# ZikangYuan/sr_livo

Hardware: AMD Instinct MI355X
Metric: sweeps/s (full ESIKF solve of a 64k-pt Livox sweep vs 1M-pt voxel map) (higher is better)
Workload: dtype f64; 1 GPU; HEADLINE: stream of 4 distinct 65536-keypoint livox sweeps (own poses and priors), 978481-pt voxel map (1000000 target), max_num_residuals=2147483647, r=1, K=20; one full ESIKF solve per sweep, every sweep crosses PCIe once (uploaded on the copy stream during the solve before it: resident in HBM when its solve starts); sweeps drawn with seeds 20251309 + 100 j, keeping those that take sweep 0's 2 E; parallelism=single GPU

## Files before the change

include/srlivo_hip_debug.h:

```cpp
#ifndef SRLIVO_HIP_DEBUG_H
#define SRLIVO_HIP_DEBUG_H

#include "srlivo_hip.h"

#ifdef __cplusplus
extern "C" {
#endif

int srl_debug_set_select_mode(srl_ctx *ctx, int select_mode);

int srl_debug_radix_sort_pairs(srl_ctx *ctx, const uint32_t *keys, int n, int bits, uint32_t *keys_sorted, uint32_t *positions_sorted);

int srl_debug_color_map_rebuilds(srl_ctx *ctx, int32_t *voxel_table, int32_t *grid_table);

int srl_debug_set_frame_order_mode(srl_ctx *ctx, int mode);
int srl_debug_frame_order_used(srl_ctx *ctx, int *used);

int srl_debug_set_gather_counts(srl_ctx *ctx, int nranks, int rank, const int64_t *counts);

int srl_debug_set_ablate(srl_ctx *ctx, int bits);
int srl_debug_set_fused_reduce(srl_ctx *ctx, int enable);
int srl_debug_set_bound_culling(srl_ctx *ctx, int enable);
int srl_debug_set_pose_box(srl_ctx *ctx, int kind);
int srl_debug_set_arm_linger(srl_ctx *ctx, double host_linger_us, double kernel_linger_us);
int srl_debug_pass_stamps(srl_ctx *ctx, int enable, long long *gpu_out, long long *host_out);
int srl_debug_frame_timing(srl_ctx *ctx, int enable, double out16[16]);
int srl_debug_set_frame_epoch(srl_ctx *ctx, int frames_to_wrap);
int srl_debug_set_launch_shape(srl_ctx *ctx, int keypoints_per_wave, int waves_per_workgroup);
int srl_debug_set_search_select_mode(srl_ctx *ctx, int select_mode);
int srl_debug_heap_topk(const double *distances, int n, int K, int32_t *out_index);
int srl_debug_device_sqrt(srl_ctx *ctx, const double *in, int n, double *out);
int srl_debug_block_times(srl_ctx *ctx, double *out, int max_blocks, int *nblocks);
enum { SRL_FLOW_PREV = 0, SRL_FLOW_CUR = 1 };
int srl_flow_levels(srl_ctx *ctx, int *L);
int srl_flow_download_level(srl_ctx *ctx, int which, int level, uint8_t *image_padded, int16_t *deriv_padded, int *rows, int *cols);

#ifdef __cplusplus
}
#endif
#endif
```

sr_livo_amd/capi.py:

```python
import ctypes as C
import os
import re

import numpy as np

_HERE = os.path.dirname(os.path.abspath(__file__))
LIB_PATH = os.environ.get("SRL_LIB_PATH") or os.path.join(_HERE, "libsrlivo_hip.so")
INCLUDE_DIR = os.path.join(os.path.dirname(_HERE), "include")

SRL_OK = 0
SRL_ERR_NO_DEVICE = -1
SRL_ERR_BAD_ARG = -3
SRL_ERR_UNSUPPORTED = -4
SRL_ERR_COMM = -7
SRL_ERR_NAN_PLANARITY = -8
SRL_ERR_NOT_ENOUGH_RESIDUALS = -9
SRL_COMM_ID_BYTES = 128


SRL_PEER_HANDLE_BYTES = 64


class SrlError(RuntimeError):
    def __init__(self, status, what, detail=""):
# ... 181 lines not shown
        "srl_map_insert": ([p, p, C.c_int, C.c_double, C.c_int, C.c_double, C.c_int, C.POINTER(C.c_int)], C.c_int),
        "srl_map_insert_report": ([p, p, C.c_int, C.c_double, C.c_int, C.c_double, C.c_int, C.c_double, p, p, C.POINTER(C.c_int),
                                   C.POINTER(C.c_int)], C.c_int),
        "srl_map_size": ([p, C.POINTER(C.c_int64), C.POINTER(C.c_int32)], C.c_int),
        "srl_map_download": ([p, p, p, p, C.c_int], C.c_int),
        "srl_map_remove_far": ([p, dp, C.c_double, C.POINTER(C.c_int32), C.POINTER(C.c_int64)], C.c_int),
        "srl_map_probe_checksum": ([p, p, C.c_int, C.c_int, C.c_double, C.POINTER(C.c_uint64)], C.c_int),
        "srl_color_opts_default": ([C.POINTER(ColorOpts)], None),
        "srl_color_map_create": ([p, C.POINTER(ColorOpts)], C.c_int),
        "srl_color_map_destroy": ([p], C.c_int),
        "srl_color_map_insert": ([p, p, C.c_int, C.c_double, C.c_double, p, p, C.c_int, p, C.c_int, C.POINTER(ColorTotals)], C.c_int),
        "srl_color_map_size": ([p, C.POINTER(C.c_int64), C.POINTER(C.c_int32), C.POINTER(C.c_int64), C.POINTER(C.c_int64)], C.c_int),
        "srl_color_map_download": ([p, p, p, p, C.c_int, p, p, C.c_int64], C.c_int),
        "srl_color_registered_download": ([p, C.c_int64, C.c_int, p], C.c_int),
        "srl_debug_color_map_rebuilds": ([p, C.POINTER(C.c_int32), C.POINTER(C.c_int32)], C.c_int),
        "srl_color_image_upload": ([p, p, C.c_int, C.c_int, C.c_int64], C.c_int),
        "srl_color_select_opts_default": ([C.POINTER(ColorSelectOpts)], None),
        "srl_color_map_select": ([p, C.POINTER(ColorCamera), C.c_int, C.c_int, p, C.c_int, C.POINTER(ColorSelectOpts), p, C.c_int64,
                                  C.POINTER(ColorSelectTotals)], C.c_int),
        "srl_color_map_render": ([p, C.POINTER(ColorCamera), p, C.c_int, C.c_double, C.POINTER(ColorRenderTotals)], C.c_int),
        "srl_color_map_vio_rows": ([p, C.POINTER(ColorVioArgs), p, C.c_int, C.POINTER(ColorVioSums), p, p], C.c_int),
        "srl_flow_opts_default": ([C.POINTER(FlowOpts)], None),
        "srl_flow_create": ([p, C.POINTER(FlowOpts)], C.c_int),
        "srl_flow_destroy": ([p], C.c_int),
        "srl_flow_track_image": ([p, p, C.c_int, C.c_int, C.c_int64, p, C.c_int, p, p, C.POINTER(C.c_int)], C.c_int),
        "srl_flow_levels": ([p, C.POINTER(C.c_int)], C.c_int),
        "srl_flow_download_level": ([p, C.c_int, C.c_int, p, p, C.POINTER(C.c_int), C.POINTER(C.c_int)], C.c_int),
        "srl_lk_create": ([p, C.c_int, C.c_int, C.c_int, C.c_int, C.c_int, C.c_double, C.c_int, C.c_double, C.POINTER(p)], C.c_int),
        "srl_lk_destroy": ([p], C.c_int),
        "srl_lk_get": ([p, C.POINTER(C.c_int), C.POINTER(C.c_int), C.POINTER(C.c_double)], C.c_int),
        "srl_lk_track_image": ([p, p, C.c_int, C.c_int, C.c_int64, p, C.c_int, p, p, C.POINTER(C.c_int)], C.c_int),
        "srl_color_cloud_opts_default": ([C.POINTER(ColorCloudOpts)], None),
        "srl_color_map_export_cloud": ([p, C.c_int64, C.c_int64, C.POINTER(ColorCloudOpts), p, p, C.c_int64, C.POINTER(ColorCloudTotals)], C.c_int),
        "srl_color_map_download_rgb": ([p, p, p, p, p, p, C.c_int64], C.c_int),
        "srl_color_registered_rgb": ([p, C.c_int64, C.c_int, p, p, p, p, p], C.c_int),
        "srl_sweep_upload": ([p, p, C.c_int], C.c_int),
        "srl_sweep_shard": ([p, C.POINTER(C.c_int), C.POINTER(C.c_int), C.POINTER(C.c_int)], C.c_int),
        "srl_sweep_prefetch": ([p, p, C.c_int], C.c_int),
        "srl_sweep_swap": ([p], C.c_int),
        "srl_sweep_wait": ([p], C.c_int),
        "srl_thread_pin_to_gpu_numa": ([p, C.POINTER(C.c_int)], C.c_int),
        "srl_pinned_alloc": ([C.c_size_t, C.POINTER(p)], C.c_int),
        "srl_pinned_free": ([p], C.c_int),
        "srl_host_register": ([p, C.c_size_t], C.c_int),
        "srl_host_unregister": ([p], C.c_int),
        "srl_comm_backend_info": ([C.c_char_p, C.c_int, C.POINTER(C.c_int), C.POINTER(C.c_int)], C.c_int),
        "srl_build_residuals": ([p, C.POINTER(Frame), C.POINTER(IcpOpts), C.POINTER(NormalEq)], C.c_int),
        "srl_build_residuals_overlap": ([p, C.POINTER(Frame), C.POINTER(IcpOpts), C.POINTER(NormalEq), p, p], C.c_int),
        "srl_set_taps": ([p, C.c_int], C.c_int),
        "srl_fetch_neighbors": ([p, p, p, p], C.c_int),
        "srl_fetch_residuals": ([p, p, p, p, p, p, p], C.c_int),
        "srl_search_neighbors": ([p, p, C.c_int, C.c_int, C.c_double, C.c_int, C.c_int, p, p, p], C.c_int),
        "srl_transform_points": ([p, p, C.c_int, dp, dp, dp, dp, p], C.c_int),
        "srl_frame_upload": ([p, p, C.c_int], C.c_int),
        "srl_frame_undistort": ([p, p, p, p, C.c_int, p, C.c_int, C.c_double, C.c_int, dp, dp, p, p], C.c_int),
        "srl_frame_take": ([p, p, C.c_int], C.c_int),
        "srl_frame_subsample": ([p, p, C.c_int, C.c_double, C.POINTER(C.c_int)], C.c_int),
        "srl_frame_take_subsampled": ([p, p, C.c_int, p, p, p], C.c_int),
        "srl_frame_size": ([p, C.POINTER(C.c_int)], C.c_int),
        "srl_frame_select_keypoints": ([p, dp, dp, dp, dp, C.c_double, p, C.POINTER(C.c_int)], C.c_int),
        "srl_frame_commit_report": ([p, dp, dp, dp, dp, C.c_double, C.c_int, C.c_double, C.c_int, p, p, p, C.POINTER(C.c_int),
                                     C.POINTER(C.c_int)], C.c_int),
        "srl_frame_commit": ([p, dp, dp, dp, dp, C.c_double, C.c_int, C.c_double, C.c_int, p, C.POINTER(C.c_int)], C.c_int),
        "srl_comm_unique_id": ([p], C.c_int),
        "srl_comm_init_rank": ([p, C.c_int, C.c_int, p], C.c_int),
        "srl_comm_destroy": ([p], C.c_int),
        "srl_comm_set_library": ([C.c_char_p], C.c_int),
        "srl_comm_suspend": ([p, C.c_int], C.c_int),
        "srl_comm_info": ([p, C.POINTER(C.c_int), C.POINTER(C.c_int), C.POINTER(C.c_int), C.POINTER(C.c_int), C.POINTER(C.c_int64)], C.c_int),
        "srl_comm_set_host_callbacks": ([p, C.c_int, C.c_int, ALLREDUCE_FN, ALLGATHER_FN, p], C.c_int),
        "srl_debug_set_gather_counts": ([p, C.c_int, C.c_int, C.POINTER(C.c_int64)], C.c_int),
        "srl_peer_export": ([p, p, C.POINTER(p)], C.c_int),
        "srl_peer_attach": ([p, C.c_int, C.c_int, p, C.POINTER(p)], C.c_int),
        "srl_peer_set_deadline_ms": ([p, C.c_int], C.c_int),
        "srl_peer_stats": ([p, C.POINTER(C.c_int64), C.POINTER(C.c_int)], C.c_int),
        "srl_peer_detach": ([p], C.c_int),
        "srl_shard_range": ([C.c_int, C.c_int, C.c_int, C.POINTER(C.c_int), C.POINTER(C.c_int)], None),
        "srl_shard_budget": ([C.c_int, C.POINTER(C.c_int64), C.c_int, C.c_int, C.POINTER(C.c_int64), C.POINTER(C.c_int)], None),
        "srl_get_timing": ([p, C.POINTER(Timing)], C.c_int),
        "srl_debug_block_times": ([p, p, C.c_int, C.POINTER(C.c_int)], C.c_int),
        "srl_debug_set_ablate": ([p, C.c_int], C.c_int),
        "srl_debug_set_fused_reduce": ([p, C.c_int], C.c_int),
        "srl_debug_set_bound_culling": ([p, C.c_int], C.c_int),
        "srl_debug_set_pose_box": ([p, C.c_int], C.c_int),
        "srl_debug_set_arm_linger": ([p, C.c_double, C.c_double], C.c_int),
        "srl_debug_pass_stamps": ([p, C.c_int, p, p], C.c_int),
        "srl_debug_frame_timing": ([p, C.c_int, p], C.c_int),
        "srl_debug_set_frame_epoch": ([p, C.c_int], C.c_int),
        "srl_set_armed_launch": ([p, C.c_int], C.c_int),
        "srl_disarm": ([p], C.c_int),
        "srl_solve_end": ([p], C.c_int),
        "srl_get_arm_stats": ([p, C.POINTER(C.c_uint64)], C.c_int),
        "srl_debug_set_launch_shape": ([p, C.c_int, C.c_int], C.c_int),
        "srl_debug_set_search_select_mode": ([p, C.c_int], C.c_int),
        "srl_debug_set_select_mode": ([p, C.c_int], C.c_int),
        "srl_debug_set_frame_order_mode": ([p, C.c_int], C.c_int),
        "srl_debug_radix_sort_pairs": ([p, p, C.c_int, C.c_int, p, p], C.c_int),
        "srl_debug_frame_order_used": ([p, C.POINTER(C.c_int)], C.c_int),
        "srl_debug_heap_topk": ([p, C.c_int, C.c_int, p], C.c_int),
        "srl_debug_device_sqrt": ([p, p, C.c_int, p], C.c_int),
        "srl_set_profiling": ([p, C.c_int], C.c_int),
        "srl_set_profiling_period": ([p, C.c_int], C.c_int),
        "srl_timing_mark": ([p], C.c_int),
        "srl_lio_create": ([C.c_int, C.POINTER(p)], C.c_int),
        "srl_lio_destroy": ([p], C.c_int),
        "srl_lio_ctx": ([p], p),
        "srl_lio_last_error": ([p], C.c_char_p),
        "srl_lio_set_extrinsics": ([p, dp, dp], C.c_int),
        "srl_lio_set_laser_point_cov": ([p, C.c_double], C.c_int),
        "srl_lio_last_solve_launches": ([p, C.POINTER(C.c_int)], C.c_int),
        "srl_lio_eskf_get_state": ([p, dp], C.c_int),
        "srl_lio_eskf_set_state": ([p, dp], C.c_int),
        "srl_lio_eskf_get_cov": ([p, dp], C.c_int),
        "srl_lio_eskf_set_cov": ([p, dp], C.c_int),
        "srl_lio_eskf_set_noise": ([p, C.c_double, C.c_double, C.c_double, C.c_double], C.c_int),
        "srl_lio_eskf_init_imu": ([p, dp, dp], C.c_int),
        "srl_lio_eskf_scale_init_cov": ([p], C.c_int),
        "srl_lio_eskf_predict": ([p, C.c_double, dp, dp], C.c_int),
        "srl_lio_eskf_observe": ([p, dp], C.c_int),
        "srl_lio_add_points_to_map": ([p, p, C.c_int, C.c_double, C.c_int, C.c_double, C.c_int], C.c_int),
        "srl_lio_map_size": ([p, C.POINTER(C.c_int64)], C.c_int),
        "srl_lio_remove_points_far_from_location": ([p, dp, C.c_double], C.c_int),
        "srl_lio_set_collect_points_world": ([p, C.c_int], C.c_int),
        "srl_lio_points_world": ([p, p, C.c_int, C.POINTER(C.c_int)], C.c_int),
        "srl_lio_set_device_subsample": ([p, C.c_int], C.c_int),
        "srl_lio_set_color_map_options": ([p, C.POINTER(ColorOpts)], C.c_int),
        "srl_lio_set_color_times": ([p, C.c_double, C.c_double, C.c_int], C.c_int),
        "srl_lio_add_points_to_map_at": ([p, p, C.c_int, C.c_double, C.c_int, C.c_double, C.c_int, C.c_double, C.c_int], C.c_int),
        "srl_lio_color_cloud": ([p, C.c_int, C.c_int, p, p, C.c_int64, C.POINTER(C.c_int64), C.POINTER(ColorCloudTotals)], C.c_int),
        "srl_lio_color_cloud_view": ([p, C.c_int, C.c_int, C.c_int, C.POINTER(C.c_void_p), C.POINTER(C.c_void_p), C.POINTER(C.c_int64),
                                      C.POINTER(ColorCloudTotals)], C.c_int),
        "srl_lio_color_topic_sizes": ([p, C.c_int64, p, C.c_int, C.POINTER(C.c_int)], C.c_int),
        "srl_lio_color_topic_state": ([p, C.POINTER(C.c_int), C.POINTER(C.c_int)], C.c_int),
        "srl_lio_select_points_for_projection": ([p, C.POINTER(ColorCamera), C.c_int, C.c_int, C.c_double, C.c_int, C.c_int, C.c_int, p, C.c_int,
                                                  C.POINTER(C.c_int), C.POINTER(ColorSelectTotals)], C.c_int),
        "srl_lio_color_visited": ([p, C.c_int, p, C.c_int, C.POINTER(C.c_int), C.POINTER(C.c_int)], C.c_int),
        "srl_lio_color_stored": ([p, p, C.c_int, C.POINTER(C.c_int)], C.c_int),
        "srl_lio_render_points_in_recent_voxel": ([p, C.POINTER(ColorCamera), C.c_double, C.POINTER(ColorRenderTotals)], C.c_int),
        "srl_lio_probe_checksum_of_committed_frame": ([p, C.c_int, C.c_double, C.POINTER(C.c_uint64), C.POINTER(C.c_int32)], C.c_int),
        "srl_lio_resident_sweep": ([p, p, C.c_int], C.c_int),
        "srl_lio_prefetch_sweep": ([p, p, C.c_int], C.c_int),
        "srl_lio_swap_sweep": ([p], C.c_int),
        "srl_lio_prefetch_sweep_during_solve": ([p, p, C.c_int], C.c_int),
        "srl_lio_update_iekf": ([p, C.POINTER(IcpOpts), p, C.c_int, dp, dp, C.c_int, p, C.c_int,
                                 C.POINTER(C.c_int), C.POINTER(C.c_int)], C.c_int),
        "srl_lio_stream_step": ([p, C.POINTER(IcpOpts), dp, dp, C.c_int, dp, dp, C.c_int, p, C.c_int, C.POINTER(C.c_int), C.POINTER(C.c_int)], C.c_int),
        "srl_lio_update_iekf_provided": ([p, C.POINTER(IcpOpts), PROVIDER_FN, p, C.c_int, dp, dp, C.c_int, p, C.c_int,
                                          C.POINTER(C.c_int), C.POINTER(C.c_int)], C.c_int),
        "srl_lio_optimize": ([p, C.POINTER(IcpOpts), C.c_double, p, p, C.c_int, dp, dp, C.c_int, p,
                              C.POINTER(C.c_int), C.POINTER(C.c_int), C.POINTER(C.c_int)], C.c_int),
        "srl_lio_eskf_try_init": ([p, dp, dp, dp, C.c_int, C.POINTER(C.c_int)], C.c_int),
        "srl_lio_eskf_get_init_stats": ([p, dp], C.c_int),
        "srl_lio_set_initial_flag": ([p, C.c_int], C.c_int),
        "srl_lio_state_initialization": ([p, C.c_int, C.c_int, dp, dp, dp], C.c_int),
        "srl_lio_set_odometry_options": ([p, C.POINTER(OdometryOpts)], C.c_int),
        "srl_lio_run_measurement": ([p, C.c_double, p, p, p, C.c_int, p, p, C.c_int, C.c_double, C.c_double,
                                     C.POINTER(ReplayResult)], C.c_int),
        "srl_lio_last_frame": ([p, C.c_int, p, p, p, C.POINTER(C.c_int)], C.c_int),
        "srl_lio_optimize_resident": ([p, C.POINTER(IcpOpts), C.c_double, p, C.c_int, dp, dp, C.c_int, p,
                                       C.POINTER(C.c_int), C.POINTER(C.c_int), C.POINTER(C.c_int)], C.c_int),
        "srl_lio_commit_frame": ([p, dp, C.c_double, C.c_int, C.c_double, C.c_int, p, C.POINTER(C.c_int)], C.c_int),
        "srl_lio_search_neighbors": ([p, dp, C.c_int, C.c_double, C.c_int, C.c_int, p, p, C.POINTER(C.c_int)], C.c_int),
        "srl_lio_neighborhood": ([p, p, C.c_int, dp, dp, dp, dp], C.c_int),
        "srl_lio_build_plane_residuals": ([p, C.POINTER(IcpOpts), p, C.c_int, dp, dp, C.c_int, p, C.c_int,
                                           C.POINTER(C.c_int), dp, C.POINTER(C.c_int), p], C.c_int),
        "srl_lio_vio_set_options": ([p, C.c_int, C.c_int, C.c_int, p, p, p], C.c_int),
# ... 390 lines not shown
        self._chk(self.lib.srl_sweep_wait(self.h), "srl_sweep_wait")

    def sweep_swap(self):
        self._chk(self.lib.srl_sweep_swap(self.h), "srl_sweep_swap")

    def sweep_shard(self):
        b, c, t = C.c_int(), C.c_int(), C.c_int()
        self._chk(self.lib.srl_sweep_shard(self.h, C.byref(b), C.byref(c), C.byref(t)), "srl_sweep_shard")
        return b.value, c.value, t.value

    def set_taps(self, on):
        self._chk(self.lib.srl_set_taps(self.h, int(on)), "srl_set_taps")

    def set_profiling(self, on):
        self._chk(self.lib.srl_set_profiling(self.h, int(on)), "srl_set_profiling")

    def timing_mark(self):
        self._chk(self.lib.srl_timing_mark(self.h), "srl_timing_mark")

    def set_profiling_period(self, period):
        self._chk(self.lib.srl_set_profiling_period(self.h, int(period)), "srl_set_profiling_period")

    def timing(self):
        t = Timing()
        self._chk(self.lib.srl_get_timing(self.h, C.byref(t)), "srl_get_timing")
        return t

    def _select(self, opts):
        mode = int(getattr(opts, "select_mode", 0) or 0)
        if mode != getattr(self, "_select_mode", 0):
            self._chk(self.lib.srl_debug_set_select_mode(self.h, mode), "srl_debug_set_select_mode")
            self._select_mode = mode

    def build_residuals(self, frame, opts, allow=(SRL_ERR_NAN_PLANARITY,)):
        self._select(opts)
        out = NormalEq()
        rc = self._chk(self.lib.srl_build_residuals(self.h, C.byref(frame), C.byref(opts), C.byref(out)), "srl_build_residuals", ok=allow)
        return out, rc

    def build_residuals_overlap(self, frame, opts, fn, allow=(SRL_ERR_NAN_PLANARITY,)):
        self._select(opts)
        out = NormalEq()
        cb = C.CFUNCTYPE(None, C.c_void_p)(lambda _u: fn())
        rc = self._chk(self.lib.srl_build_residuals_overlap(self.h, C.byref(frame), C.byref(opts), C.byref(out), cb, None),
                       "srl_build_residuals_overlap", ok=allow)
        return out, rc

    def pin_thread_to_gpu_numa(self):
        node = C.c_int(-1)
        rc = self.lib.srl_thread_pin_to_gpu_numa(self.h, C.byref(node))
        return node.value if rc == 0 else None

    def fetch_neighbors(self, K=20):
        _, n, _ = self.sweep_shard()
        ids = np.empty((n, K), dtype=np.int32)
        status = np.empty(n, dtype=np.uint8)
        ncand = np.empty(n, dtype=np.int32)
        self._chk(self.lib.srl_fetch_neighbors(self.h, _ptr(ids), _ptr(status), _ptr(ncand)), "srl_fetch_neighbors")
        return ids, status, ncand

    def fetch_residuals(self):
        _, n, _ = self.sweep_shard()
        normal = np.empty((n, 3)); a2d = np.empty(n); w = np.empty(n); off = np.empty(n); d = np.empty(n); J = np.empty((n, 6))
        self._chk(self.lib.srl_fetch_residuals(self.h, _ptr(normal), _ptr(a2d), _ptr(w), _ptr(off), _ptr(d), _ptr(J)), "srl_fetch_residuals")
        return dict(normal=normal, a2D=a2d, weight=w, norm_offset=off, distance=d, jacobian=J)

    def search_neighbors(self, world_xyz, nb=1, size=1.0, K=20, thr=1):
        q = _f64(world_xyz, (-1, 3))
        ids = np.empty((len(q), K), dtype=np.int32)
        xyz = np.empty((len(q), K, 3), dtype=np.float32)
        nf = np.empty(len(q), dtype=np.int32)
        self._chk(self.lib.srl_search_neighbors(self.h, _ptr(q), len(q), nb, size, K, thr, _ptr(ids), _ptr(xyz), _ptr(nf)), "srl_search_neighbors")
        return ids, xyz, nf

    def set_launch_shape(self, kpw, wpb):
        self._chk(self.lib.srl_debug_set_launch_shape(self.h, int(kpw), int(wpb)), "srl_debug_set_launch_shape")

    def set_fused_reduce(self, on):
        self._chk(self.lib.srl_debug_set_fused_reduce(self.h, 1 if on else 0), "srl_debug_set_fused_reduce")

    def set_bound_culling(self, on):
        self._chk(self.lib.srl_debug_set_bound_culling(self.h, 1 if on else 0), "srl_debug_set_bound_culling")

    def set_search_select_mode(self, mode):
        self._chk(self.lib.srl_debug_set_search_select_mode(self.h, int(mode)), "srl_debug_set_search_select_mode")

    def set_armed_launch(self, on):
        mode = int(on) if on in (0, 1, 2) and not isinstance(on, bool) else (1 if on else 0)
        self._chk(self.lib.srl_set_armed_launch(self.h, mode), "srl_set_armed_launch")

    def solve_end(self):
        self._chk(self.lib.srl_solve_end(self.h), "srl_solve_end")

    def disarm(self):
        self._chk(self.lib.srl_disarm(self.h), "srl_disarm")

    def arm_stats(self):
        out = (C.c_uint64 * 4)()
        self._chk(self.lib.srl_get_arm_stats(self.h, out), "srl_get_arm_stats")
        return dict(zip(("armed", "fired", "cancelled", "expired"), (int(v) for v in out)))

    def set_pose_box(self, kind):
        self._chk(self.lib.srl_debug_set_pose_box(self.h, int(kind)), "srl_debug_set_pose_box")

    FRAME_STAGES = ("upload", "select_group", "select_download", "select_host_order", "select_gather", "commit_transform", "commit_download",
                    "insert_sort", "insert_segments", "insert_lookup_create", "insert_replay")

    def set_frame_epoch(self, frames_to_wrap):
        self._chk(self.lib.srl_debug_set_frame_epoch(self.h, int(frames_to_wrap)), "srl_debug_set_frame_epoch")

    def frame_timing(self, enable=True):
        out = np.zeros(16)
        self._chk(self.lib.srl_debug_frame_timing(self.h, 1 if enable else 0, _ptr(out)), "srl_debug_frame_timing")
        return dict(zip(self.FRAME_STAGES, (float(v) for v in out)))

    def pass_stamps(self, enable=True, read=True):
        g = np.zeros((64, 32), dtype=np.int64); h = np.zeros((64, 4), dtype=np.int64)
        self._chk(self.lib.srl_debug_pass_stamps(self.h, 1 if enable else 0, _ptr(g) if read else None, _ptr(h) if read else None), "srl_debug_pass_stamps")
        return g, h

    def set_arm_linger(self, host_linger_us=150.0, kernel_linger_us=300.0):
        self._chk(self.lib.srl_debug_set_arm_linger(self.h, float(host_linger_us), float(kernel_linger_us)), "srl_debug_set_arm_linger")

    def device_sqrt(self, x):
        x = _f64(x).ravel()
        out = np.empty_like(x)
        self._chk(self.lib.srl_debug_device_sqrt(self.h, _ptr(x), len(x), _ptr(out)), "srl_debug_device_sqrt")
        return out

    def transform_points(self, raw_xyz, q, t, R_il=None, t_il=None):
        r = _f64(raw_xyz, (-1, 3))
        out = np.empty_like(r)
        R_il = _f64(np.eye(3) if R_il is None else R_il).ravel()
        t_il = _f64(np.zeros(3) if t_il is None else t_il)
        self._chk(self.lib.srl_transform_points(self.h, _ptr(r), len(r), _dptr(_f64(q)), _dptr(_f64(t)), _dptr(R_il), _dptr(t_il), _ptr(out)), "srl_transform_points")
        return out

    def frame_upload(self, raw_xyz):
        r = _f64(raw_xyz, (-1, 3))
        self._chk(self.lib.srl_frame_upload(self.h, _ptr(r), len(r)), "srl_frame_upload")

    def frame_undistort(self, raw_xyz, relative_time_ms, imu_states, time_frame_begin, mode, R_il=None, t_il=None, imu_point_in=None,
                        want_outputs=True):
        r = _f64(raw_xyz, (-1, 3)); rel = _f64(relative_time_ms)
        st = _f64(imu_states, (-1, 17))
        R_il = _f64(np.eye(3) if R_il is None else R_il).ravel()
        t_il = _f64(np.zeros(3) if t_il is None else t_il)
        pin = None if imu_point_in is None else _f64(imu_point_in, (-1, 3))
        imu = np.empty_like(r) if want_outputs else None
        out = np.empty_like(r) if want_outputs else None
        self._chk(self.lib.srl_frame_undistort(self.h, _ptr(r), _ptr(rel), None if pin is None else _ptr(pin), len(r), _ptr(st), len(st),
                                               float(time_frame_begin), int(mode), _dptr(R_il), _dptr(t_il), _ptr(imu), _ptr(out)),
                  "srl_frame_undistort")
        return imu, out

    def frame_take(self, index):
        idx = np.ascontiguousarray(index, dtype=np.int32)
        self._chk(self.lib.srl_frame_take(self.h, _ptr(idx), len(idx)), "srl_frame_take")

    def frame_subsample(self, order, sample_size):
        o = np.ascontiguousarray(order, dtype=np.int32)
        m = C.c_int()
        self._chk(self.lib.srl_frame_subsample(self.h, _ptr(o), len(o), float(sample_size), C.byref(m)), "srl_frame_subsample")
        self._kept = m.value
        return m.value

# ... 627 lines not shown
```

sr_livo_amd/csrc/srl_capi.cpp:

```cpp
#include "../../include/srlivo_hip.h"
#include "../../include/srlivo_hip_debug.h"
#include "host/srl_la.h"
#include "srl_device.h"
#include "srl_hash.h"
#include "srl_heap.h"

#include <hip/hip_runtime.h>
#include <sched.h>

#include <algorithm>
#include <atomic>
#include <chrono>
#include <climits>
#include <cstdio>
#include <cstdlib>
#include <cstring>
#include <mutex>
#include <string>
#include <vector>

struct SrlMapState;
int srl_map_insert_device(struct srl_ctx *ctx, const double *world_xyz, int n, double voxel_size, int cap,
                          double min_distance_points, int min_num_points, int *num_added);

#include "srl_ctx.h"
int srl_map_insert_report_device(srl_ctx *ctx, const double *world_xyz, int n, double voxel_size, int cap, double min_distance_points, int min_num_points,
                                 double ref_z, uint8_t *outcome, srl_cloud_point *cloud, int *num_cloud, int *num_added);

namespace {

unsigned next_pow2(unsigned v) { unsigned p = 1; while (p < v) p <<= 1; return p; }
inline long long steady_ns() { return std::chrono::duration_cast<std::chrono::nanoseconds>(std::chrono::steady_clock::now().time_since_epoch()).count(); }

constexpr int SRL_MAX_DEVICES = 64;
std::atomic<int> g_live_ctx[SRL_MAX_DEVICES];
inline int live_contexts(int device) { return (device >= 0 && device < SRL_MAX_DEVICES) ? g_live_ctx[device].load(std::memory_order_relaxed) : 1; }

int ensure_work(srl_ctx *ctx, int n) {
    if (n <= ctx->work_cap) return SRL_OK;
    const int cap = std::max(n, 1024);
    const int nblocks = std::max((cap + SRL_KPB - 1) / SRL_KPB, 1024 + 8);
    int rc;
    if ((rc = ensure(ctx, ctx->d_rec, (size_t)cap * 8))) return rc;
    if ((rc = ensure(ctx, ctx->d_status, (size_t)cap))) return rc;
    if ((rc = ensure(ctx, ctx->d_bound, (size_t)cap * 4))) return rc;
    ctx->bound_n = 0;
    if ((rc = ensure(ctx, ctx->d_partials, (size_t)nblocks * SRL_PART_STRIDE))) return rc;
    if ((rc = ensure(ctx, ctx->d_binfo, (size_t)nblocks))) return rc;
    ctx->work_cap = cap;
    ctx->block_cap = nblocks;
    return SRL_OK;
}

bool srl_is_pinned(const void *p) {
    hipPointerAttribute_t attr;
    if (hipPointerGetAttributes(&attr, p) != hipSuccess) { (void)hipGetLastError(); return false; }
    return attr.type == hipMemoryTypeHost;
}

int srl_ring_init(srl_ctx *ctx) {
    if (ctx->h_ring) return SRL_OK;
    HIPCHK(ctx, hipHostMalloc((void **)&ctx->h_ring, (size_t)srl_ctx::RING_SLOTS * srl_ctx::RING_SLOT_BYTES, hipHostMallocDefault));
    for (int i = 0; i < srl_ctx::RING_SLOTS; i++) { HIPCHK(ctx, hipEventCreateWithFlags(&ctx->ring_ev[i], hipEventDisableTiming)); ctx->ring_busy[i] = false; }
    return SRL_OK;
}

int ensure_taps(srl_ctx *ctx, int n, int K) {
    if (n <= ctx->tap_cap && K <= ctx->tap_K) return SRL_OK;
    const int cap = std::max(n, ctx->tap_cap), kk = std::max(K, ctx->tap_K);
    int rc;
    if ((rc = ensure(ctx, ctx->d_tap_ids, (size_t)cap * kk))) return rc;
    if ((rc = ensure(ctx, ctx->d_tap_ncand, (size_t)cap))) return rc;
    if ((rc = ensure(ctx, ctx->d_tap_normal, (size_t)cap * 3))) return rc;
    if ((rc = ensure(ctx, ctx->d_tap_a2d, (size_t)cap))) return rc;
    if ((rc = ensure(ctx, ctx->d_tap_offset, (size_t)cap))) return rc;
    ctx->tap_cap = cap;
    ctx->tap_K = kk;
    return SRL_OK;
}

}

int srl_ctx_ensure_work(srl_ctx *ctx, int n) { return ensure_work(ctx, n); }
bool srl_ctx_is_pinned(const void *p) { return srl_is_pinned(p); }

int srl_ctx_grow_map(srl_ctx *ctx, unsigned need_slabs, unsigned need_slots);

extern "C" {

int srl_device_count(int *count) {
    int c = 0;
    if (hipGetDeviceCount(&c) != hipSuccess) { if (count) *count = 0; return SRL_ERR_NO_DEVICE; }
    if (count) *count = c;
    return SRL_OK;
}

const char *srl_status_str(int s) {
    switch (s) {
        case SRL_OK: return "ok";
        case SRL_ERR_NO_DEVICE: return "no HIP device (the product has no CPU fallback)";
        case SRL_ERR_HIP: return "HIP runtime error";
        case SRL_ERR_BAD_ARG: return "bad argument";
        case SRL_ERR_UNSUPPORTED: return "option outside the supported envelope";
        case SRL_ERR_NO_MAP: return "no map uploaded";
        case SRL_ERR_NO_SWEEP: return "no sweep uploaded";
        case SRL_ERR_COMM: return "RCCL error";
        case SRL_ERR_NAN_PLANARITY: return "NaN planarity (optimize.cpp:348-350 throws)";
        case SRL_ERR_NOT_ENOUGH_RESIDUALS: return "not enough residuals (optimize.cpp:110)";
        default: return "unknown status";
    }
}

void srl_icp_opts_default(srl_icp_opts *o) {
    o->threshold_voxel_occupancy = 1;
    o->init_num_frames = 20;
    o->size_voxel_map = 1.0;
    o->num_iters_icp = 5;
    o->min_number_neighbors = 20;
    o->voxel_neighborhood = 1;
    o->power_planarity = 2.0;
    o->max_number_neighbors = 20;
    o->max_dist_to_plane_icp = 0.3;
    o->threshold_orientation_norm = 0.1;
    o->threshold_translation_norm = 0.01;
    o->max_num_residuals = 600;
    o->weight_alpha = 0.9;
    o->weight_neighborhood = 0.1;
}

int srl_ctx_create(int device, srl_ctx **out) {
    if (!out) return SRL_ERR_BAD_ARG;
    *out = nullptr;
    int count = 0;
    if (hipGetDeviceCount(&count) != hipSuccess || count <= 0 || device < 0 || device >= count) return SRL_ERR_NO_DEVICE;
    if (hipSetDevice(device) != hipSuccess) return SRL_ERR_NO_DEVICE;
    srl_ctx *ctx = new srl_ctx();
    ctx->device = device;
    { int cu = 0; if (hipDeviceGetAttribute(&cu, hipDeviceAttributeMultiprocessorCount, device) == hipSuccess && cu > 0) ctx->num_cu = cu; }
    if (hipStreamCreateWithFlags(&ctx->stream, hipStreamNonBlocking) != hipSuccess) { delete ctx; return SRL_ERR_NO_DEVICE; }
    if (hipMalloc((void **)&ctx->d_out, sizeof(SrlDevOut)) != hipSuccess ||
        hipHostMalloc((void **)&ctx->h_out, sizeof(SrlDevOut)) != hipSuccess ||
        hipMalloc((void **)&ctx->d_count, sizeof(long long)) != hipSuccess ||
        hipHostMalloc((void **)&ctx->h_count, sizeof(long long)) != hipSuccess) {
        delete ctx;
        return SRL_ERR_HIP;
    }
    {
        const size_t row_bytes = (size_t)(SRL_FUSED_MAX_BLOCKS + SRL_FUSED_MAX_GROUPS) * SRL_ROW_GRANULES * 8;
        if (hipMalloc((void **)&ctx->d_granules, row_bytes) != hipSuccess || hipMemset(ctx->d_granules, 0, row_bytes) != hipSuccess) { delete ctx; return SRL_ERR_HIP; }
    }
    if (hipHostMalloc((void **)&ctx->h_mail, sizeof(SrlMailbox), hipHostMallocCoherent | hipHostMallocMapped) != hipSuccess) {
        delete ctx;
        return SRL_ERR_HIP;
    }
    std::memset(ctx->h_mail, 0, sizeof(SrlMailbox));
    for (int i = 0; i < 4; i++) hipEventCreate(&ctx->ev[i]);
    if (device < SRL_MAX_DEVICES) g_live_ctx[device].fetch_add(1, std::memory_order_relaxed);
    ctx->counted = true;
    *out = ctx;
    return SRL_OK;
}

int srl_ctx_destroy(srl_ctx *ctx) {
    if (!ctx) return SRL_OK;
    hipSetDevice(ctx->device);
    if (ctx->counted && ctx->device < SRL_MAX_DEVICES) g_live_ctx[ctx->device].fetch_sub(1, std::memory_order_relaxed);
    if (ctx->armed) srl_ctx_disarm(ctx);
    if (ctx->stream) hipStreamSynchronize(ctx->stream);
    if (ctx->copy_stream) hipStreamSynchronize(ctx->copy_stream);
    if (ctx->color) srl_color_map_destroy(ctx);
    if (ctx->flow) srl_flow_destroy(ctx);
    if (ctx->pose_box_pinned) hipHostFree(ctx->pose_box_pinned);
    if (ctx->pose_box_dev) hipFree(ctx->pose_box_dev);
    if (ctx->d_pose_relay) hipFree(ctx->d_pose_relay);
    if (ctx->comm && srl_rccl()) srl_rccl()->CommDestroy(ctx->comm);
    if (ctx->parked_comm && srl_rccl()) srl_rccl()->CommDestroy(ctx->parked_comm);
    if (ctx->d_sub_kept) hipFree(ctx->d_sub_kept);
    if (ctx->d_sub_seen) hipFree(ctx->d_sub_seen);
    void *bufs[] = {ctx->d_corr_in, ctx->d_corr_rel, ctx->d_corr_imu, ctx->d_corr_raw, ctx->d_corr_seg, ctx->d_frame_raw, ctx->d_frame_world, ctx->d_table, ctx->d_slabs, ctx->d_raw, ctx->d_rec, ctx->d_status, ctx->d_partials, ctx->d_binfo,
                    ctx->d_out, ctx->d_count, ctx->d_bound, ctx->d_granules, ctx->d_rec_granules, ctx->d_raw_next, ctx->d_stage_next, ctx->d_stage_cur, ctx->d_tap_ids, ctx->d_tap_ncand, ctx->d_tap_normal, ctx->d_tap_a2d,
                    ctx->d_tap_offset, ctx->d_gather, ctx->d_peer, ctx->d_mail};
    for (int r = 0; r < SRL_MAX_PEERS; r++) if (ctx->peer_mapped[r]) hipIpcCloseMemHandle(ctx->peer_mapped[r]);
    if (ctx->d_inbox) hipFree(ctx->d_inbox);
    for (void *b : bufs) if (b) hipFree(b);
    if (ctx->h_out) hipHostFree(ctx->h_out);
    if (ctx->h_count) hipHostFree(ctx->h_count);
    if (ctx->h_mail) hipHostFree(ctx->h_mail);
    if (ctx->h_arm_stamps) hipHostFree(ctx->h_arm_stamps);
    if (ctx->h_scratch) hipHostFree(ctx->h_scratch);
    if (ctx->h_frame_x) hipHostFree(ctx->h_frame_x);
    for (SrlEpochTable *t : {&ctx->sel_table, &ctx->ins_table}) { if (t->keyw) hipFree(t->keyw); if (t->minw) hipFree(t->minw); }
    if (ctx->d_frame_sync) hipFree(ctx->d_frame_sync);
    if (ctx->d_tr1_sched) hipFree(ctx->d_tr1_sched);
    if (ctx->h_insert_cnt) hipHostFree(ctx->h_insert_cnt);
    if (ctx->ev_insert) hipEventDestroy(ctx->ev_insert);
    if (ctx->ev_world) hipEventDestroy(ctx->ev_world);
    if (ctx->ev_frame_read) hipEventDestroy(ctx->ev_frame_read);
    if (ctx->h_ring) { hipHostFree(ctx->h_ring); for (int i = 0; i < srl_ctx::RING_SLOTS; i++) if (ctx->ring_ev[i]) hipEventDestroy(ctx->ring_ev[i]); }
    for (auto &b : ctx->pool_free) hipFree(b.p);
    ctx->pool_free.clear();
    for (int i = 0; i < 4; i++) if (ctx->ev[i]) hipEventDestroy(ctx->ev[i]);
    for (int i = 0; i < srl_ctx::PROF_RING; i++) for (int k = 0; k < 2; k++) if (ctx->ring[i][k]) hipEventDestroy(ctx->ring[i][k]);
    for (int sl = 0; sl < 2; sl++) for (int k = 0; k < 2; k++) if (ctx->up_ev[sl][k]) hipEventDestroy(ctx->up_ev[sl][k]);
    if (ctx->upload_ev) hipEventDestroy(ctx->upload_ev);
    if (ctx->copy_stream) { hipStreamSynchronize(ctx->copy_stream); hipStreamDestroy(ctx->copy_stream); }
    if (ctx->prefix_stream) { hipStreamSynchronize(ctx->prefix_stream); hipStreamDestroy(ctx->prefix_stream); }
    if (ctx->stream) hipStreamDestroy(ctx->stream);
    delete ctx;
    return SRL_OK;
}

const char *srl_last_error(const srl_ctx *ctx) { return ctx ? ctx->err.c_str() : "null context"; }

int srl_map_upload(srl_ctx *ctx, const int16_t *keys_xyz, const int32_t *counts, const float *xyz, int V, int cap) {
    if (!ctx || V < 0 || (V > 0 && (!keys_xyz || !counts || !xyz))) return SRL_ERR_BAD_ARG;
    SRL_DISARM(ctx);
    if (cap != SRL_VOXEL_CAP) { ctx->err = "max_num_points_in_voxel must be 20"; return SRL_ERR_UNSUPPORTED; }
    HIPCHK(ctx, hipSetDevice(ctx->device));
    { const int rcs = srl_map_settle(ctx); if (rcs) return rcs; }
    ctx->bound_n = 0;
    const unsigned slab_cap = std::max<unsigned>(1024u, (unsigned)V + (unsigned)V / 2u + 4096u);
    if (slab_cap > SRL_MAX_SLABS) { ctx->err = "map too large: slab byte offsets are 32-bit (16.7 M voxels)"; return SRL_ERR_UNSUPPORTED; }
    const unsigned table_cap = next_pow2(std::max<unsigned>(2048u, SRL_TABLE_FACTOR * slab_cap));
    std::vector<SrlSlab> slabs((size_t)V);
    std::vector<SrlMapSlot> table((size_t)table_cap);
    for (auto &s : table) { s.key = SRL_EMPTY_KEY; s.slab = 0; s.count = 0; }
    long long npts = 0;
    const unsigned mask = table_cap - 1;
    for (int v = 0; v < V; v++) {
        SrlSlab &s = slabs[v];
        std::memset(&s, 0, sizeof s);
        const int c = counts[v];
        if (c < 0 || c > cap) { ctx->err = "voxel count out of range"; return SRL_ERR_BAD_ARG; }
        for (int i = 0; i < c; i++)
            for (int d = 0; d < 3; d++) s.xyz[i][d] = xyz[((size_t)v * cap + i) * 3 + d];
        s.count = (unsigned)c;
        s.key = srl_pack_key(keys_xyz[3 * v], keys_xyz[3 * v + 1], keys_xyz[3 * v + 2]);
        npts += c;
        unsigned h = srl_hash_key(s.key) & mask;
        while (table[h].key != SRL_EMPTY_KEY) {
            if (table[h].key == s.key) { ctx->err = "duplicate voxel key in upload"; return SRL_ERR_BAD_ARG; }
            h = (h + 1) & mask;
        }
        table[h].key = s.key;
        table[h].slab = (unsigned)v;
        table[h].count = (unsigned)c;
    }
    if (ctx->d_slabs) { HIPCHK(ctx, hipFree(ctx->d_slabs)); ctx->d_slabs = nullptr; }
    if (ctx->d_table) { HIPCHK(ctx, hipFree(ctx->d_table)); ctx->d_table = nullptr; }
    HIPCHK(ctx, hipMalloc((void **)&ctx->d_slabs, ((size_t)slab_cap + 1) * SRL_SLAB_BYTES));
    HIPCHK(ctx, hipMemsetD32Async((hipDeviceptr_t)(ctx->d_slabs + (size_t)slab_cap * SRL_SLAB_BYTES), 0x7f800000, SRL_SLAB_BYTES / 4, ctx->stream));
    HIPCHK(ctx, hipMalloc((void **)&ctx->d_table, (size_t)table_cap * sizeof(SrlMapSlot)));
    HIPCHK(ctx, hipMemsetAsync(ctx->d_slabs, 0, (size_t)slab_cap * SRL_SLAB_BYTES, ctx->stream));
    if (V > 0) HIPCHK(ctx, hipMemcpyAsync(ctx->d_slabs, slabs.data(), (size_t)V * SRL_SLAB_BYTES, hipMemcpyHostToDevice, ctx->stream));
    HIPCHK(ctx, hipMemcpyAsync(ctx->d_table, table.data(), (size_t)table_cap * sizeof(SrlMapSlot), hipMemcpyHostToDevice, ctx->stream));
    HIPCHK(ctx, hipStreamSynchronize(ctx->stream));
    ctx->slab_cap = slab_cap;
    ctx->table_cap = table_cap;
    ctx->num_voxels = V;
    ctx->num_points = npts;
    return SRL_OK;
}

int srl_map_size(srl_ctx *ctx, int64_t *num_points, int32_t *num_voxels) {
    if (!ctx) return SRL_ERR_BAD_ARG;
    { const int rcs = srl_map_settle(ctx); if (rcs) return rcs; }
    if (num_points) *num_points = ctx->num_points;
    if (num_voxels) *num_voxels = ctx->num_voxels;
    return SRL_OK;
}

int srl_map_download(srl_ctx *ctx, int16_t *keys_xyz, int32_t *counts, float *xyz, int max_voxels) {
    if (!ctx) return SRL_ERR_BAD_ARG;
    SRL_DISARM(ctx);
    if (!ctx->d_slabs) return SRL_ERR_NO_MAP;
    { const int rcs = srl_map_settle(ctx); if (rcs) return rcs; }
    const int V = ctx->num_voxels;
    if (max_voxels < V) return SRL_ERR_BAD_ARG;
    HIPCHK(ctx, hipSetDevice(ctx->device));
    std::vector<SrlSlab> slabs((size_t)V);
    if (V > 0) HIPCHK(ctx, hipMemcpyAsync(slabs.data(), ctx->d_slabs, (size_t)V * SRL_SLAB_BYTES, hipMemcpyDeviceToHost, ctx->stream));
    HIPCHK(ctx, hipStreamSynchronize(ctx->stream));
    for (int v = 0; v < V; v++) {
        short x, y, z;
        srl_unpack_key(slabs[v].key, &x, &y, &z);
        if (keys_xyz) { keys_xyz[3 * v] = x; keys_xyz[3 * v + 1] = y; keys_xyz[3 * v + 2] = z; }
        if (counts) counts[v] = (int32_t)slabs[v].count;
        if (xyz)
            for (int i = 0; i < SRL_CAP; i++)
                for (int d = 0; d < 3; d++)
                    xyz[((size_t)v * SRL_CAP + i) * 3 + d] = (i < (int)slabs[v].count) ? slabs[v].xyz[i][d] : 0.0f;
    }
    return SRL_OK;
}

int srl_map_insert(srl_ctx *ctx, const double *world_xyz, int n, double voxel_size, int cap,
                   double min_distance_points, int min_num_points, int *num_added) {
    if (!ctx || n < 0 || (n > 0 && !world_xyz)) return SRL_ERR_BAD_ARG;
    SRL_DISARM(ctx);
    if (cap != SRL_VOXEL_CAP) { ctx->err = "max_num_points_in_voxel must be 20"; return SRL_ERR_UNSUPPORTED; }
    return srl_map_insert_device(ctx, world_xyz, n, voxel_size, cap, min_distance_points, min_num_points, num_added);
}

int srl_map_insert_report(srl_ctx *ctx, const double *world_xyz, int n, double voxel_size, int cap, double min_distance_points, int min_num_points,
                          double ref_z, uint8_t *outcome, srl_cloud_point *cloud, int *num_cloud, int *num_added) {
    if (num_cloud) *num_cloud = 0;
    if (num_added) *num_added = 0;
    if (!ctx || n < 0 || (n > 0 && !world_xyz)) return SRL_ERR_BAD_ARG;
    SRL_DISARM(ctx);
    if (cap != SRL_VOXEL_CAP) { ctx->err = "max_num_points_in_voxel must be 20"; return SRL_ERR_UNSUPPORTED; }
    return srl_map_insert_report_device(ctx, world_xyz, n, voxel_size, cap, min_distance_points, min_num_points, ref_z, outcome, cloud, num_cloud, num_added);
}

namespace {
int upload_aos(srl_ctx *ctx, const char *src, size_t bytes, double *d_stage, hipStream_t st, bool last = true, int pinned = -1) {
    if (pinned < 0 ? srl_is_pinned(src) : pinned != 0) {
        HIPCHK(ctx, hipMemcpyAsync(d_stage, src, bytes, hipMemcpyHostToDevice, st));
        if (last) {
            if (!ctx->upload_ev) HIPCHK(ctx, hipEventCreateWithFlags(&ctx->upload_ev, hipEventDisableTiming));
            HIPCHK(ctx, hipEventRecord(ctx->upload_ev, st));
            ctx->upload_pending = true;
        }
        return SRL_OK;
    }
    int rc2 = srl_ring_init(ctx);
    if (rc2) return rc2;
    size_t off = 0;
    while (off < bytes) {
        const size_t len = std::min(bytes - off, (size_t)srl_ctx::RING_SLOT_BYTES);
        const int slot = ctx->ring_next++ % srl_ctx::RING_SLOTS;
        if (ctx->ring_busy[slot]) { HIPCHK(ctx, hipEventSynchronize(ctx->ring_ev[slot])); ctx->ring_busy[slot] = false; }
        std::memcpy(ctx->h_ring + (size_t)slot * srl_ctx::RING_SLOT_BYTES, src + off, len);
        {
            hipError_t e__ = hipMemcpyAsync(reinterpret_cast<char *>(d_stage) + off, ctx->h_ring + (size_t)slot * srl_ctx::RING_SLOT_BYTES, len,
                                            hipMemcpyHostToDevice, st);
            if (e__ != hipSuccess) {
                char buf[256];
                std::snprintf(buf, sizeof buf, "ring upload: %s (dst %p + %zu, ring %p slot %d, len %zu, stream %p, main stream %p)", hipGetErrorString(e__),
                              (void *)d_stage, off, (void *)ctx->h_ring, slot, len, (void *)st, (void *)ctx->stream);
                ctx->err = buf;
                return SRL_ERR_HIP;
            }
        }
        HIPCHK(ctx, hipEventRecord(ctx->ring_ev[slot], st));
        ctx->ring_busy[slot] = true;
        off += len;
    }
    return SRL_OK;
}
}

int srl_sweep_upload(srl_ctx *ctx, const double *raw_xyz, int n) {
    if (!ctx || n < 0 || (n > 0 && !raw_xyz)) return SRL_ERR_BAD_ARG;
    SRL_DISARM(ctx);
    HIPCHK(ctx, hipSetDevice(ctx->device));
    int b = 0, cnt = 0;
    srl_shard_range(n, ctx->nranks, ctx->rank, &b, &cnt);
    ctx->total_n = n;
    ctx->shard_begin = b;
    ctx->n = cnt;
    ctx->sweep_loaded = true;
    ctx->taps_valid = false;
    ctx->passes_in_solve = 0;
    ctx->tail_pending = false;
    ctx->bound_n = 0;
    if (cnt > ctx->sweep_cap) {
        const int cap = std::max(cnt, 1024);
        int rc = ensure(ctx, ctx->d_raw, (size_t)cap * 3);
        if (rc) return rc;
        ctx->sweep_cap = cap;
    }
    int rc = ensure_work(ctx, cnt);
    if (rc) return rc;
    if (cnt > 0) {
        int rcu = upload_aos(ctx, reinterpret_cast<const char *>(raw_xyz + (size_t)b * 3), (size_t)cnt * 3 * sizeof(double), ctx->d_rec, ctx->stream);
        if (rcu) return rcu;
        HIPCHK(ctx, srl_launch_aos_to_soa(ctx->d_rec, cnt, ctx->d_raw, ctx->d_raw + ctx->sweep_cap, ctx->d_raw + 2 * (size_t)ctx->sweep_cap, ctx->stream));
    }
    ctx->soa_valid_n = cnt;
    return SRL_OK;
}

int srl_sweep_wait(srl_ctx *ctx) {
    if (!ctx) return SRL_ERR_BAD_ARG;
    SRL_DISARM(ctx);
    if (ctx->upload_pending) {
        HIPCHK(ctx, hipSetDevice(ctx->device));
        HIPCHK(ctx, hipEventSynchronize(ctx->upload_ev));
        if (ctx->prefix_stream) HIPCHK(ctx, hipStreamSynchronize(ctx->prefix_stream));
        ctx->upload_pending = false;
    }
    return SRL_OK;
}

int srl_sweep_prefetch(srl_ctx *ctx, const double *raw_xyz, int n) {
    if (!ctx || n < 0 || (n > 0 && !raw_xyz)) return SRL_ERR_BAD_ARG;
    HIPCHK(ctx, hipSetDevice(ctx->device));
    if (!ctx->copy_stream) SRL_DISARM(ctx);
    { const int rcc = ensure_copy_stream(ctx); if (rcc) return rcc; }
    if (!ctx->up_ev[0][0]) {
        SRL_DISARM(ctx);
        for (int sl = 0; sl < 2; sl++) for (int k = 0; k < 2; k++) HIPCHK(ctx, hipEventCreateWithFlags(&ctx->up_ev[sl][k], hipEventDisableTiming));
    }
    int b = 0, cnt = 0;
    srl_shard_range(n, ctx->nranks, ctx->rank, &b, &cnt);
    if (cnt > ctx->next_cap || cnt > ctx->stage_next_cap) {
        const int cap = std::max(cnt, 1024);
        SRL_DISARM(ctx);
        HIPCHK(ctx, hipStreamSynchronize(ctx->copy_stream));
        int rc;
        if (cnt > ctx->next_cap) { if ((rc = ensure(ctx, ctx->d_raw_next, (size_t)cap * 3))) return rc; ctx->next_cap = cap; HIPCHK(ctx, hipMemsetAsync(ctx->d_raw_next, 0, (size_t)cap * 3 * sizeof(double), ctx->copy_stream)); }
        if (cnt > ctx->stage_next_cap) { if ((rc = ensure(ctx, ctx->d_stage_next, (size_t)cap * 3))) return rc; ctx->stage_next_cap = cap; }
    }
    const int slot = ctx->next_slot ^ 1;
    const int pre = (ctx->prefix_hint > 0 && ctx->prefix_hint < cnt) ? ctx->prefix_hint : cnt;
    if (cnt > 0) {
        const char *src = reinterpret_cast<const char *>(raw_xyz + (size_t)b * 3);
        const int pinned = srl_is_pinned(src) ? 1 : 0;
        if (pre < cnt && pinned) {
            if (!ctx->prefix_stream) { SRL_DISARM(ctx); HIPCHK(ctx, hipStreamCreateWithFlags(&ctx->prefix_stream, hipStreamNonBlocking)); }
            int rcu = upload_aos(ctx, src, (size_t)pre * 3 * sizeof(double), ctx->d_stage_next, ctx->prefix_stream, false, 1);
            if (rcu) return rcu;
            HIPCHK(ctx, hipEventRecord(ctx->up_ev[slot][0], ctx->prefix_stream));
            rcu = upload_aos(ctx, src + (size_t)pre * 3 * sizeof(double), (size_t)(cnt - pre) * 3 * sizeof(double), ctx->d_stage_next + (size_t)pre * 3, ctx->copy_stream, true, 1);
            if (rcu) return rcu;
            ctx->up_one_dma[slot] = false;
        } else {
            int rcu = upload_aos(ctx, src, (size_t)cnt * 3 * sizeof(double), ctx->d_stage_next, ctx->copy_stream, true, pinned);
            if (rcu) return rcu;
            ctx->up_one_dma[slot] = true;
        }
    } else {
        ctx->up_one_dma[slot] = true;
    }
    HIPCHK(ctx, hipEventRecord(ctx->up_ev[slot][1], ctx->copy_stream));
    ctx->next_ready = ctx->up_ev[slot][1];
    ctx->next_slot = slot; ctx->next_prefix_n = ctx->up_one_dma[slot] ? cnt : pre;
    ctx->next_n = cnt; ctx->next_begin = b; ctx->next_total = n;
    return SRL_OK;
}

int srl_sweep_swap(srl_ctx *ctx) {
    if (!ctx) return SRL_ERR_BAD_ARG;
    if (ctx->next_n < 0) { SRL_DISARM(ctx); ctx->err = "srl_sweep_swap: nothing prefetched"; return SRL_ERR_NO_SWEEP; }
    HIPCHK(ctx, hipSetDevice(ctx->device));
    const bool one_dma = ctx->up_one_dma[ctx->next_slot];
    hipEvent_t ev_full = ctx->up_ev[ctx->next_slot][1], ev_pre = ctx->up_ev[ctx->next_slot][one_dma ? 1 : 0];
    hipError_t up_pre = hipEventQuery(ev_pre);
    hipError_t up = (one_dma || up_pre != hipSuccess) ? up_pre : hipEventQuery(ev_full);
    if (up_pre == hipErrorNotReady && ctx->armed && ctx->next_n <= ctx->work_cap) {
        const long long t_give_up = steady_ns() + 25000;
        while ((up_pre = hipEventQuery(ev_pre)) == hipErrorNotReady && steady_ns() < t_give_up) { }
    }
    for (hipError_t e : {up, up_pre})
        if (e != hipSuccess && e != hipErrorNotReady) { ctx->err = std::string("hipEventQuery: ") + hipGetErrorString(e); return SRL_ERR_HIP; }
    if (up_pre != hipSuccess || ctx->next_n > ctx->work_cap) SRL_DISARM(ctx);
    if (up_pre != hipSuccess) {
        HIPCHK(ctx, hipStreamWaitEvent(ctx->stream, ev_full, 0));
        if (!one_dma) HIPCHK(ctx, hipStreamWaitEvent(ctx->stream, ev_pre, 0));
        up = hipSuccess;
    }
    ctx->tail_pending = up != hipSuccess;
    ctx->bound_n = 0;
    ctx->cur_slot = ctx->next_slot;
    ctx->cur_prefix_n = up == hipSuccess ? ctx->next_n : ctx->next_prefix_n;
    ctx->passes_in_solve = 0;
    std::swap(ctx->d_raw, ctx->d_raw_next);
    std::swap(ctx->sweep_cap, ctx->next_cap);
    std::swap(ctx->d_stage_cur, ctx->d_stage_next);
    std::swap(ctx->stage_cur_cap, ctx->stage_next_cap);
    ctx->soa_valid_n = 0;
    ctx->n = ctx->next_n; ctx->shard_begin = ctx->next_begin; ctx->total_n = ctx->next_total;
    ctx->next_n = -1;
    ctx->sweep_loaded = true;
    ctx->taps_valid = false;
    return ensure_work(ctx, ctx->n);
}

int srl_thread_pin_to_gpu_numa(srl_ctx *ctx, int *numa_node) {
    if (!ctx) return SRL_ERR_BAD_ARG;
    if (numa_node) *numa_node = -1;
    char bus[64] = {0};
    if (hipDeviceGetPCIBusId(bus, (int)sizeof bus, ctx->device) != hipSuccess) { (void)hipGetLastError(); return SRL_ERR_UNSUPPORTED; }
    for (char *c = bus; *c; ++c) if (*c >= 'A' && *c <= 'F') *c = (char)(*c - 'A' + 'a');
    const std::string base = std::string("/sys/bus/pci/devices/") + bus;
    int node = -1;
    if (FILE *f = std::fopen((base + "/numa_node").c_str(), "r")) { if (std::fscanf(f, "%d", &node) != 1) node = -1; std::fclose(f); }
    char list[1024] = {0};
    if (FILE *f = std::fopen((base + "/local_cpulist").c_str(), "r")) { if (!std::fgets(list, (int)sizeof list, f)) list[0] = 0; std::fclose(f); }
    if (node < 0 || !list[0]) return SRL_ERR_UNSUPPORTED;
    cpu_set_t allowed, want;
    CPU_ZERO(&want);
    if (sched_getaffinity(0, sizeof allowed, &allowed) != 0) return SRL_ERR_UNSUPPORTED;
    int any = 0;
    for (const char *p = list; *p && *p != '\n';) {
        char *end = nullptr;
        const long a = std::strtol(p, &end, 10);
        long b = a;
        if (end == p) break;
        p = end;
        if (*p == '-') { b = std::strtol(p + 1, &end, 10); p = end; }
        for (long c = a; c <= b && c < CPU_SETSIZE; ++c) if (CPU_ISSET((int)c, &allowed)) { CPU_SET((int)c, &want); any = 1; }
        if (*p == ',') ++p;
    }
    if (!any) return SRL_ERR_UNSUPPORTED;
    if (sched_setaffinity(0, sizeof want, &want) != 0) return SRL_ERR_UNSUPPORTED;
    if (numa_node) *numa_node = node;
    return SRL_OK;
}

int srl_pinned_alloc(size_t bytes, void **out) {
    if (!out) return SRL_ERR_BAD_ARG;
    *out = nullptr;
    if (hipHostMalloc(out, bytes ? bytes : 1, hipHostMallocDefault) != hipSuccess) { (void)hipGetLastError(); return SRL_ERR_HIP; }
    return SRL_OK;
}
int srl_pinned_free(void *p) {
    if (!p) return SRL_OK;
    return hipHostFree(p) == hipSuccess ? SRL_OK : SRL_ERR_HIP;
}
int srl_host_register(void *p, size_t bytes) {
    if (!p || !bytes) return SRL_ERR_BAD_ARG;
    if (hipHostRegister(p, bytes, hipHostRegisterDefault) != hipSuccess) { (void)hipGetLastError(); return SRL_ERR_HIP; }
    return SRL_OK;
}
int srl_host_unregister(void *p) {
    if (!p) return SRL_ERR_BAD_ARG;
    if (hipHostUnregister(p) != hipSuccess) { (void)hipGetLastError(); return SRL_ERR_HIP; }
    return SRL_OK;
}

int srl_sweep_shard(srl_ctx *ctx, int *begin, int *count, int *total) {
    if (!ctx) return SRL_ERR_BAD_ARG;
    if (begin) *begin = ctx->shard_begin;
    if (count) *count = ctx->n;
    if (total) *total = ctx->total_n;
    return SRL_OK;
}

int srl_set_taps(srl_ctx *ctx, int enable) {
    if (!ctx) return SRL_ERR_BAD_ARG;
    SRL_DISARM(ctx);
    ctx->taps = enable != 0;
    if (!ctx->taps) ctx->taps_valid = false;
    return SRL_OK;
}
// ... 272 lines not shown
    const bool init_mode = f->frame_id < o->init_num_frames;
    p.nb = init_mode ? 2 : o->voxel_neighborhood;
    p.thr = init_mode ? 1 : o->threshold_voxel_occupancy;
    p.K = o->max_number_neighbors;
    if (p.nb < 1 || p.nb > 2) { ctx->err = "voxel_neighborhood must be 1 or 2"; return SRL_ERR_UNSUPPORTED; }
    if (p.K < 1 || p.K > SRL_MAX_NEIGHBORS) { ctx->err = "max_number_neighbors must be in [1,32]"; return SRL_ERR_UNSUPPORTED; }
    if (!(o->size_voxel_map > 0.0)) return SRL_ERR_BAD_ARG;

    p.kpw = srl_keypoints_per_wave(n_eff);
    p.wpb = 4;
    const int k1 = srl_keypoints_per_wave_one_round(n_eff, ctx->num_cu);
    if (n_eff >= 2048 && srl_assoc_lds_bytes(p.K, p.nb, k1, 16) <= SRL_LDS_LIMIT) { p.kpw = k1; p.wpb = 16; }
    if (ctx->force_kpw) {
        p.kpw = ctx->force_kpw;
        const bool only16 = p.kpw != 4 && p.kpw != 8 && p.kpw != 16;
        p.wpb = ((ctx->force_wpb == 16 || only16) && srl_assoc_lds_bytes(p.K, p.nb, p.kpw, 16) <= SRL_LDS_LIMIT) ? 16 : 4;
        if (only16 && p.wpb != 16) p.kpw = 4;
    }
    if (ctx->ablate != 0 && srl_assoc_lds_bytes(p.K, p.nb, 16, 16) <= SRL_LDS_LIMIT) { p.kpw = 16; p.wpb = 16; }
    p.kpb = p.kpw * p.wpb;
    p.nblocks = (n_eff + p.kpb - 1) / p.kpb;

    p.cut = cut_possible(ctx, o);
    p.transport = pass_transport(ctx);
    p.dbg_gather = ctx->dbg_gather;
    const bool fusable = !ctx->taps && ctx->ablate == 0 && o->max_num_residuals > 0 && ctx->fuse_reduce && !ctx->dbg_gather;
    p.fuse_cut = fusable && p.cut && p.transport == Transport::single && p.wpb == 16 && p.kpb <= SRL_FUSED_CUT_MAX_KPB && p.nblocks <= 512;
    p.fused = p.fuse_cut || (fusable && !p.cut && p.wpb == 16 && p.nblocks <= SRL_FUSED_MAX_BLOCKS);
    p.tagged_mail = p.fused && p.transport != Transport::rccl;
    p.mailbox = p.transport != Transport::rccl && (p.transport == Transport::single || p.fused);
    const bool fast_sel = ctx->select_mode == 0 || ctx->select_mode == 4;
    p.arm_ok = ctx->arm_mode != 0 && p.fused && fast_sel && ctx->profiling != 1 && (p.transport != Transport::host_callback || ctx->cb_ar);
    return SRL_OK;
}

static void prepare_assoc_args(srl_ctx *ctx, const srl_frame *f, const srl_icp_opts *o, int n_eff, const PassPlan &p, SrlAssocArgs &a) {
    std::memset(&a, 0, sizeof a);
    a.raw_x = ctx->d_raw;
    a.raw_y = ctx->d_raw + ctx->sweep_cap;
    a.raw_z = ctx->d_raw + 2 * (size_t)ctx->sweep_cap;
    a.n = n_eff;
    a.aos = (n_eff > ctx->soa_valid_n) ? ctx->d_stage_cur : nullptr;
    a.table = ctx->d_table;
    a.table_mask = ctx->table_cap - 1;
    a.slabs = ctx->d_slabs;
    a.inf_off = ctx->slab_cap * (unsigned)SRL_SLAB_BYTES;
    a.write_rec = ((ctx->taps || p.cut) && !p.fuse_cut) ? 1 : 0;
    {
        const srl::Quat q(f->q[0], f->q[1], f->q[2], f->q[3]);
        const srl::Mat3 Rn = q.normalized().toRotationMatrix();
        const srl::Mat3 R = q.toRotationMatrix();
        std::memcpy(a.Rn, Rn.a, sizeof a.Rn);
        std::memcpy(a.R, R.a, sizeof a.R);
    }
    std::memcpy(a.t, f->t, sizeof a.t);
    std::memcpy(a.t_last, f->t_last, sizeof a.t_last);
    std::memcpy(a.R_il, f->R_il, sizeof a.R_il);
    std::memcpy(a.t_il, f->t_il, sizeof a.t_il);
    a.size_voxel = o->size_voxel_map;
    a.max_dist = o->max_dist_to_plane_icp;
    {
        double lw = std::abs(o->weight_alpha), ln = std::abs(o->weight_neighborhood);
        const double sum = lw + ln;
        lw /= sum;
        ln /= sum;
        a.lambda_w = lw;
        a.lambda_n = ln;
    }
    a.power_planarity = o->power_planarity;
    a.nbr_scale = o->max_dist_to_plane_icp * o->min_number_neighbors;
    a.K = p.K;
    a.min_nb = o->min_number_neighbors;
    a.thr_cap = p.thr;
    a.select_mode = ctx->select_mode;
    a.ablate = ctx->ablate;
    a.stamps = ctx->h_arm_stamps;
    a.rec = ctx->d_rec;
    a.status = ctx->d_status;
    a.partials = ctx->d_partials;
    a.binfo = ctx->d_binfo;
    if (ctx->taps) {
        a.tap_ids = ctx->d_tap_ids;
        a.tap_ncand = ctx->d_tap_ncand;
        a.tap_normal = ctx->d_tap_normal;
        a.tap_a2d = ctx->d_tap_a2d;
        a.tap_offset = ctx->d_tap_offset;
    }
    {
        float sv = (float)o->size_voxel_map;
        int sv_bits; std::memcpy(&sv_bits, &sv, 4);
        const int sig[4] = {p.K, p.nb, p.thr, sv_bits};
        if (std::memcmp(sig, ctx->bound_sig, sizeof sig) != 0) { ctx->bound_n = 0; std::memcpy(ctx->bound_sig, sig, sizeof sig); }
        a.bound_out = ctx->d_bound;
        a.bound_in = ctx->bound_mode != 0 ? ctx->d_bound : nullptr;
        a.bound_use = a.bound_in ? std::min(ctx->bound_n, n_eff) : 0;
    }
    if (p.fused) {
        a.granules = ctx->d_granules;
        a.mailbox = p.transport == Transport::rccl ? ctx->d_mail : ctx->h_mail;
        a.mail_tagged = p.tagged_mail ? 1 : 0;
    }
    if (p.fuse_cut) {
        a.rec_granules = ctx->d_rec_granules;
        a.cut_max = o->max_num_residuals;
    }
}

static int grow_pass_buffers(srl_ctx *ctx, const PassPlan &p) {
    int rc;
    ctx->taps_valid = false;
    if (ctx->taps) {
        if ((rc = ensure_taps(ctx, ctx->n, p.K))) return rc;
        if (ctx->n > 0) {
            HIPCHK(ctx, hipMemsetAsync(ctx->d_tap_ids, 0xFF, (size_t)ctx->n * p.K * sizeof(int), ctx->stream));
            HIPCHK(ctx, hipMemsetAsync(ctx->d_tap_normal, 0, (size_t)ctx->n * 3 * sizeof(double), ctx->stream));
            HIPCHK(ctx, hipMemsetAsync(ctx->d_tap_a2d, 0, (size_t)ctx->n * sizeof(double), ctx->stream));
            HIPCHK(ctx, hipMemsetAsync(ctx->d_tap_offset, 0, (size_t)ctx->n * sizeof(double), ctx->stream));
        }
    }
    ctx->last_nblocks = p.nblocks;
    if (p.nblocks > ctx->block_cap) {
        if ((rc = ensure(ctx, ctx->d_partials, (size_t)p.nblocks * SRL_PART_STRIDE))) return rc;
        if ((rc = ensure(ctx, ctx->d_binfo, (size_t)p.nblocks))) return rc;
        ctx->block_cap = p.nblocks;
    }
    if (ctx->profiling == 2 && ctx->ring_head - ctx->ring_tail >= (unsigned)srl_ctx::PROF_RING && (rc = drain_ring(ctx, true))) return rc;
    if (p.fused && p.transport == Transport::rccl && !ctx->d_mail && (rc = ensure(ctx, ctx->d_mail, 1))) return rc;
    const size_t need = (size_t)p.nblocks * p.kpb * 16;
    if (p.fuse_cut && need > ctx->rec_granule_cap) {
        if ((rc = ensure(ctx, ctx->d_rec_granules, need))) return rc;
        HIPCHK(ctx, hipMemsetAsync(ctx->d_rec_granules, 0, need * sizeof(unsigned long long), ctx->stream));
        ctx->rec_granule_cap = need;
    }
    return SRL_OK;
}

struct ExchangeTag { unsigned long long seq; unsigned epoch; int slot; };
static ExchangeTag exchange_tag(unsigned long long seq) {
    if ((unsigned)seq == 0u) ++seq;
    return {seq, (unsigned)seq, (int)(seq & 1ull)};
}
static ExchangeTag next_exchange(srl_ctx *ctx) {
    const ExchangeTag t = exchange_tag(ctx->peer_seq + 1);
    ctx->peer_seq = t.seq;
    return t;
}

static SrlAssocArgs arm_signature(const SrlAssocArgs &src) {
    SrlAssocArgs sg = src;
    std::memset(sg.Rn, 0, sizeof sg.Rn); std::memset(sg.R, 0, sizeof sg.R); std::memset(sg.t, 0, sizeof sg.t);
    std::memset(sg.t_last, 0, sizeof sg.t_last);
    sg.pose_box = nullptr; sg.pose_relay = nullptr; sg.pose_relayed = 0; sg.pose_epoch = 0; sg.arm_linger_ticks = 0;
    sg.raw_x = sg.raw_y = sg.raw_z = nullptr; sg.alt_x = sg.alt_y = sg.alt_z = nullptr; sg.n = 0; sg.aos = nullptr; sg.alt_aos = nullptr;
    sg.bound_use = 0;
    return sg;
}

static int fire_or_cancel(srl_ctx *ctx, const PassPlan &p, SrlAssocArgs &a, unsigned long long &seq_now, bool &fired) {
    fired = false;
    bool needs_tail = false;
    if (ctx->tail_pending) {
        if (hipEventQuery(ctx->up_ev[ctx->cur_slot][1]) == hipSuccess) { ctx->tail_pending = false; ctx->cur_prefix_n = ctx->n; }
        else needs_tail = a.n > ctx->cur_prefix_n;
        (void)hipGetLastError();
    }
    if (!ctx->armed) return SRL_OK;
    const SrlAssocArgs sg = arm_signature(a);
    const double age_us = (double)(steady_ns() - ctx->armed_at_ns) * 1e-3;
    const bool on_raw = a.raw_x == ctx->armed_raw && ctx->sweep_cap == ctx->armed_raw_cap && a.aos == nullptr;
    const bool on_alt = !on_raw && ctx->armed_alt != nullptr && a.raw_x == ctx->armed_alt && ctx->sweep_cap == ctx->armed_alt_cap &&
                        a.aos != nullptr && a.aos == ctx->armed_alt_aos;
    if (p.arm_ok && !needs_tail && age_us < ctx->arm_host_linger_us && p.nb == ctx->armed_nb && p.kpw == ctx->armed_kpw &&
        p.nblocks <= ctx->armed_nblocks && (on_raw || on_alt) && std::memcmp(&sg, &ctx->armed_sig, sizeof sg) == 0) {
        pose_box_write(ctx, a.Rn, a.R, a.t, (unsigned)seq_now, SRL_ARM_GO | (on_alt ? SRL_ARM_ALT : 0u), (unsigned)a.n, a.t_last);
        ctx->armed = false;
        ctx->armed_ring = -1;
        ctx->arm_stats[1]++;
        ctx->cur_measured = ctx->armed_measured;
        ctx->cur_gen = ctx->armed_gen;
        fired = true;
        return SRL_OK;
    }
    if (const int rc = srl_ctx_disarm(ctx)) return rc;
    seq_now = ++ctx->seq;
    if (p.fused) a.seq = seq_now;
    return SRL_OK;
}

static int prof_role(const srl_ctx *ctx) {
    if (ctx->prof_period <= 1) return 2;
    const unsigned long long r = ctx->prof_count % (unsigned long long)ctx->prof_period;
    return r == 1 ? 2 : (r == 0 ? 1 : 0);
}

static int launch_assoc(srl_ctx *ctx, const PassPlan &p, const SrlAssocArgs &args, bool armed) {
    if (!armed && ctx->tail_pending) {
        HIPCHK(ctx, hipStreamWaitEvent(ctx->stream, ctx->up_ev[ctx->cur_slot][1], 0));
        ctx->tail_pending = false; ctx->cur_prefix_n = ctx->n;
    }
    const bool prof = ctx->profiling == 1, prof_light = ctx->profiling == 2;
    const int role = prof_light ? prof_role(ctx) : 0;
    int prev = -1;
    if (armed && role != 0) {
        int rc;
        if (ctx->ring_head - ctx->ring_tail >= (unsigned)srl_ctx::PROF_RING - 2 && (rc = drain_ring(ctx, true))) return rc;
        if (ctx->ring_head != 0 && !ctx->ring_void[(ctx->ring_head - 1) % srl_ctx::PROF_RING] && ctx->ring_last_count == (long long)ctx->prof_count - 1)
            prev = (int)((ctx->ring_head - 1) % srl_ctx::PROF_RING);
    }
    const unsigned slot = ctx->ring_head % srl_ctx::PROF_RING;
    if (prof) HIPCHK(ctx, hipEventRecord(ctx->ev[0], ctx->stream));
    if (role == 2 && prev < 0) HIPCHK(ctx, hipEventRecord(ctx->ring[slot][0], ctx->stream));
    HIPCHK(ctx, srl_launch_assoc(args, p.nb, p.kpw, p.wpb, ctx->stream));
    if (prof) HIPCHK(ctx, hipEventRecord(ctx->ev[1], ctx->stream));
    if (role != 0) {
        HIPCHK(ctx, hipEventRecord(ctx->ring[slot][1], ctx->stream));
        ctx->ring_prev[slot] = prev; ctx->ring_marker[slot] = role == 1; ctx->ring_void[slot] = false; ctx->ring_gen[slot] = ctx->timing_gen;
        ctx->ring_last_count = (long long)ctx->prof_count;
        ctx->ring_head++;
    }
    if (prof_light) ctx->prof_count++;
    const bool measured = !prof_light || role == 2;
    if (armed) { ctx->armed_ring = role != 0 ? (int)slot : -1; ctx->armed_measured = measured; ctx->armed_gen = ctx->timing_gen; }
    else { ctx->cur_measured = measured; ctx->cur_gen = ctx->timing_gen; }
    return SRL_OK;
}

static bool arm_wanted(const srl_ctx *ctx) {
    return ctx->arm_mode == 2 ||
           (live_contexts(ctx->device) <= 1 && !ctx->peer_shares_device && !ctx->comm_shares_device &&
            (ctx->next_n >= 0 || ctx->expected_passes == 0 || ctx->passes_in_solve + 1 < ctx->expected_passes));
}

static int arm_next(srl_ctx *ctx, const PassPlan &p, const SrlAssocArgs &a) {
    int rc;
    if ((rc = ensure_pose_box(ctx))) return rc;
    SrlAssocArgs nx = a;
    nx.seq = ctx->seq + 1;
    nx.bound_use = a.bound_in ? a.n : 0;
    const bool has_alt = ctx->d_raw_next != nullptr && ctx->next_cap > 0 && ctx->d_stage_next != nullptr;
    nx.aos = nullptr;
    nx.alt_aos = has_alt ? ctx->d_stage_next : nullptr;
    nx.alt_x = has_alt ? ctx->d_raw_next : nullptr;
    nx.alt_y = has_alt ? ctx->d_raw_next + ctx->next_cap : nullptr;
    nx.alt_z = has_alt ? ctx->d_raw_next + 2 * (size_t)ctx->next_cap : nullptr;
    if (p.transport == Transport::peer) {
        const ExchangeTag t = exchange_tag(ctx->peer_seq + 1);
        nx.peer_epoch = t.epoch;
        nx.peer_slot = t.slot;
    }
    nx.pose_box = ctx->h_pose_box;
    nx.pose_relay = ctx->d_pose_relay;
    nx.pose_relayed = ctx->pose_box_kind == 1 ? 0 : 1;
    nx.pose_epoch = (unsigned)nx.seq;
    nx.arm_linger_ticks = ctx->arm_linger_ticks;
    if ((rc = launch_assoc(ctx, p, nx, true))) return rc;
    ctx->armed_sig = arm_signature(nx);
    ctx->armed_nb = p.nb; ctx->armed_kpw = p.kpw; ctx->armed_nblocks = p.nblocks;
    ctx->armed_raw = nx.raw_x; ctx->armed_raw_cap = ctx->sweep_cap;
    ctx->armed_alt = nx.alt_x; ctx->armed_alt_cap = has_alt ? ctx->next_cap : 0; ctx->armed_alt_aos = nx.alt_aos;
    ctx->armed_at_ns = steady_ns();
    ctx->armed = true;
    ctx->arm_stats[0]++;
    return SRL_OK;
}

static int reduce_unfused(srl_ctx *ctx, const PassPlan &p, const srl_icp_opts *o, int n_eff, unsigned long long seq) {
    int64_t budget = o->max_num_residuals;
    int mode = 0;
    const long long *gather = nullptr;
    if (p.transport == Transport::single || !p.cut) {
        srl_shard_budget(o->max_num_residuals, nullptr, ctx->nranks, ctx->rank, &budget, &mode);
    } else {
        HIPCHK(ctx, srl_launch_count(ctx->d_binfo, p.nblocks, o->max_num_residuals <= 0 ? 1 : 0, ctx->d_count, ctx->stream));
        if (p.transport == Transport::peer) {
            const ExchangeTag t = next_exchange(ctx);
            HIPCHK(ctx, srl_launch_peer_counts(ctx->d_peer, t.epoch, t.slot, ctx->d_count, ctx->d_gather, ctx->stream));
            gather = ctx->d_gather;
        } else if (p.transport == Transport::rccl) {
            NCCLCHK(ctx, AllGather(ctx->d_count, ctx->d_gather, 1, ncclInt64, ctx->comm, ctx->stream));
            gather = ctx->d_gather;
        } else if (p.dbg_gather) {
            gather = ctx->d_gather;
        } else {
            HIPCHK(ctx, hipMemcpyAsync(ctx->h_count, ctx->d_count, sizeof(long long), hipMemcpyDeviceToHost, ctx->stream));
            HIPCHK(ctx, hipStreamSynchronize(ctx->stream));
            if (!ctx->cb_ag) { ctx->err = "nranks > 1 without communicator"; return SRL_ERR_COMM; }
            int64_t mine = *ctx->h_count;
            std::vector<int64_t> all64((size_t)ctx->nranks, 0);
            if (ctx->cb_ag(&mine, all64.data(), ctx->cb_user) != 0) { ctx->err = "allgather callback failed"; return SRL_ERR_COMM; }
            srl_shard_budget(o->max_num_residuals, all64.data(), ctx->nranks, ctx->rank, &budget, &mode);
        }
    }
    SrlReduceArgs ra;
    ra.rec = ctx->d_rec;
    ra.status = ctx->d_status;
    ra.partials = ctx->d_partials;
    ra.binfo = ctx->d_binfo;
    ra.n = n_eff;
    ra.kpb = p.kpb;
    ra.nblocks = p.nblocks;
    ra.max_res = budget;
    ra.gather = gather;
    ra.rank = ctx->rank;
    ra.max_num_residuals = o->max_num_residuals;
    ra.out = ctx->d_out;
    ra.mailbox = p.mailbox ? ctx->h_mail : nullptr;
    ra.seq = seq;
    HIPCHK(ctx, srl_launch_reduce(ra, mode, ctx->stream));
    if (p.transport == Transport::peer) {
        const ExchangeTag t = next_exchange(ctx);
        HIPCHK(ctx, srl_launch_peer_rows(ctx->d_peer, t.epoch, t.slot, ctx->d_out, ctx->h_mail, seq, gather, ctx->stream));
    }
    return SRL_OK;
}

static int host_allreduce(srl_ctx *ctx, SrlDevOut *out) {
    if (!ctx->cb_ar) { ctx->err = "nranks > 1 without communicator"; return SRL_ERR_COMM; }
    if (ctx->cb_ar(reinterpret_cast<double *>(out), SRL_REDUCED_DOUBLES, ctx->cb_user) != 0) { ctx->err = "allreduce callback failed"; return SRL_ERR_COMM; }
    return SRL_OK;
}
// ... 14 lines not shown
        if (fired && __atomic_load_n(&ctx->h_mail->expired, __ATOMIC_ACQUIRE) == seq) {
            ctx->arm_stats[3]++;
            ctx->err = "armed launch expired";
            return SRL_INTERNAL_ARM_EXPIRED;
        }
        if ((++spins & 0xFFFFF) == 0) {
            const hipError_t qe = hipStreamQuery(ctx->stream);
            if (qe != hipSuccess && qe != hipErrorNotReady) { ctx->err = std::string("reduce kernel: ") + hipGetErrorString(qe); return SRL_ERR_HIP; }
            if (qe == hipSuccess && !mail_arrived(ctx, p.tagged_mail, seq)) {
                const unsigned long long *gran = ctx->h_mail->g;
                char dbg[256];
                int bad = -1; unsigned bad_tag = 0;
                if (p.tagged_mail) for (int i = 0; i < 2 * OUT_WORDS; i++) if ((unsigned)(gran[i] >> 32) != (unsigned)seq) { bad = i; bad_tag = (unsigned)(gran[i] >> 32); break; }
                std::snprintf(dbg, sizeof dbg, "reduce kernel finished without publishing (seq %llu, tagged %d, fired %d, fused %d, blocks %d, first stale granule %d tag %u, plain seq %llu)",
                              seq, (int)p.tagged_mail, (int)fired, (int)p.fused, p.nblocks, bad, bad_tag, (unsigned long long)ctx->h_mail->seq);
                ctx->err = dbg;
                return SRL_ERR_HIP;
            }
        }
    }
    if (p.tagged_mail) {
        const unsigned long long *gran = ctx->h_mail->g;
        unsigned long long *w = reinterpret_cast<unsigned long long *>(ctx->h_out);
        for (int i = 0; i < OUT_WORDS; i++)
            w[i] = (__atomic_load_n(&gran[2 * i], __ATOMIC_RELAXED) & 0xFFFFFFFFull) | (__atomic_load_n(&gran[2 * i + 1], __ATOMIC_RELAXED) << 32);
    } else {
        std::memcpy(ctx->h_out, &ctx->h_mail->out, sizeof(SrlDevOut));
    }
    return SRL_OK;
}

static int wait_result(srl_ctx *ctx, const PassPlan &p, unsigned long long seq, bool fired, long long &last_visited_local) {
    const bool copied = p.transport == Transport::host_callback && !p.fused;
    int rc;
    if (copied) {
        HIPCHK(ctx, hipMemcpyAsync(ctx->h_out, ctx->d_out, sizeof(SrlDevOut), hipMemcpyDeviceToHost, ctx->stream));
        HIPCHK(ctx, hipStreamSynchronize(ctx->stream));
    } else if ((rc = read_mailbox(ctx, p, seq, fired))) {
        return rc;
    }
    last_visited_local = ctx->h_out->last_visited;
    if (p.transport == Transport::host_callback && (rc = host_allreduce(ctx, ctx->h_out))) return rc;
    if (copied) {
        if (ctx->h_out->d_timeout > 0.5) { ctx->err = "fused final reduction timed out on another rank"; return SRL_INTERNAL_FUSED_TIMEOUT; }
        return SRL_OK;
    }
    if (ctx->h_out->pad == SRL_PEER_TIMEOUT_MARK) {
        ctx->err = "direct peer exchange: a rank's row has not arrived yet";
        return SRL_INTERNAL_PEER_TIMEOUT;
    }
    if (ctx->h_out->pad != 0 || ctx->h_out->d_timeout > 0.5) {
        ctx->err = "fused final reduction timed out waiting for a workgroup's row";
        if (fired && p.transport == Transport::rccl) ctx->arm_stats[3]++;
        return SRL_INTERNAL_FUSED_TIMEOUT;
    }
    return SRL_OK;
}

static int finish_pass(srl_ctx *ctx, const PassPlan &p, const srl_icp_opts *o, const SrlAssocArgs &a, int n_eff, long long last_visited_local,
                       unsigned long long seq, bool fired, srl_normal_eq *out) {
    const SrlDevOut &r = *ctx->h_out;
    const long long visited_total = (long long)(r.d_visited + 0.5);
    if (p.fused && !p.fuse_cut) {
        const long long expect = ctx->nranks > 1 ? (long long)ctx->total_n : (long long)n_eff;
        if (visited_total != expect) {
            char buf[256];
            std::snprintf(buf, sizeof buf, "fused pass visited %lld of %lld keypoints (fired %d, seq %llu; residuals %.0f, time-out flag %.0f, marker %lld)", visited_total, expect,
                          (int)fired, seq, r.d_num_res, r.d_timeout, (long long)r.pad);
            ctx->err = buf;
            return SRL_ERR_HIP;
        }
    }
    std::memcpy(out->HtH, r.HtH, sizeof out->HtH);
    std::memcpy(out->Hth, r.Hth, sizeof out->Hth);
    out->loss_sum = r.loss;
    out->num_residuals = (int32_t)(r.d_num_res + 0.5);
    out->success = out->num_residuals >= o->min_number_neighbors ? 1 : 0;
    out->sum_candidates = (int64_t)(r.d_sum_pk + 0.5);
    out->last_visited = visited_total - 1;
    out->nan_error = r.d_nan > 0.5 ? 1 : 0;
    out->num_fallback = (int32_t)(r.d_fallback + 0.5);

    if (a.aos != nullptr && n_eff > ctx->soa_valid_n) ctx->soa_valid_n = n_eff;
    ctx->bound_n = n_eff;
    ctx->last_K = p.K;
    ctx->last_nb = p.nb;
    ctx->last_visited_local = last_visited_local;
    ctx->taps_valid = ctx->taps;
    return SRL_OK;
}

struct PassClock { std::chrono::steady_clock::time_point entry, prep, launched, enq, res; };

static long long clock_ns(std::chrono::steady_clock::time_point t) {
    return std::chrono::duration_cast<std::chrono::nanoseconds>(t.time_since_epoch()).count();
}

static int account_pass(srl_ctx *ctx, const PassPlan &p, int n_eff, const PassClock &c) {
    using us = std::chrono::duration<double, std::micro>;
    using ms = std::chrono::duration<double, std::milli>;
    const bool prof = ctx->profiling == 1, prof_light = ctx->profiling == 2;
    if (prof) {
        HIPCHK(ctx, hipEventSynchronize(ctx->ev[3]));
        hipEventElapsedTime(&ctx->timing.assoc_ms, ctx->ev[0], ctx->ev[1]);
        hipEventElapsedTime(&ctx->timing.reduce_ms, ctx->ev[1], ctx->ev[2]);
        hipEventElapsedTime(&ctx->timing.total_ms, ctx->ev[0], ctx->ev[3]);
        ctx->timing.calls += 1;
        ctx->timing.sum_assoc_ms += ctx->timing.assoc_ms;
        ctx->timing.sum_reduce_ms += ctx->timing.reduce_ms;
        ctx->timing.sum_total_ms += ctx->timing.total_ms;
        ctx->timing.sum_keypoints += n_eff;
        const auto t_end = std::chrono::steady_clock::now();
        ctx->timing.sum_host_launch_us += us(c.enq - c.entry).count();
        ctx->timing.sum_host_wait_us += us(c.res - c.enq).count();
        ctx->timing.sum_host_total_us += us(t_end - c.entry).count();
    }
    const double sum_pk = ctx->h_out->d_sum_pk;
    const long long side = 2 * p.nb + 1;
    const long long per_kp = 24 + 12 * side * side * side;
    const double pk_share = (ctx->nranks > 1 && ctx->total_n > 0) ? sum_pk * ((double)ctx->n / (double)ctx->total_n) : sum_pk;
    ctx->timing.algorithmic_bytes = per_kp * (long long)n_eff + (long long)(12.0 * pk_share);
    if (prof || (prof_light && ctx->cur_measured && ctx->cur_gen == ctx->timing_gen)) {
        ctx->timing.sum_algorithmic_bytes += ctx->timing.algorithmic_bytes; ctx->timing.sum_keypoints += prof_light ? n_eff : 0; ctx->timing.sum_passes += 1;
    }
    if (ctx->profiling == 3) {
        ctx->timing.calls += 1;
        ctx->timing.sum_host_launch_us += us(c.launched - c.prep).count();
        ctx->timing.sum_host_wait_us += us(c.res - c.enq).count();
        ctx->timing.sum_host_total_us += us(std::chrono::steady_clock::now() - c.entry).count();
        ctx->timing.sum_assoc_ms += ms(c.prep - c.entry).count();
        ctx->timing.sum_reduce_ms += ms(c.enq - c.launched).count();
    }
    return SRL_OK;
}

static int build_residuals_pass(srl_ctx *ctx, const srl_frame *f, const srl_icp_opts *o, srl_normal_eq *out, int n_eff) {
    PassClock clk{std::chrono::steady_clock::now()};
    HIPCHK(ctx, hipSetDevice(ctx->device));
    PassPlan p;
    int rc;
    if ((rc = plan_pass(ctx, f, o, n_eff, p))) return rc;
    if ((rc = grow_pass_buffers(ctx, p))) return rc;
    SrlAssocArgs a;
    prepare_assoc_args(ctx, f, o, n_eff, p, a);
    unsigned long long seq_now = ++ctx->seq;
    if (p.transport == Transport::peer && ctx->peer_failed) {
        ctx->err = "direct peer exchange: this session has failed (a rank's row never arrived); srl_peer_detach, srl_peer_export and srl_peer_attach on every rank start a new one";
        return SRL_ERR_COMM;
    }
    if (p.fused) a.seq = seq_now;
    if (p.fused && p.transport == Transport::peer) {
        const ExchangeTag t = next_exchange(ctx);
        a.peer = ctx->d_peer; a.peer_epoch = t.epoch; a.peer_slot = t.slot;
    }
    bool fired = false;
    if ((rc = fire_or_cancel(ctx, p, a, seq_now, fired))) return rc;
    clk.prep = std::chrono::steady_clock::now();
    if (!fired && (rc = launch_assoc(ctx, p, a, false))) return rc;
    clk.launched = std::chrono::steady_clock::now();
    long long *stamps = ctx->h_arm_stamps ? ctx->arm_host_stamps[seq_now & 63ull] : nullptr;
    if (stamps) { stamps[0] = clock_ns(clk.entry); stamps[1] = clock_ns(clk.launched); stamps[3] = fired ? 1 : 0; }
    const bool arm = p.arm_ok && arm_wanted(ctx);
    if (arm && p.transport != Transport::rccl && (rc = arm_next(ctx, p, a))) return rc;
    if (!p.fused && (rc = reduce_unfused(ctx, p, o, n_eff, seq_now))) return rc;
    if (ctx->profiling == 1) HIPCHK(ctx, hipEventRecord(ctx->ev[2], ctx->stream));
    clk.enq = std::chrono::steady_clock::now();
// ... 54 lines not shown
        if (distance) distance[k] = rec[(size_t)k * 8 + 6];
        if (weight) weight[k] = rec[(size_t)k * 8 + 7];
    }
    return SRL_OK;
}

int srl_search_neighbors(srl_ctx *ctx, const double *world_xyz, int n, int nb_voxels_visited, double size_voxel_map,
                         int max_num_neighbors, int threshold_voxel_capacity, int32_t *ids, float *nb_xyz,
                         int32_t *num_found) {
    if (!ctx || n < 0 || (n > 0 && (!world_xyz || !ids || !num_found))) return SRL_ERR_BAD_ARG;
    SRL_DISARM(ctx);
    if (!ctx->d_table) return SRL_ERR_NO_MAP;
    if (nb_voxels_visited < 1 || nb_voxels_visited > 2) { ctx->err = "nb_voxels_visited must be 1 or 2"; return SRL_ERR_UNSUPPORTED; }
    if (max_num_neighbors < 1 || max_num_neighbors > SRL_MAX_NEIGHBORS) { ctx->err = "max_num_neighbors must be in [1,32]"; return SRL_ERR_UNSUPPORTED; }
    if (n == 0) return SRL_OK;
    HIPCHK(ctx, hipSetDevice(ctx->device));
    const int K = max_num_neighbors;
    DevBuf b_q, b_ids, b_nf, b_xyz;
    HIPCHK(ctx, b_q.alloc(ctx, (size_t)n * 3 * sizeof(double)));
    HIPCHK(ctx, b_ids.alloc(ctx, (size_t)n * K * sizeof(int)));
    HIPCHK(ctx, b_nf.alloc(ctx, (size_t)n * sizeof(int)));
    if (nb_xyz) HIPCHK(ctx, b_xyz.alloc(ctx, (size_t)n * K * 3 * sizeof(float)));
    double *d_q = b_q.as<double>();
    int *d_ids = b_ids.as<int>(), *d_nf = b_nf.as<int>();
    float *d_xyz = nb_xyz ? b_xyz.as<float>() : nullptr;
    HIPCHK(ctx, hipMemcpyAsync(d_q, world_xyz, (size_t)n * 3 * sizeof(double), hipMemcpyHostToDevice, ctx->stream));
    HIPCHK(ctx, hipMemsetAsync(d_ids, 0xFF, (size_t)n * K * sizeof(int), ctx->stream));
    if (d_xyz) HIPCHK(ctx, hipMemsetAsync(d_xyz, 0, (size_t)n * K * 3 * sizeof(float), ctx->stream));
    SrlSearchArgs a;
    a.q = d_q; a.n = n; a.table = ctx->d_table; a.table_mask = ctx->table_cap - 1; a.slabs = ctx->d_slabs;
    a.size_voxel = size_voxel_map; a.K = K; a.thr_cap = threshold_voxel_capacity; a.select_mode = ctx->search_select_mode;
    a.ids = d_ids; a.nb_xyz = d_xyz; a.num_found = d_nf;
    HIPCHK(ctx, srl_launch_search(a, nb_voxels_visited, ctx->stream));
    HIPCHK(ctx, hipMemcpyAsync(ids, d_ids, (size_t)n * K * sizeof(int), hipMemcpyDeviceToHost, ctx->stream));
    HIPCHK(ctx, hipMemcpyAsync(num_found, d_nf, (size_t)n * sizeof(int), hipMemcpyDeviceToHost, ctx->stream));
    if (nb_xyz) HIPCHK(ctx, hipMemcpyAsync(nb_xyz, d_xyz, (size_t)n * K * 3 * sizeof(float), hipMemcpyDeviceToHost, ctx->stream));
    HIPCHK(ctx, hipStreamSynchronize(ctx->stream));
    return SRL_OK;
}

int srl_transform_points(srl_ctx *ctx, const double *raw_xyz, int n, const double q[4], const double t[3],
                         const double R_il[9], const double t_il[3], double *out_xyz) {
    if (!ctx || n < 0 || (n > 0 && (!raw_xyz || !out_xyz)) || !q || !t || !R_il || !t_il) return SRL_ERR_BAD_ARG;
    SRL_DISARM(ctx);
    if (n == 0) return SRL_OK;
    HIPCHK(ctx, hipSetDevice(ctx->device));
    DevBuf b_in, b_o;
    HIPCHK(ctx, b_in.alloc(ctx, (size_t)n * 3 * sizeof(double)));
    HIPCHK(ctx, b_o.alloc(ctx, (size_t)n * 3 * sizeof(double)));
    double *d_in = b_in.as<double>(), *d_o = b_o.as<double>();
    HIPCHK(ctx, hipMemcpyAsync(d_in, raw_xyz, (size_t)n * 3 * sizeof(double), hipMemcpyHostToDevice, ctx->stream));
    SrlXform X;
    const srl::Mat3 R = srl::Quat(q[0], q[1], q[2], q[3]).toRotationMatrix();
    std::memcpy(X.R, R.a, sizeof X.R);
    std::memcpy(X.t, t, sizeof X.t);
    std::memcpy(X.R_il, R_il, sizeof X.R_il);
    std::memcpy(X.t_il, t_il, sizeof X.t_il);
    HIPCHK(ctx, srl_launch_transform(d_in, n, X, d_o, ctx->stream));
    HIPCHK(ctx, hipMemcpyAsync(out_xyz, d_o, (size_t)n * 3 * sizeof(double), hipMemcpyDeviceToHost, ctx->stream));
    HIPCHK(ctx, hipStreamSynchronize(ctx->stream));
    return SRL_OK;
}

int srl_debug_set_ablate(srl_ctx *ctx, int bits) {
    if (!ctx) return SRL_ERR_BAD_ARG;
    SRL_DISARM(ctx);
    ctx->ablate = bits;
    return SRL_OK;
}
int srl_debug_set_launch_shape(srl_ctx *ctx, int keypoints_per_wave, int waves_per_workgroup) {
    if (!ctx) return SRL_ERR_BAD_ARG;
    SRL_DISARM(ctx);
    if (keypoints_per_wave != 0 && keypoints_per_wave != 2 && keypoints_per_wave != 3 && keypoints_per_wave != 6 && keypoints_per_wave != 12 && keypoints_per_wave != 4 && keypoints_per_wave != 8 && keypoints_per_wave != 16) return SRL_ERR_BAD_ARG;
    if (waves_per_workgroup != 0 && waves_per_workgroup != 4 && waves_per_workgroup != 16) return SRL_ERR_BAD_ARG;
    ctx->force_kpw = keypoints_per_wave;
    ctx->force_wpb = waves_per_workgroup;
    return SRL_OK;
}
int srl_debug_set_bound_culling(srl_ctx *ctx, int enable) {
    if (!ctx) return SRL_ERR_BAD_ARG;
    SRL_DISARM(ctx);
    ctx->bound_mode = enable ? 1 : 0;
    ctx->bound_n = 0;
    return SRL_OK;
}
int srl_debug_set_fused_reduce(srl_ctx *ctx, int enable) {
    if (!ctx) return SRL_ERR_BAD_ARG;
    SRL_DISARM(ctx);
    ctx->fuse_reduce = enable != 0;
    return SRL_OK;
}
int srl_debug_set_select_mode(srl_ctx *ctx, int select_mode) {
    if (!ctx || select_mode < 0 || select_mode > 5) return SRL_ERR_BAD_ARG;
    SRL_DISARM(ctx);
    ctx->select_mode = select_mode;
    return SRL_OK;
}
int srl_debug_set_frame_order_mode(srl_ctx *ctx, int mode) {
    if (!ctx || mode < 0 || mode > 1) return SRL_ERR_BAD_ARG;
    ctx->frame_order_mode = mode;
    return SRL_OK;
}
int srl_debug_frame_order_used(srl_ctx *ctx, int *used) {
    if (!ctx || !used) return SRL_ERR_BAD_ARG;
    *used = ctx->frame_order_used;
    return SRL_OK;
}
int srl_debug_set_search_select_mode(srl_ctx *ctx, int select_mode) {
    if (!ctx || select_mode < 0 || select_mode > 5) return SRL_ERR_BAD_ARG;
    ctx->search_select_mode = select_mode;
    return SRL_OK;
}
int srl_debug_heap_topk(const double *distances, int n, int K, int32_t *out_index) {
    if (n < 0 || K < 1 || K > SRL_MAX_NEIGHBORS || (n > 0 && !distances) || !out_index) return SRL_ERR_BAD_ARG;
    double hd[SRL_MAX_NEIGHBORS];
    int he[SRL_MAX_NEIGHBORS];
    int size = 0;
    for (int i = 0; i < n; i++) size = srl_heap_offer(hd, he, size, K, distances[i], i);
    int out[SRL_MAX_NEIGHBORS];
    srl_heap_drain(hd, he, size, out);
    for (int i = 0; i < size; i++) out_index[i] = out[i];
    return size;
}
int srl_debug_device_sqrt(srl_ctx *ctx, const double *in, int n, double *out) {
    if (!ctx || n < 0 || (n > 0 && (!in || !out))) return SRL_ERR_BAD_ARG;
    SRL_DISARM(ctx);
    if (n == 0) return SRL_OK;
    HIPCHK(ctx, hipSetDevice(ctx->device));
    DevBuf b;
    HIPCHK(ctx, b.alloc(ctx, (size_t)n * sizeof(double)));
    HIPCHK(ctx, hipMemcpyAsync(b.as<double>(), in, (size_t)n * sizeof(double), hipMemcpyHostToDevice, ctx->stream));
    HIPCHK(ctx, srl_launch_sqrt(b.as<double>(), n, ctx->stream));
    HIPCHK(ctx, hipMemcpyAsync(out, b.as<double>(), (size_t)n * sizeof(double), hipMemcpyDeviceToHost, ctx->stream));
    HIPCHK(ctx, hipStreamSynchronize(ctx->stream));
    return SRL_OK;
}

void srl_shard_range(int n, int nranks, int rank, int *begin, int *count) {
    const long long b = (long long)rank * n / nranks;
    const long long e = (long long)(rank + 1) * n / nranks;
    if (begin) *begin = (int)b;
    if (count) *count = (int)(e - b);
}

void srl_shard_budget(int max_num_residuals, const int64_t *accepted_per_rank, int nranks, int rank,
                      int64_t *budget, int *mode) {
    (void)nranks;
    int64_t b = max_num_residuals;
    int m = 0;
    if (max_num_residuals <= 0) {
        int64_t prior = 0;
        for (int r = 0; r < rank; r++) prior += accepted_per_rank ? accepted_per_rank[r] : (int64_t)1;
        m = (prior > 0) ? 2 : 1;
    } else {
        int64_t prior = 0;
        for (int r = 0; r < rank; r++) prior += accepted_per_rank ? accepted_per_rank[r] : 0;
        b = (int64_t)max_num_residuals - prior;
        if (b <= 0) m = 2;
    }
    if (budget) *budget = b;
    if (mode) *mode = m;
}

int srl_build_residuals(srl_ctx *ctx, const srl_frame *f, const srl_icp_opts *o, srl_normal_eq *out) {
    if (!ctx || !f || !o || !out) return SRL_ERR_BAD_ARG;
    if (!ctx->d_table) return SRL_ERR_NO_MAP;
// ... 331 lines not shown
```

sr_livo_amd/csrc/srl_ctx.h:

```cpp
#pragma once
#include "../../include/srlivo_hip.h"
#include "srl_device.h"
#include "host/tr1_relation.h"

#include <hip/hip_runtime.h>
#include "srl_rccl.h"

#include <string>
#include <vector>

struct SrlEpochTable {
    unsigned long long *keyw = nullptr;
    unsigned long long *minw = nullptr;
    unsigned cap = 0;
    unsigned epoch16 = 0;
    unsigned counter32 = 0;
};

#define SRL_PEER_POISON_WORD SRL_PEER_INBOX_GRANULES
#define SRL_PEER_DEVICE_WORD (SRL_PEER_INBOX_GRANULES + 1)
#define SRL_PEER_INBOX_ALLOC_GRANULES (SRL_PEER_INBOX_GRANULES + 8)

struct srl_ctx {
    int device = 0;
    bool counted = false;
    hipStream_t stream = nullptr;
    std::string err;

    SrlMapSlot *d_table = nullptr;
    unsigned table_cap = 0;
    unsigned char *d_slabs = nullptr;
    unsigned slab_cap = 0;
    int num_voxels = 0;
    long long num_points = 0;

    double *d_raw = nullptr;
    int sweep_cap = 0;
    int n = 0;
    int shard_begin = 0;
    int total_n = 0;
    bool sweep_loaded = false;
    int search_select_mode = 0;
    int select_mode = 0;
    int ablate = 0;
    void (*overlap_fn)(void *) = nullptr;
    void *overlap_user = nullptr;

    double *d_raw_next = nullptr;
    double *d_stage_next = nullptr;
    double *d_stage_cur = nullptr;
    int soa_valid_n = 0;
    int next_cap = 0, stage_next_cap = 0, stage_cur_cap = 0;
    int next_n = -1, next_begin = 0, next_total = 0;
    hipStream_t copy_stream = nullptr;
    hipStream_t prefix_stream = nullptr;
    int num_cu = 256;
    hipEvent_t next_ready = nullptr;
    hipEvent_t up_ev[2][2] = {};
    bool up_one_dma[2] = {true, true};
    int next_slot = 0;
    int next_prefix_n = 0;
    int prefix_hint = 0;
    float *d_bound = nullptr;
    int bound_n = 0;
    int bound_sig[4] = {0, 0, 0, 0};
    int bound_mode = 1;
    bool tail_pending = false;
    int cur_slot = 0, cur_prefix_n = 0;

    double *d_frame_raw = nullptr;
    double *d_frame_world = nullptr;
    int frame_cap = 0;
    int frame_n = -1;
    int frame_world_n = -1;
    bool frame_world_seen = false;
    struct SrlColorMap *color = nullptr;
    struct SrlFlow *flow = nullptr;
    double *d_corr_in = nullptr, *d_corr_rel = nullptr, *d_corr_imu = nullptr, *d_corr_raw = nullptr;
    int *d_corr_seg = nullptr;
    int corr_cap = 0;
    int corr_n = -1;
    int *d_sub_kept = nullptr;
    unsigned *d_sub_seen = nullptr;
    int sub_cap = 0;
    int sub_n = -1;
    unsigned sub_seen_tag = 0;

    bool frame_timing = false;
    double frame_stage_us[16] = {};
    long long frame_stage_last_ns = 0;

    hipEvent_t upload_ev = nullptr;
    bool upload_pending = false;

    static constexpr int RING_SLOTS = 4;
    static constexpr int RING_SLOT_BYTES = 256 * 1024;
    char *h_ring = nullptr;
    hipEvent_t ring_ev[RING_SLOTS] = {};
    bool ring_busy[RING_SLOTS] = {};
    unsigned ring_next = 0;

    char *h_scratch = nullptr;
    size_t h_scratch_bytes = 0;
    char *h_frame_x = nullptr;
    size_t h_frame_x_bytes = 0;
    unsigned *d_frame_sync = nullptr;
    unsigned frame_tag = 0;
    SrlTr1Sched *d_tr1_sched = nullptr;
    int tr1_steps = -1;
    unsigned tr1_first[SRL_TR1_MAX_STEPS] = {0}, tr1_nb[SRL_TR1_MAX_STEPS + 1] = {0};
    int frame_order_mode = 0;
    int frame_order_used = 0;
    int *h_insert_cnt = nullptr;
    hipEvent_t ev_insert = nullptr, ev_world = nullptr;
    bool insert_pending = false;
    hipEvent_t ev_frame_read = nullptr;
    SrlEpochTable sel_table, ins_table;

    double *d_rec = nullptr;
    unsigned char *d_status = nullptr;
    double *d_partials = nullptr;
    SrlBlockInfo *d_binfo = nullptr;
    int work_cap = 0;
    int block_cap = 0;
    SrlDevOut *d_out = nullptr;
    SrlDevOut *h_out = nullptr;
    long long *d_count = nullptr;
    long long *h_count = nullptr;
    unsigned long long *d_rec_granules = nullptr;
    size_t rec_granule_cap = 0;
    unsigned long long *d_granules = nullptr;
    int force_kpw = 0, force_wpb = 0;
    bool fuse_reduce = true;
    SrlMailbox *h_mail = nullptr;
    unsigned long long seq = 0;

    int arm_mode = 1;
    int passes_in_solve = 0;
    int expected_passes = 0;
    int pose_box_kind = -1;
    bool pose_box_dev_visible = false;
    unsigned long long *h_pose_box = nullptr;
    unsigned long long *pose_box_pinned = nullptr;
    unsigned long long *pose_box_dev = nullptr;
    unsigned long long *d_pose_relay = nullptr;
    bool armed = false;
    SrlAssocArgs armed_sig;
    int armed_nb = 0, armed_kpw = 0;
    int armed_nblocks = 0;
// ... 6 lines not shown
    unsigned arm_linger_ticks = 30000u;
    unsigned long long arm_stats[4] = {0, 0, 0, 0};
    bool ring_void[512] = {};
    bool ring_marker[512] = {};
    int prof_period = 1;
    unsigned long long prof_count = 0;
    long long ring_last_count = -2;
    bool armed_measured = false, cur_measured = true;
    unsigned timing_gen = 0, armed_gen = 0, cur_gen = 0;
    unsigned ring_gen[512] = {};
    int ring_prev[512] = {};
    long long *h_arm_stamps = nullptr;
    long long arm_host_stamps[64][4] = {};

    bool taps = false;
    int tap_cap = 0, tap_K = 0;
    int *d_tap_ids = nullptr;
    int *d_tap_ncand = nullptr;
    double *d_tap_normal = nullptr, *d_tap_a2d = nullptr, *d_tap_offset = nullptr;
    bool taps_valid = false;
    int last_K = 0;
    long long last_visited_local = -1;

    int nranks = 1, rank = 0;
    ncclComm_t comm = nullptr;
    ncclComm_t parked_comm = nullptr;
    int parked_nranks = 0, parked_rank = 0;
    bool force_coll = false;
    srl_allreduce_fn cb_ar = nullptr;
    srl_allgather_i64_fn cb_ag = nullptr;
    void *cb_user = nullptr;
    long long *d_gather = nullptr;
    size_t d_gather_cap = 0;
    unsigned long long *d_inbox = nullptr;
    SrlPeerTable *d_peer = nullptr;
    void *peer_mapped[SRL_MAX_PEERS] = {};
    bool peer_on = false;
    int peer_seen = 0;
    bool peer_shares_device = false;
    bool comm_shares_device = false;
    bool peer_failed = false;
    unsigned long long *peer_inbox[SRL_MAX_PEERS] = {};
    int peer_deadline_ms = 10000;
    unsigned long long peer_retries = 0;
    unsigned long long peer_seq = 0;
    SrlMailbox *d_mail = nullptr;
    bool dbg_gather = false;

    struct PoolBlock { void *p; size_t bytes; };
    std::vector<PoolBlock> pool_free;

    int last_nblocks = 0;
    int profiling = 0;
    static constexpr int PROF_RING = 512;
    hipEvent_t ring[PROF_RING][2] = {};
    unsigned ring_head = 0, ring_tail = 0;

    hipEvent_t ev[4] = {nullptr, nullptr, nullptr, nullptr};
    srl_timing timing = {};
    int last_nb = 1;
};

#define HIPCHK(ctx, call)                                                                      \
    do {                                                                                       \
        hipError_t e__ = (call);                                                               \
        if (e__ != hipSuccess) {                                                               \
            (ctx)->err = std::string(#call) + ": " + hipGetErrorString(e__);                   \
            return SRL_ERR_HIP;                                                                \
        }                                                                                      \
    } while (0)

#define NCCLCHK(ctx, call)                                                                     \
    do {                                                                                       \
        const SrlRccl *rc__ = srl_rccl();                                                      \
        if (!rc__) { (ctx)->err = srl_rccl_error(); return SRL_ERR_COMM; }                     \
        ncclResult_t r__ = rc__->call;                                                         \
        if (r__ != ncclSuccess) {                                                              \
            (ctx)->err = std::string(#call) + ": " + rc__->GetErrorString(r__);                \
            return SRL_ERR_COMM;                                                               \
        }                                                                                      \
    } while (0)

extern "C" int srl_ctx_disarm(srl_ctx *ctx);
#define SRL_DISARM(ctx) do { if ((ctx)->armed) { int rcd__ = srl_ctx_disarm(ctx); if (rcd__) return rcd__; } } while (0)

#include <chrono>
inline void srl_stage_begin(srl_ctx *ctx) {
    if (!ctx->frame_timing) return;
    hipStreamSynchronize(ctx->stream);
    ctx->frame_stage_last_ns = std::chrono::duration_cast<std::chrono::nanoseconds>(std::chrono::steady_clock::now().time_since_epoch()).count();
}
inline void srl_stage_end(srl_ctx *ctx, int slot) {
    if (!ctx->frame_timing) return;
    hipStreamSynchronize(ctx->stream);
    const long long now = std::chrono::duration_cast<std::chrono::nanoseconds>(std::chrono::steady_clock::now().time_since_epoch()).count();
    ctx->frame_stage_us[slot] += (double)(now - ctx->frame_stage_last_ns) * 1e-3;
    ctx->frame_stage_last_ns = now;
}

inline int srl_map_settle(srl_ctx *ctx) {
    if (!ctx->insert_pending) return SRL_OK;
    HIPCHK(ctx, hipEventSynchronize(ctx->ev_insert));
    ctx->num_voxels += ctx->h_insert_cnt[1];
    ctx->num_points += ctx->h_insert_cnt[2];
    ctx->insert_pending = false;
    return SRL_OK;
}

inline int ensure_copy_stream(srl_ctx *ctx) {
    if (!ctx->copy_stream) HIPCHK(ctx, hipStreamCreateWithFlags(&ctx->copy_stream, hipStreamNonBlocking));
    return SRL_OK;
}
inline int srl_mark_frame_read(srl_ctx *ctx) {
    if (!ctx->ev_frame_read) HIPCHK(ctx, hipEventCreateWithFlags(&ctx->ev_frame_read, hipEventDisableTiming));
    HIPCHK(ctx, hipEventRecord(ctx->ev_frame_read, ctx->stream));
    return SRL_OK;
}

inline int ensure_frame_exchange(srl_ctx *ctx, size_t bytes) {
    if (!ctx->d_frame_sync) {
        HIPCHK(ctx, hipMalloc((void **)&ctx->d_frame_sync, 256));
        HIPCHK(ctx, hipMemsetAsync(ctx->d_frame_sync, 0, 256, ctx->stream));
    }
    if (bytes <= ctx->h_frame_x_bytes) return SRL_OK;
    if (ctx->h_frame_x) {
        HIPCHK(ctx, hipStreamSynchronize(ctx->stream));
        HIPCHK(ctx, hipHostFree(ctx->h_frame_x)); ctx->h_frame_x = nullptr; ctx->h_frame_x_bytes = 0;
    }
    const size_t cap = ((bytes + bytes / 2 + 4095) / 4096) * 4096;
    HIPCHK(ctx, hipHostMalloc((void **)&ctx->h_frame_x, cap, hipHostMallocCoherent | hipHostMallocMapped));
    ctx->h_frame_x_bytes = cap;
    return SRL_OK;
}

inline int ensure_host_scratch(srl_ctx *ctx, size_t bytes) {
    if (bytes <= ctx->h_scratch_bytes) return SRL_OK;
    if (ctx->h_scratch) {
        HIPCHK(ctx, hipStreamSynchronize(ctx->stream));
        HIPCHK(ctx, hipHostFree(ctx->h_scratch)); ctx->h_scratch = nullptr; ctx->h_scratch_bytes = 0;
    }
    const size_t cap = ((bytes + bytes / 2 + 4095) / 4096) * 4096;
    HIPCHK(ctx, hipHostMalloc((void **)&ctx->h_scratch, cap, hipHostMallocDefault));
    ctx->h_scratch_bytes = cap;
    return SRL_OK;
}

template <class T>
int ensure(srl_ctx *ctx, T *&p, size_t count) {
    if (p) { HIPCHK(ctx, hipFree(p)); p = nullptr; }
    if (count == 0) count = 1;
    HIPCHK(ctx, hipMalloc((void **)&p, count * sizeof(T)));
    return SRL_OK;
}

inline int ensure_gather(srl_ctx *ctx, size_t nranks) {
    if (ctx->d_gather && nranks <= ctx->d_gather_cap) return SRL_OK;
    const size_t cap = nranks < 64 ? 64 : nranks;
    int rc = ensure(ctx, ctx->d_gather, cap);
    if (rc) { ctx->d_gather_cap = 0; return rc; }
    ctx->d_gather_cap = cap;
    return SRL_OK;
}

struct DevBuf {
    srl_ctx *ctx = nullptr;
    void *p = nullptr;
// ... 24 lines not shown
```

sr_livo_amd/csrc/srl_device.h:

```cpp
#pragma once
#include <hip/hip_runtime.h>
#include <stddef.h>
#include <stdint.h>


#define SRL_CAP 20
#define SRL_SLAB_BYTES 256
#define SRL_MAX_SLABS 16777215u
#ifndef SRL_KPB
#define SRL_KPB 64
#endif
#ifndef SRL_ASSOC_WAVES_PER_SIMD
#define SRL_ASSOC_WAVES_PER_SIMD 4
#endif
#define SRL_BLOCK 256
#define SRL_SURV_CAP 64
#define SRL_WAVE_SCRATCH 2048
#define SRL_MAXK 32
#define SRL_EMPTY_KEY 0xFFFFFFFFFFFFFFFFull
#define SRL_TABLE_FACTOR 4u
#define SRL_PART_STRIDE 32
#define SRL_ROW_GRANULES 128
#define SRL_FUSED_MAX_BLOCKS 2048
#define SRL_FUSED_GROUP 256
// ... 80 lines not shown
};

struct SrlMailbox {
    SrlDevOut out;
    unsigned long long seq;
    unsigned long long expired;
    unsigned long long pad[10];
    unsigned long long g[2 * (sizeof(SrlDevOut) / 8)];
};
static_assert(sizeof(SrlDevOut) == 52 * 8 && offsetof(SrlDevOut, pad) == 51 * 8, "SrlDevOut is 52 words, the marker word last");
static_assert(offsetof(SrlMailbox, g) % 64 == 0, "the tagged record starts on a cache line");

#define SRL_POSE_BOX_CTRL 42
#define SRL_POSE_BOX_N 43
#define SRL_POSE_BOX_TLAST 44
#define SRL_POSE_BOX_USED 50
#define SRL_POSE_BOX_WRITTEN 56
#define SRL_POSE_BOX_GRANULES 64
#define SRL_ARM_GO 1u
#define SRL_ARM_CANCEL 2u
#define SRL_ARM_EXPIRED 3u
#define SRL_ARM_CODE_MASK 3u
#define SRL_ARM_ALT 4u

#define SRL_REDUCED_DOUBLES 50

#define SRL_MAX_PEERS 8
#define SRL_PEER_ROW 64
#define SRL_PEER_INBOX_GRANULES (2 * SRL_MAX_PEERS * 2 * SRL_PEER_ROW)
#define SRL_PEER_TIMEOUT_MARK 0x9EE9ll
struct SrlPeerTable {
    unsigned long long *inbox[SRL_MAX_PEERS];
    int nranks, rank;
};

struct SrlAssocArgs {
    const double *raw_x, *raw_y, *raw_z;
    const double *aos;
    int n;
    const SrlMapSlot *table;
    unsigned table_mask;
    const unsigned char *slabs;
    int write_rec;
    unsigned inf_off;
    double Rn[9];
    double R[9];
    double t[3];
    double t_last[3];
    double R_il[9];
    double t_il[3];
    double size_voxel;
    double max_dist;
    double lambda_w, lambda_n;
    double power_planarity;
    double nbr_scale;
    int K;
    int min_nb;
    int thr_cap;
    int select_mode;
    int ablate;
    unsigned long long *granules;
    unsigned long long *rec_granules;
    long long cut_max;
    SrlMailbox *mailbox;
    int mail_tagged;
    int pad_mail;
    unsigned long long seq;
    const unsigned long long *pose_box;
    const double *alt_x, *alt_y, *alt_z;
    const double *alt_aos;
    unsigned long long *pose_relay;
    int pose_relayed;
    int pad_relay;
    unsigned pose_epoch;
    unsigned arm_linger_ticks;
    long long *stamps;
    const SrlPeerTable *peer;
    unsigned peer_epoch;
    int peer_slot;
    const float *bound_in;
    float *bound_out;
    int bound_use;
    int pad_bound;
    double *rec;
    unsigned char *status;
    double *partials;
    SrlBlockInfo *binfo;
    int *tap_ids;
    int *tap_ncand;
    double *tap_normal;
    double *tap_a2d;
    double *tap_offset;
};

#define SRL_POSE_DOUBLES 24
static_assert(sizeof(SrlAssocArgs) <= 4096, "the struct travels in the kernarg segment");

struct SrlReduceArgs {
    const double *rec;
    const unsigned char *status;
    const double *partials;
    const SrlBlockInfo *binfo;
    int n;
    int nblocks;
    long long max_res;
    const long long *gather;
    int rank;
    int max_num_residuals;
    SrlDevOut *out;
    SrlMailbox *mailbox;
    unsigned long long seq;
    int kpb;
};

struct SrlSearchArgs {
    const double *q;
    int n;
    const SrlMapSlot *table;
    unsigned table_mask;
    const unsigned char *slabs;
    double size_voxel;
    int K;
    int thr_cap;
    int select_mode;
    int *ids;
    float *nb_xyz;
    int *num_found;
};

hipError_t srl_launch_assoc(const SrlAssocArgs &a, int nb_voxels, int kpw, int wpb, hipStream_t s);
int srl_assoc_lds_bytes(int K, int nb_voxels, int kpw, int wpb);
static inline int srl_keypoints_per_wave(int n) { return n <= 16384 ? 4 : (n <= 32768 ? 8 : 16); }
static inline int srl_keypoints_per_wave_one_round(int n, int num_cu) {
    const int set[7] = {2, 3, 4, 6, 8, 12, 16};
    for (int i = 0; i < 7; ++i) if ((long long)16 * set[i] * num_cu >= n) return set[i];
    return 16;
}
#define SRL_LDS_LIMIT (160 * 1024)
hipError_t srl_launch_reduce(const SrlReduceArgs &a, int mode, hipStream_t s);
hipError_t srl_launch_count(const SrlBlockInfo *binfo, int nblocks, int count_planes, long long *out_total, hipStream_t s);
hipError_t srl_launch_publish(const SrlDevOut *src, SrlMailbox *mb, unsigned long long seq, hipStream_t s);
hipError_t srl_launch_peer_rows(const SrlPeerTable *peer, unsigned epoch, int slot, const SrlDevOut *src, SrlMailbox *mb, unsigned long long seq,
                                const long long *gather_check, hipStream_t s);
hipError_t srl_launch_peer_counts(const SrlPeerTable *peer, unsigned epoch, int slot, const long long *count, long long *gather_out, hipStream_t s);
hipError_t srl_launch_search(const SrlSearchArgs &a, int nb_voxels, hipStream_t s);
struct SrlXform { double R[9], t[3], R_il[9], t_il[3]; };
hipError_t srl_launch_transform(const double *raw_aos, int n, const SrlXform &X, double *out_aos, hipStream_t s);
hipError_t srl_launch_aos_to_soa(const double *aos, int n, double *x, double *y, double *z, hipStream_t s);
hipError_t srl_launch_sqrt(double *io, int n, hipStream_t s);
```

sr_livo_amd/csrc/srl_frame_kernels.hip:

```cpp
#include "srl_ctx.h"
#include "srl_frame_scratch.h"
#include "srl_hash.h"
#include "host/srl_la.h"
#include "host/tr1_order.h"


#include <algorithm>
#include <chrono>
#include <cstdio>
#include <cstdlib>
#include <cstring>
#include <vector>

int srl_map_insert_impl(srl_ctx *ctx, const double *world_xyz, bool on_device, int n, double voxel_size,
                        double min_distance_points, int min_num_points, int *num_added, bool defer_counters,
                        const SrlFrameTransform *xf = nullptr, int (*after_first_kernel)(srl_ctx *, void *) = nullptr, void *user = nullptr,
                        const SrlInsertReport *report = nullptr);

namespace {

using Xf = SrlXf;

__global__ void k_frame_world(const double *raw, int n, const Xf X, double *world) {
    const int i = blockIdx.x * blockDim.x + threadIdx.x;
// ... 718 lines not shown
        } else {
            int rcc = ensure_copy_stream(ctx);
            if (rcc) return rcc;
            if (ctx->ev_frame_read) HIPCHK(ctx, hipStreamWaitEvent(ctx->copy_stream, ctx->ev_frame_read, 0));
            HIPCHK(ctx, hipMemcpyAsync(ctx->d_frame_raw, raw_xyz, (size_t)n * 3 * sizeof(double), hipMemcpyHostToDevice, ctx->copy_stream));
            if (!ctx->upload_ev) HIPCHK(ctx, hipEventCreateWithFlags(&ctx->upload_ev, hipEventDisableTiming));
            HIPCHK(ctx, hipEventRecord(ctx->upload_ev, ctx->copy_stream));
            HIPCHK(ctx, hipStreamWaitEvent(ctx->stream, ctx->upload_ev, 0));
            ctx->upload_pending = true;
        }
    }
    srl_stage_end(ctx, 0);
    return SRL_OK;
}

int srl_frame_size(srl_ctx *ctx, int *n) {
    if (!ctx || !n) return SRL_ERR_BAD_ARG;
    *n = ctx->frame_n < 0 ? 0 : ctx->frame_n;
    return ctx->frame_n < 0 ? SRL_ERR_NO_SWEEP : SRL_OK;
}

int srl_frame_select_keypoints(srl_ctx *ctx, const double q[4], const double t[3], const double R_il[9], const double t_il[3],
                               double sample_voxel_size, int32_t *keypoint_index, int *num_keypoints) {
    if (!ctx || !q || !t || !R_il || !t_il || !(sample_voxel_size > 0.0)) return SRL_ERR_BAD_ARG;
    SRL_DISARM(ctx);
    if (ctx->frame_n < 0 || !ctx->d_frame_raw) { ctx->err = "no frame uploaded"; return SRL_ERR_NO_SWEEP; }
    if (ctx->nranks > 1) { ctx->err = "frame pipeline is single-rank (shard with srl_sweep_upload instead)"; return SRL_ERR_UNSUPPORTED; }
    HIPCHK(ctx, hipSetDevice(ctx->device));
    const int n = ctx->frame_n;
    if (num_keypoints) *num_keypoints = 0;
    hipStream_t st = ctx->stream;
    static const bool trace = std::getenv("SRL_FRAME_TIMING") != nullptr;
    const auto tp0 = std::chrono::steady_clock::now();
    auto tp1 = tp0, tp2 = tp0, tp3 = tp0;
    srl_stage_begin(ctx);
    ctx->frame_order_used = 0;
    int m = 0;
    if (n > 0) {
        if (n > ctx->sweep_cap) {
            if (ctx->d_raw) { HIPCHK(ctx, hipFree(ctx->d_raw)); ctx->d_raw = nullptr; }
            const int cap = std::max(n, 1024);
            HIPCHK(ctx, hipMalloc((void **)&ctx->d_raw, (size_t)cap * 3 * sizeof(double)));
            ctx->sweep_cap = cap;
        }
        int rc = srl_ctx_ensure_work(ctx, n);
        if (rc) return rc;
        Xf X;
        fill_xf(X, q, t, R_il, t_il);
        double *sx = ctx->d_raw, *sy = ctx->d_raw + ctx->sweep_cap, *sz = ctx->d_raw + 2 * (size_t)ctx->sweep_cap;
        GridChain C;
        C.gather_raw = ctx->d_frame_raw; C.gx = sx; C.gy = sy; C.gz = sz;
        rc = grid_chain_enqueue(ctx, C, n, [&](const GroupArgs &G) {
            hipLaunchKernelGGL(k_select_group, dim3((n + 255) / 256), dim3(256), 0, st, ctx->d_frame_raw, n, X, sample_voxel_size, G);
        });
        if (rc) return rc;
        srl_stage_end(ctx, 1);
        tp1 = std::chrono::steady_clock::now();
        rc = grid_chain_wait(ctx, C, "keypoint selection");
        if (rc) return rc;
        srl_stage_end(ctx, 2);
        tp2 = std::chrono::steady_clock::now();
        m = C.m;
        rc = grid_chain_order(ctx, C);
        if (rc) return rc;
        srl_stage_end(ctx, 3);
        if (C.list_on_host) {
            tp3 = std::chrono::steady_clock::now();
            if (m > 0) {
                hipLaunchKernelGGL(k_gather_soa, dim3((m + 255) / 256), dim3(256), 0, st, ctx->d_frame_raw, C.h_list, m, sx, sy, sz);
                HIPCHK(ctx, hipGetLastError());
            }
        } else {
            tp3 = tp2;
            if (keypoint_index && m > 0) {
                HIPCHK(ctx, hipMemcpyAsync(C.h_list, C.d_list, (size_t)m * 4, hipMemcpyDeviceToHost, st));
                HIPCHK(ctx, hipStreamSynchronize(st));
            }
        }
        if (keypoint_index) std::memcpy(keypoint_index, C.h_list, (size_t)m * 4);
    } else {
        srl_stage_end(ctx, 3);
    }
    if (num_keypoints) *num_keypoints = m;
    ctx->total_n = m; ctx->shard_begin = 0; ctx->n = m; ctx->sweep_loaded = true; ctx->taps_valid = false; ctx->bound_n = 0; ctx->tail_pending = false;
    ctx->soa_valid_n = m; ctx->passes_in_solve = 0;
    if (n > 0) { const int rcm = srl_mark_frame_read(ctx); if (rcm) return rcm; }
    srl_stage_end(ctx, 4);
    if (trace) {
        const auto tp4 = std::chrono::steady_clock::now();
        auto us = [](std::chrono::steady_clock::time_point a, std::chrono::steady_clock::time_point b) { return std::chrono::duration<double, std::micro>(b - a).count(); };
        std::fprintf(stderr, "[srl_frame_select_keypoints] n %d -> %d (order %d): enqueue %.0f us, wait %.0f us, host order replay %.0f us, gather + rest %.0f us\n",
                     n, m, ctx->frame_order_used, us(tp0, tp1), us(tp1, tp2), us(tp2, tp3), us(tp3, tp4));
    }
    return SRL_OK;
}

}

namespace {
int frame_commit_impl(srl_ctx *ctx, const double q[4], const double t[3], const double R_il[9], const double t_il[3], double voxel_size, int cap,
                      double min_distance_points, int min_num_points, double *world_out, int *num_added, const SrlInsertReport *report) {
    if (!ctx || !q || !t || !R_il || !t_il) return SRL_ERR_BAD_ARG;
    SRL_DISARM(ctx);
    if (cap != SRL_VOXEL_CAP) { ctx->err = "max_num_points_in_voxel must be 20"; return SRL_ERR_UNSUPPORTED; }
    if (ctx->frame_n < 0 || !ctx->d_frame_raw) { ctx->err = "no frame uploaded"; return SRL_ERR_NO_SWEEP; }
    HIPCHK(ctx, hipSetDevice(ctx->device));
    const int n = ctx->frame_n;
    if (num_added) *num_added = 0;
    if (n == 0) return SRL_OK;
    SrlFrameTransform xf;
    xf.raw = ctx->d_frame_raw; xf.world = ctx->d_frame_world;
    fill_xf(xf.X, q, t, R_il, t_il);
    struct Download { double *world_out; int n; } dl = {world_out, n};
    auto world_ready = [](srl_ctx *c, void *user) -> int {
        const Download *d = static_cast<const Download *>(user);
        { const int rcm = srl_mark_frame_read(c); if (rcm) return rcm; }
        if (d->world_out) {
            int rcc = ensure_copy_stream(c);
            if (rcc) return rcc;
            HIPCHK(c, hipStreamWaitEvent(c->copy_stream, c->ev_frame_read, 0));
            HIPCHK(c, hipMemcpyAsync(d->world_out, c->d_frame_world, (size_t)d->n * 3 * sizeof(double), hipMemcpyDeviceToHost, c->copy_stream));
            if (!c->ev_world) HIPCHK(c, hipEventCreateWithFlags(&c->ev_world, hipEventDisableTiming));
            HIPCHK(c, hipEventRecord(c->ev_world, c->copy_stream));
        }
        return SRL_OK;
    };
    srl_stage_begin(ctx);
    const bool fused = n <= SRL_SCAN_MAX && !ctx->frame_timing;
    if (!fused) {
        hipLaunchKernelGGL(k_frame_world, dim3((n + 255) / 256), dim3(256), 0, ctx->stream, ctx->d_frame_raw, n, xf.X, ctx->d_frame_world);
        HIPCHK(ctx, hipGetLastError());
        srl_stage_end(ctx, 5);
        const int rcw = world_ready(ctx, &dl);
        if (rcw) return rcw;
        srl_stage_end(ctx, 6);
    }
    const int rci = srl_map_insert_impl(ctx, ctx->d_frame_world, true, n, voxel_size, min_distance_points, min_num_points, num_added,
                                        num_added == nullptr && !report, fused ? &xf : nullptr, fused ? +world_ready : nullptr, &dl, report);
    if (world_out && rci == SRL_OK) HIPCHK(ctx, hipEventSynchronize(ctx->ev_world));
    if (rci == SRL_OK) { ctx->frame_world_n = n; ctx->frame_world_seen = true; }
    return rci;
}
}

extern "C" {
int srl_frame_commit(srl_ctx *ctx, const double q[4], const double t[3], const double R_il[9], const double t_il[3],
                     double voxel_size, int cap, double min_distance_points, int min_num_points, double *world_out, int *num_added) {
    return frame_commit_impl(ctx, q, t, R_il, t_il, voxel_size, cap, min_distance_points, min_num_points, world_out, num_added, nullptr);
}
int srl_frame_commit_report(srl_ctx *ctx, const double q[4], const double t[3], const double R_il[9], const double t_il[3],
                            double voxel_size, int cap, double min_distance_points, int min_num_points, double *world_out, uint8_t *outcome,
                            srl_cloud_point *cloud, int *num_cloud, int *num_added) {
    if (num_cloud) *num_cloud = 0;
    if (num_added) *num_added = 0;
    if (!ctx || !q || !t || !R_il || !t_il) return SRL_ERR_BAD_ARG;
    const SrlInsertReport rep = {t[2], outcome, cloud, num_cloud};
    return frame_commit_impl(ctx, q, t, R_il, t_il, voxel_size, cap, min_distance_points, min_num_points, world_out, num_added, &rep);
}
}
```

sr_livo_amd/csrc/srl_kernels.hip:

```cpp
#include "srl_device.h"
#include "srl_hash.h"
#include "srl_heap.h"

#include <math.h>
#include <type_traits>

namespace {

struct alignas(8) VoxEnt { unsigned slab; unsigned count; };
struct Surv { double d2; float x, y, z; unsigned id; };
static_assert(sizeof(Surv) == 24, "survivor record is 24 bytes");
static_assert(SRL_SURV_CAP * 24 + (SRL_MAXK + 1) * 8 <= SRL_WAVE_SCRATCH, "general-path scratch (survivors + sorted d2) must fit");
static_assert(64 * 8 + SRL_MAXK * 16 + SRL_MAXK * 4 <= SRL_WAVE_SCRATCH, "heap replay scratch must fit");

__device__ __forceinline__ int lane_id() {
    return __builtin_amdgcn_mbcnt_hi(~0u, __builtin_amdgcn_mbcnt_lo(~0u, 0));
}
__device__ __forceinline__ int lanes_below(unsigned long long m) {
    return __builtin_amdgcn_mbcnt_hi((unsigned)(m >> 32), __builtin_amdgcn_mbcnt_lo((unsigned)m, 0));
}

struct Cand { bool valid; double d2; float x, y, z; unsigned id; };

__device__ __forceinline__ Cand eval_cand(int e, int nv, const VoxEnt *vox, const unsigned char *slabs,
// ... 174 lines not shown
            const Cand c = eval_cand(lane + 64 * j, nv, vox, slabs, qx, qy, qz);
            const bool s = c.valid && ((float)c.d2 <= tau);
            const unsigned long long m = __ballot(s);
            const int pos = c_surv + lanes_below(m);
            if (s && pos < SRL_SURV_CAP) {
                Surv r; r.d2 = c.d2; r.x = c.x; r.y = c.y; r.z = c.z; r.id = c.id;
                surv[pos] = r;
            }
            c_surv += __popcll(m);
        }
        __builtin_amdgcn_wave_barrier();
        if (c_surv > SRL_SURV_CAP) use_fallback = true;
    }

    if (!use_fallback) {
        const int i = lane;
        const bool act = i < c_surv;
        Surv me;
        if (act) me = surv[i];
        else { me.d2 = __builtin_huge_val(); me.x = me.y = me.z = 0.0f; me.id = 0; }
        int rank = 0;
        for (int j = 0; j < c_surv; ++j) {
            const double dj = surv[j].d2;
            rank += ((dj < me.d2) || (dj == me.d2 && j < i)) ? 1 : 0;
        }
        if (act && rank <= K) sorted[rank] = me.d2;
        __builtin_amdgcn_wave_barrier();
        bool bad = false;
        if (act && rank < K && rank + 1 < c_surv) bad = !(sorted[rank + 1] > me.d2 * SRL_NEAR_TIE);
        tie = __ballot(bad) != 0ull;
        if (!tie && act && rank < K) sink.put(rank, me.x, me.y, me.z, me.id);
        fallback_out = 0;
    } else {
        double last_d2 = -1.0;
        int last_e = -1;
        const int next = total < K + 1 ? total : K + 1;
        for (int r = 0; r < next; ++r) {
            double bd2 = __builtin_huge_val();
            int be = 0x7fffffff;
            for (int j = 0; j < rounds; ++j) {
                const int e = lane + 64 * j;
                const Cand c = eval_cand(e, nv, vox, slabs, qx, qy, qz);
                const bool gt = c.valid && (c.d2 > last_d2 || (c.d2 == last_d2 && e > last_e));
                if (gt && (c.d2 < bd2 || (c.d2 == bd2 && e < be))) { bd2 = c.d2; be = e; }
            }
#pragma unroll
            for (int off = 32; off >= 1; off >>= 1) {
                const double od = __shfl_xor(bd2, off);
                const int oe = __shfl_xor(be, off);
                if (od < bd2 || (od == bd2 && oe < be)) { bd2 = od; be = oe; }
            }
            if (r > 0 && !(bd2 > last_d2 * SRL_NEAR_TIE)) { tie = true; break; }
            if (r < nsel && (be & 63) == lane) {
                const Cand c = eval_cand(be, nv, vox, slabs, qx, qy, qz);
                sink.put(r, c.x, c.y, c.z, c.id);
            }
            last_d2 = bd2;
            last_e = be;
        }
        fallback_out = 1;
    }
    __builtin_amdgcn_wave_barrier();
    if (tie) {
        select_topk_replay(qx, qy, qz, nv, vox, slabs, K, surv, lane, sink, total_out);
        fallback_out = 1;
    }
}

struct LaneRole {
    int pdx, pdy, pdz;
    int c0, slot;
};
__device__ __forceinline__ LaneRole lane_role(int lane) {
    LaneRole r;
    const int pl = lane & 31;
    const int ix = pl / 9, iy = (pl / 3) % 3, iz = pl % 3;
    r.pdx = ix - 1; r.pdy = iy - 1; r.pdz = iz - 1;
    r.c0 = lane / SRL_CAP;
    r.slot = lane - r.c0 * SRL_CAP;
    return r;
}

struct ProbeReq {
    unsigned long long key;
    unsigned h;
    SrlMapSlot s0, s1;
};
__device__ __forceinline__ ProbeReq probe_issue(const int *kv, int kl, const LaneRole &role, const SrlMapSlot *table,
                                                unsigned mask, int lane) {
    ProbeReq r;
    r.key = SRL_EMPTY_KEY; r.h = 0;
    r.s0.key = SRL_EMPTY_KEY; r.s0.slab = 0; r.s0.count = 0;
    r.s1 = r.s0;
    if ((lane & 31) < 27) {
        const int *k = kv + (kl + (lane >> 5)) * 4;
        r.key = srl_pack_key((short)(k[0] + role.pdx), (short)(k[1] + role.pdy), (short)(k[2] + role.pdz));
        r.h = srl_hash_key(r.key) & mask;
        r.s0 = table[r.h];
        r.s1 = table[(r.h + 1) & mask];
    }
    return r;
}
__device__ __forceinline__ int probe_finish(const ProbeReq &r, int thr_cap, const SrlMapSlot *table, unsigned mask,
                                            VoxEnt *vox, int lane, int *ncand_pair, bool cull = false, const float *qf_pair = nullptr,
                                            const int *kv_pair = nullptr, const LaneRole *role = nullptr, float size_voxel = 1.0f) {
    const bool prober = (lane & 31) < 27;
    const bool m0 = prober && r.s0.key == r.key;
    const bool m1 = prober && !m0 && r.s0.key != SRL_EMPTY_KEY && r.s1.key == r.key;
    bool found = m0 || m1;
    unsigned slab = m0 ? r.s0.slab : r.s1.slab, cnt = m0 ? r.s0.count : r.s1.count;
    const bool more = prober && !found && r.s0.key != SRL_EMPTY_KEY && r.s1.key != SRL_EMPTY_KEY;
    if (__ballot(more) != 0ull) {
        if (more) {
            unsigned h = (r.h + 2) & mask;
            for (unsigned probe = 2; probe <= mask; ++probe) {
                const SrlMapSlot sl = table[h];
                if (sl.key == r.key) { slab = sl.slab; cnt = sl.count; found = true; break; }
                if (sl.key == SRL_EMPTY_KEY) break;
                h = (h + 1) & mask;
            }
        }
    }
    found = found && (int)cnt >= thr_cap && cnt > 0;
    {
#if defined(__HIP_DEVICE_COMPILE__)
        int v = found ? (int)cnt : 0;
        v += __builtin_amdgcn_update_dpp(0, v, 0x111, 0xF, 0xF, false);
        v += __builtin_amdgcn_update_dpp(0, v, 0x112, 0xF, 0xF, false);
        v += __builtin_amdgcn_update_dpp(0, v, 0x114, 0xF, 0xF, false);
        v += __builtin_amdgcn_update_dpp(0, v, 0x118, 0xF, 0xF, false);
        v += __builtin_amdgcn_update_dpp(0, v, 0x142, 0xA, 0xF, false);
        if ((lane & 31) == 31) ncand_pair[lane >> 5] = v;
#endif
    }
    if (cull) {
        const int hh = lane >> 5;
        const float *qf = qf_pair + 8 * hh;
        const int *kv = kv_pair + 4 * hh;
        const float r2 = qf[5];
        float bd2 = 0.0f;
        const int pd[3] = {role->pdx, role->pdy, role->pdz};
#pragma unroll
        for (int ax = 0; ax < 3; ++ax) {
            const int v = kv[ax] + pd[ax];
            const float lo = (float)(v > 0 ? v : v - 1) * size_voxel, hi = (float)(v < 0 ? v : v + 1) * size_voxel;
            const float d = fmaxf(fmaxf(lo - qf[ax], qf[ax] - hi), 0.0f);
            bd2 += d * d;
        }
        found = found && bd2 <= r2;
    }
    const unsigned long long m = __ballot(found);
    const unsigned m_lo = (unsigned)m, m_hi = (unsigned)(m >> 32);
    const int nv_a = __popc(m_lo), nv_b = __popc(m_hi);
    if (prober) {
        const bool upper = lane >= 32;
        const unsigned f_lo = found ? m_lo : (~m_lo & 0x7FFFFFFu), f_hi = found ? m_hi : (~m_hi & 0x7FFFFFFu);
        const int below = upper ? (int)__builtin_amdgcn_mbcnt_hi(f_hi, 0u) : (int)__builtin_amdgcn_mbcnt_lo(f_lo, 0u);
        const int nv_own = upper ? nv_b : nv_a;
        VoxEnt ve; ve.slab = found ? slab : 0u; ve.count = found ? cnt : 0u;
        vox[(upper ? 32 : 0) + (found ? below : nv_own + below)] = ve;
    }
    __builtin_amdgcn_wave_barrier();
    return nv_a | (nv_b << 8);
}

struct LdsSink {
    float *col;
    int row;
    int plane;
    int *tap_ids;
    __device__ __forceinline__ void put(int rank, float x, float y, float z, unsigned id) {
        float *p = col + rank * row;
        p[0] = x;
        p[plane] = y;
        p[2 * plane] = z;
        if (tap_ids) tap_ids[rank] = (int)id;
    }
};

struct alignas(16) SurvRec { float x, y, z; int code; };
#define SRL_PAIR_MAX_ROUNDS 4

__device__ __forceinline__ float d2_f32(float px, float py, float pz, float qx, float qy, float qz) {
#pragma clang fp contract(fast)
    const float dx = px - qx, dy = py - qy, dz = pz - qz;
    return dx * dx + dy * dy + dz * dz;
}

template <class Sink>
__device__ __forceinline__ int finish_survivors(double qx, double qy, double qz, int c, const VoxEnt *vox, int K, void *scratch,
                                                int lane, Sink &sink, double *tau_out = nullptr) {
    SurvRec *recs = reinterpret_cast<SurvRec *>(__builtin_assume_aligned(scratch, 16));
    double *keys = reinterpret_cast<double *>(reinterpret_cast<unsigned char *>(scratch) + 1024);
    double *sorted = keys + 66;
    __builtin_amdgcn_wave_barrier();
    const bool act = lane < c;
    SurvRec me;
    me.x = me.y = me.z = 0.0f; me.code = 0;
    double my = __builtin_huge_val();
    if (act) {
        me = recs[lane];
        const double dx = (double)me.x - qx;
        const double dy = (double)me.y - qy;
// ... 611 lines not shown
    }
}

#if defined(__HIP_DEVICE_COMPILE__) && defined(SRL_ARM_STAMPS)
__device__ __forceinline__ void arm_stamp(KargBytes karg, int slot) {
#if !defined(SRL_STAMP_DETAIL)
    if (slot >= 16) return;
#endif
    typedef const __attribute__((address_space(4))) SrlAssocArgs *KP;
    KP q = (KP)karg;
    asm volatile("" : "+s"(q));
    long long *st = q->stamps;
    if (st != nullptr && threadIdx.x == 0) {
        const bool first = blockIdx.x == 0, last = blockIdx.x == gridDim.x - 1;
        if (slot >= 16) { if (last) __hip_atomic_store(st + ((q->seq & 63ull) * 32 + slot), (long long)wall_clock64(), __ATOMIC_RELAXED, __HIP_MEMORY_SCOPE_SYSTEM); return; }
        if (first) __hip_atomic_store(st + ((q->seq & 63ull) * 32 + slot), (long long)wall_clock64(), __ATOMIC_RELAXED, __HIP_MEMORY_SCOPE_SYSTEM);
        if (last) __hip_atomic_store(st + ((q->seq & 63ull) * 32 + 8 + slot), (long long)wall_clock64(), __ATOMIC_RELAXED, __HIP_MEMORY_SCOPE_SYSTEM);
    }
}
#else
__device__ inline void arm_stamp(KargBytes, int) {}
#endif

#ifndef SRL_P2_POLICY
#define SRL_P2_POLICY 1
#endif
#if SRL_P2_POLICY == 0
__host__ __device__ constexpr int p2_lanes_per_keypoint(int kpb) { return kpb >= 48 ? 1 : (kpb >= 32 ? 2 : 4); }
#else
__host__ __device__ constexpr int p2_lanes_per_keypoint(int kpb) { return kpb >= 192 ? 1 : (kpb >= 128 ? 2 : 4); }
#endif
__host__ __device__ constexpr int p2_keypoints_per_wave(int kpb) { return 64 / p2_lanes_per_keypoint(kpb); }

template <int NB, int FAST, int KPW, int WPB, int DBG = 0, int ARMED = 0>
__device__ __forceinline__ bool assoc_tile(KargBytes karg, const SrlAssocArgs &A, const int tile) {
    constexpr int KPB = WPB * KPW;
    extern __shared__ __attribute__((aligned(16))) unsigned char smem[];
    const int Kn = A.K;
    const int abl = DBG ? A.ablate : 0;
    constexpr bool POSE_LDS = ARMED != 0;
    const LdsLayout L = lds_layout(Kn, NB, KPW, WPB, ARMED);
    const int NB_ROW = L.nb_row;
    const int tid = threadIdx.x;
    const int lane = lane_id();
    const int wave = tid >> 6;
    float *s_nb = reinterpret_cast<float *>(smem + L.off_nb);
    const int nb_plane = Kn * NB_ROW;
    double *s_pw = reinterpret_cast<double *>(smem + L.off_pw);
    double *s_pimu = reinterpret_cast<double *>(smem + L.off_pimu);
    float *s_qf = reinterpret_cast<float *>(smem + L.off_qf);
    int *s_kv = reinterpret_cast<int *>(smem + L.off_kv);
    int *s_nfound = reinterpret_cast<int *>(smem + L.off_nfound);
    int *s_ncand = reinterpret_cast<int *>(smem + L.off_ncand);
    int *s_next = reinterpret_cast<int *>(smem + L.off_next);
    unsigned short *s_defer = reinterpret_cast<unsigned short *>(smem + L.off_defer);
    unsigned char *wbase = smem + L.off_wave + wave * L.wave_bytes;
    VoxEnt *vox = reinterpret_cast<VoxEnt *>(wbase + L.off_vox);
    Surv *surv = reinterpret_cast<Surv *>(wbase + L.off_scratch);
    double *s_wpart = reinterpret_cast<double *>(smem + L.off_wpart);
    int *s_winfo = reinterpret_cast<int *>(smem + L.off_winfo);

    const long long dbg_t0 = (DBG && (abl & 128)) ? (long long)wall_clock64() : 0;
#if defined(__HIP_DEVICE_COMPILE__)
    typedef const __attribute__((address_space(4))) SrlAssocArgs *KernargPtr;
#endif
    double *s_pose = reinterpret_cast<double *>(smem + L.off_pose);
    auto n_pass = [&]() -> int {
        if constexpr (ARMED) return __builtin_amdgcn_readfirstlane(reinterpret_cast<const int *>(s_pose + SRL_POSE_DOUBLES)[1]);
        else return A.n;
    };
    int n_fallback = 0;
#if defined(__HIP_DEVICE_COMPILE__)
    auto tile_stamp = [&](int slot) {
        if constexpr (ARMED) {
            arm_stamp(karg, slot - 8);
        }
    };
#else
    auto tile_stamp = [&](int) {};
#endif
    tile_stamp(10);
    bool use_bounds = A.bound_in != nullptr && A.bound_use > 0;
    if constexpr (ARMED) use_bounds = use_bounds && reinterpret_cast<const int *>(s_pose + SRL_POSE_DOUBLES)[2] == 0 && n_pass() == A.n;
    const int bbase_kp = tile * KPB;
    const int wbase_kp = bbase_kp + wave * KPW;

    if (tid < 4) s_next[tid] = 0;
    if (lane < KPW) {
        const int kq = wave * KPW + lane;
        const int g = wbase_kp + lane;
        D3 p_imu = d3(0, 0, 0), p_w = d3(0, 0, 0);
        if constexpr (ARMED) {
            if (g < n_pass()) {
                p_imu = d3(s_pimu[kq * 3 + 0], s_pimu[kq * 3 + 1], s_pimu[kq * 3 + 2]);
                p_w = add(matvec(s_pose, p_imu), d3(s_pose[18], s_pose[19], s_pose[20]));
            }
        } else {
            if (g < A.n) {
                D3 raw;
                if (A.aos != nullptr) {
                    const double *p = A.aos + 3 * (size_t)g;
                    raw = d3(p[0], p[1], p[2]);
                    const_cast<double *>(A.raw_x)[g] = raw.x; const_cast<double *>(A.raw_y)[g] = raw.y; const_cast<double *>(A.raw_z)[g] = raw.z;
                } else {
                    raw = d3(A.raw_x[g], A.raw_y[g], A.raw_z[g]);
                }
                p_imu = add(matvec(A.R_il, raw), d3(A.t_il[0], A.t_il[1], A.t_il[2]));
                p_w = add(matvec(A.Rn, p_imu), d3(A.t[0], A.t[1], A.t[2]));
            }
            s_pimu[kq * 3 + 0] = p_imu.x; s_pimu[kq * 3 + 1] = p_imu.y; s_pimu[kq * 3 + 2] = p_imu.z;
        }
        s_pw[kq * 3 + 0] = p_w.x; s_pw[kq * 3 + 1] = p_w.y; s_pw[kq * 3 + 2] = p_w.z;
        const bool unit = A.size_voxel == 1.0;
        const int kv[3] = {(int)(short)(int)(unit ? p_w.x : p_w.x / A.size_voxel), (int)(short)(int)(unit ? p_w.y : p_w.y / A.size_voxel),
                           (int)(short)(int)(unit ? p_w.z : p_w.z / A.size_voxel)};
        {
            const float qxf = (float)p_w.x, qyf = (float)p_w.y, qzf = (float)p_w.z;
            const float u = 5.9604645e-8f;
            const float am = fmaxf(fmaxf(fabsf(qxf), fabsf(qyf)), fabsf(qzf)) * u + 1e-30f;
            const float h = 4.0f * am * 0.5001f;
            const float m0 = h * (1.0f + 1e-6f) + 8.0f * u * 1e-6f + 4.0f * am * am;
            const float m1 = 2.0f * h + 16.0f * u;
            float *qf = s_qf + kq * 8;
            qf[0] = qxf; qf[1] = qyf; qf[2] = qzf;
            qf[3] = (2.0f * m0) * 1.00001f;
            qf[4] = (1.0f + 2.0f * m1) * 1.00001f;
            float r2 = __builtin_huge_valf();
            if (use_bounds && g < A.bound_use) {
                const float4 bp = reinterpret_cast<const float4 *>(A.bound_in)[g];
                const float ex = qxf - bp.x, ey = qyf - bp.y, ez = qzf - bp.z;
                const float mag = fmaxf(fabsf(qxf) + fabsf(qyf) + fabsf(qzf), fabsf(bp.x) + fabsf(bp.y) + fabsf(bp.z));
                const float slack = 1e-3f + 1e-6f * mag;
                const float rt = sqrtf(bp.w) * 1.000001f;
                const float sz = (float)A.size_voxel;
                const float bq[3] = {bp.x, bp.y, bp.z};
                bool inside = true;
#pragma unroll
                for (int ax = 0; ax < 3; ++ax) {
                    const int vlo = kv[ax] - NB, vhi = kv[ax] + NB;
                    const float lo = (float)(vlo > 0 ? vlo : vlo - 1) * sz, hi = (float)(vhi < 0 ? vhi : vhi + 1) * sz;
                    inside = inside && (bq[ax] - rt) - slack >= lo && (bq[ax] + rt) + slack <= hi;
                }
                if (inside) {
                    const float r = rt + sqrtf(ex * ex + ey * ey + ez * ez) * 1.000001f + slack;
                    r2 = (r * r) * 1.00001f;
                }
            }
            qf[5] = r2;
            *reinterpret_cast<double *>(qf + 6) = __builtin_huge_val();
        }
        s_kv[kq * 4 + 0] = kv[0];
        s_kv[kq * 4 + 1] = kv[1];
        s_kv[kq * 4 + 2] = kv[2];
        s_nfound[kq] = 0;
        s_ncand[kq] = 0;
    } else if (wave == WPB - 1 && lane < KPW + 2) {
        const int kq = KPB + (lane - KPW);
        s_kv[kq * 4 + 0] = 0; s_kv[kq * 4 + 1] = 0; s_kv[kq * 4 + 2] = 0;
    }
    __syncthreads();
    tile_stamp(11);

    {
        const int left = n_pass() - bbase_kp;
        const int n_here = __builtin_amdgcn_readfirstlane(left < KPB ? left : KPB);
        auto make_sink = [&](int kl) {
            LdsSink sink;
            sink.col = s_nb + kl;
            sink.row = NB_ROW;
            sink.plane = nb_plane;
            sink.tap_ids = A.tap_ids ? (A.tap_ids + (size_t)(bbase_kp + kl) * Kn) : nullptr;
            return sink;
        };
        auto keypoint_general = [&](int kl, bool tie) {
            const double qx = s_pw[kl * 3 + 0], qy = s_pw[kl * 3 + 1], qz = s_pw[kl * 3 + 2];
            LdsSink sink = make_sink(kl);
            int total = 0, fb = 0;
            const int nv = probe_voxels<NB>(qx, qy, qz, A.size_voxel, A.thr_cap, A.table, A.table_mask, vox, lane);
            select_topk(qx, qy, qz, nv, vox, A.slabs, Kn, tie ? 5 : A.select_mode, surv, lane, sink, total, fb);
            n_fallback += (NB == 1) ? 1 : fb;
            if (lane == 0) {
                s_nfound[kl] = total < Kn ? total : Kn;
                s_ncand[kl] = total;
            }
        };
        if constexpr (NB == 1 && FAST != 0) {
            const LaneRole role = lane_role(lane);
            const int npairs = n_here > 0 ? (n_here + 1) >> 1 : 0;
            auto take = [&]() { int p = 0; if (lane == 0) p = atomicAdd(s_next, 1); return __builtin_amdgcn_readfirstlane(p); };
            int cur = take();
            ProbeReq preq;
            if (!(abl & 32)) preq = probe_issue(s_kv, 2 * (cur < npairs ? cur : npairs), role, A.table, A.table_mask, lane);
            while (cur < npairs) {
                const int nxt = take();
                const int nv_pair = __builtin_amdgcn_readfirstlane((abl & 8) ? 0 : probe_finish(preq, A.thr_cap, A.table, A.table_mask, vox, lane, s_ncand + 2 * cur, use_bounds, s_qf + 16 * cur,
                                                                                                               s_kv + 8 * cur, &role, (float)A.size_voxel));
                if (!(abl & 32)) preq = probe_issue(s_kv, 2 * (nxt < npairs ? nxt : npairs), role, A.table, A.table_mask, lane);
                auto file = [&](int kl, int done, int total) {
                    (void)total;
                    if (done == SEL_DONE) {
                    } else {
                        s_defer[atomicAdd(s_next + 1, 1)] = (unsigned short)(kl | (done == SEL_TIE ? 0x8000 : 0));
                    }
                };
                const int r_a = (int)((((unsigned)nv_pair & 0xFFu) + 2u) * 0x5556u >> 16), r_b = (int)(((((unsigned)nv_pair >> 8) & 0xFFu) + 2u) * 0x5556u >> 16);
                const int r_max = r_a > r_b ? r_a : r_b;
                if (2 * cur + 1 < n_here && r_max <= SRL_PAIR_MAX_ROUNDS && !(abl & (4 | 256))) {
                    const int kl = 2 * cur;
                    LdsSink sink_a = make_sink(kl), sink_b = make_sink(kl + 1);
                    int total_a = 0, total_b = 0, done;
                    if (r_max <= 2) done = select_pair_f32_r<2>(s_pw + kl * 3, s_pw + kl * 3 + 3, s_qf + kl * 8, s_qf + kl * 8 + 8, vox, A.slabs, A.inf_off, Kn, surv, lane, role, sink_a, sink_b, total_a, total_b, abl);
                    else if (r_max <= 3) done = select_pair_f32_r<3>(s_pw + kl * 3, s_pw + kl * 3 + 3, s_qf + kl * 8, s_qf + kl * 8 + 8, vox, A.slabs, A.inf_off, Kn, surv, lane, role, sink_a, sink_b, total_a, total_b, abl);
                    else done = select_pair_f32_r<4>(s_pw + kl * 3, s_pw + kl * 3 + 3, s_qf + kl * 8, s_qf + kl * 8 + 8, vox, A.slabs, A.inf_off, Kn, surv, lane, role, sink_a, sink_b, total_a, total_b, abl);
                    (void)total_a; (void)total_b;
                    if (done != (SEL_DONE | (SEL_DONE << 8))) {
                        if (lane == 0) {
                            if ((done & 0xFF) != SEL_DONE) s_defer[atomicAdd(s_next + 1, 1)] = (unsigned short)(kl | ((done & 0xFF) == SEL_TIE ? 0x8000 : 0));
                            if ((done >> 8) != SEL_DONE) s_defer[atomicAdd(s_next + 1, 1)] = (unsigned short)((kl + 1) | ((done >> 8) == SEL_TIE ? 0x8000 : 0));
                        }
                    }
                } else {
#pragma nounroll
                    for (int h = 0; h < 2; ++h) {
                        const int kl = 2 * cur + h;
                        if (kl >= n_here) break;
                        const int nv_fast = h ? (nv_pair >> 8) : (nv_pair & 0xFF);
                        const double qx = s_pw[kl * 3 + 0], qy = s_pw[kl * 3 + 1], qz = s_pw[kl * 3 + 2];
                        LdsSink sink = make_sink(kl);
                        int total = nv_fast;
                        int done = SEL_DONE;
                        if (!(abl & 4)) done = select_topk_f32(qx, qy, qz, s_qf + kl * 8, nv_fast, vox + 32 * h, A.slabs, A.inf_off, Kn, surv, lane, role, sink, total, abl);
                        if (lane == 0) file(kl, done, total);
                    }
                }
                cur = nxt;
            }
        } else if constexpr (NB == 2 && FAST != 0) {
            const LaneRole role = lane_role(lane);
            auto take = [&]() { int p = 0; if (lane == 0) p = atomicAdd(s_next, 1); return __builtin_amdgcn_readfirstlane(p); };
            for (int kl = take(); kl < n_here; kl = take()) {
                const double qx = s_pw[kl * 3 + 0], qy = s_pw[kl * 3 + 1], qz = s_pw[kl * 3 + 2];
                int total_all = 0;
                const int nv = probe_voxels<NB>(qx, qy, qz, A.size_voxel, A.thr_cap, A.table, A.table_mask, vox, lane, use_bounds ? s_qf + kl * 8 : nullptr, &total_all);
                if (lane < 3) { VoxEnt z; z.slab = 0u; z.count = 0u; vox[nv + lane] = z; }
                __builtin_amdgcn_wave_barrier();
                LdsSink sink = make_sink(kl);
                int total = 0;
                const int done = select_topk_f32_loop(qx, qy, qz, s_qf + kl * 8, nv, vox, A.slabs, A.inf_off, Kn, surv, lane, role, sink, total);
                total = total_all;
                if (lane == 0) {
                    if (done == SEL_DONE) {
                        s_nfound[kl] = total < Kn ? total : Kn;
                        s_ncand[kl] = total;
                    } else {
                        s_defer[atomicAdd(s_next + 1, 1)] = (unsigned short)(kl | (done == SEL_TIE ? 0x8000 : 0));
                    }
                }
            }
        } else {
            for (int kl = wave * KPW; kl < (wave + 1) * KPW && kl < n_here; ++kl) keypoint_general(kl, false);
        }
        if constexpr (FAST != 0) {
            __syncthreads();
            const int n_defer = __builtin_amdgcn_readfirstlane(s_next[1]);
            if (n_defer > 0) {
                auto take2 = [&]() { int p = 0; if (lane == 0) p = atomicAdd(s_next + 2, 1); return __builtin_amdgcn_readfirstlane(p); };
                for (int i = take2(); i < n_defer; i = take2()) {
                    const int e = __builtin_amdgcn_readfirstlane((int)s_defer[i]);
                    keypoint_general(e & 0x7FFF, (e & 0x8000) != 0);
                }
            }
        }
    }
    __syncthreads();
    tile_stamp(12);

    if (abl & 64) return true;
#if defined(__HIP_DEVICE_COMPILE__)
    KernargPtr bp = (KernargPtr)karg;
    asm volatile("" : "+s"(bp));
// ... 45 lines not shown
        }
        bc = d3(lpk_sum(bc.x), lpk_sum(bc.y), lpk_sum(bc.z));
        const double icnt = rcp_nr((double)nf);
        bc = d3(bc.x * icnt, bc.y * icnt, bc.z * icnt);
        double c00 = 0, c01 = 0, c02 = 0, c11 = 0, c12 = 0, c22 = 0;
        for (int i = sl; i < nf; i += LPK) {
            const float *p = s_nb + i * NB_ROW + kl;
            const double ex = (double)p[0] - bc.x, ey = (double)p[nb_plane] - bc.y, ez = (double)p[2 * nb_plane] - bc.z;
            c00 += ex * ex; c01 += ex * ey; c02 += ex * ez;
            c11 += ey * ey; c12 += ey * ez;
            c22 += ez * ez;
        }
        double C[3][3];
        C[0][0] = lpk_sum(c00); C[0][1] = lpk_sum(c01); C[0][2] = lpk_sum(c02);
        C[1][1] = lpk_sum(c11); C[1][2] = lpk_sum(c12); C[2][2] = lpk_sum(c22);
        C[1][0] = C[0][1]; C[2][0] = C[0][2]; C[2][1] = C[1][2];
        if constexpr (ARMED) arm_stamp(karg, 21);
        double ev[3];
        D3 nrm;
        bool jacobi = b.select_mode == 4;
        if (!jacobi) {
            eig3_closed(C, ev, nrm);
            jacobi = (ev[1] - ev[0]) < 1e-3 * ev[2];
        }
        if (jacobi) { eig3_jacobi(C, ev, nrm); nrm = normalized3(nrm); }
        if constexpr (ARMED) arm_stamp(karg, 22);
        const double sigma_1 = sqrt(fabs(ev[2]));
        const double sigma_2 = sqrt(fabs(ev[1]));
        const double sigma_3 = sqrt(fabs(ev[0]));
        const double a2D = (sigma_2 - sigma_3) * rcp_nr(sigma_1);
        if (a2D != a2D) nan_bad = true;
        const double w_plan = (b.power_planarity == 2.0) ? a2D * a2D : pow(a2D, b.power_planarity);
        const D3 tl = POSE_LDS ? d3(s_pose[21], s_pose[22], s_pose[23]) : d3(b.t_last[0], b.t_last[1], b.t_last[2]);
        if (dot3(nrm, sub(tl, p_imu)) < 0.0) nrm = d3(-1.0 * nrm.x, -1.0 * nrm.y, -1.0 * nrm.z);
        const D3 nn0 = d3((double)s_nb[kl], (double)s_nb[nb_plane + kl], (double)s_nb[2 * nb_plane + kl]);
        const D3 dq = sub(nn0, p_w);
        weight = b.lambda_w * w_plan + b.lambda_n * exp(-sqrt(dot3(dq, dq)) * rcp_nr(b.nbr_scale));
        const D3 nv = normalized3_fast(nrm);
        const double off = -dot3(nv, nn0);
        double Rm[9], tv[3];
#pragma unroll
        for (int i = 0; i < 9; ++i) Rm[i] = POSE_LDS ? s_pose[9 + i] : b.R[i];
#pragma unroll
        for (int i = 0; i < 3; ++i) tv[i] = POSE_LDS ? s_pose[18 + i] : b.t[i];
        const D3 pe = add(matvec(Rm, p_imu), d3(tv[0], tv[1], tv[2]));
        dist = dot3(nv, pe) + off;
        status = 1;
        if (b.tap_normal && sl == 0) {
            b.tap_normal[(size_t)g * 3 + 0] = nv.x; b.tap_normal[(size_t)g * 3 + 1] = nv.y; b.tap_normal[(size_t)g * 3 + 2] = nv.z;
            b.tap_a2d[g] = a2D;
            b.tap_offset[g] = off;
        }
        if (dist < b.max_dist && !nan_bad) {
            status = 2;
            J[0] = nv.x * weight; J[1] = nv.y * weight; J[2] = nv.z * weight;
            const double m0 = -nv.x, m1 = -nv.y, m2 = -nv.z;
            const double r0 = (m0 * Rm[0] + m1 * Rm[3]) + m2 * Rm[6];
            const double r1 = (m0 * Rm[1] + m1 * Rm[4]) + m2 * Rm[7];
            const double r2 = (m0 * Rm[2] + m1 * Rm[5]) + m2 * Rm[8];
            const double s0 = (r0 * 0.0 + r1 * p_imu.z) + r2 * (-p_imu.y);
            const double s1 = (r0 * (-p_imu.z) + r1 * 0.0) + r2 * p_imu.x;
            const double s2 = (r0 * p_imu.y + r1 * (-p_imu.x)) + r2 * 0.0;
            J[3] = s0 * weight; J[4] = s1 * weight; J[5] = s2 * weight;
        }
    }
    if constexpr (ARMED) arm_stamp(karg, 23);
    if (g < n2 && sl == 0 && b.bound_out != nullptr) {
        const float *qf = reinterpret_cast<const float *>(smem + L.off_qf) + kl * 8;
        const double tau = *reinterpret_cast<const double *>(qf + 6);
        float4 bo;
        bo.x = qf[0]; bo.y = qf[1]; bo.z = qf[2];
        bo.w = (float)tau * 1.0000002f;
        reinterpret_cast<float4 *>(b.bound_out)[g] = bo;
    }
    if (g < n2 && b.write_rec && sl == 0) {
        double2 *r = reinterpret_cast<double2 *>(b.rec + (size_t)g * 8);
        double2 v;
        v.x = J[0]; v.y = J[1]; r[0] = v;
        v.x = J[2]; v.y = J[3]; r[1] = v;
        v.x = J[4]; v.y = J[5]; r[2] = v;
        v.x = dist; v.y = weight; r[3] = v;
        b.status[g] = (unsigned char)status;
        if (b.tap_ncand) b.tap_ncand[g] = s_ncand[kl];
    }

    if (b.rec_granules != nullptr && owner_lane && sl == 0) {
        typedef __attribute__((address_space(1))) unsigned long long gu64r;
        const bool accd = status == 2;
        const double rec8[8] = {J[0], J[1], J[2], J[3], J[4], J[5], dist, weight};
        const unsigned long long tag = (unsigned long long)(unsigned)b.seq << 32;
        gu64r *dst = (gu64r *)(b.rec_granules + ((size_t)blockIdx.x * KPB + kl) * 16);
#pragma unroll
        for (int d = 0; d < 8; ++d) {
            const unsigned long long bits = accd ? (unsigned long long)__double_as_longlong(rec8[d]) : 0ull;
            __hip_atomic_store(dst + 2 * d, tag | (bits & 0xFFFFFFFFull), __ATOMIC_RELAXED, __HIP_MEMORY_SCOPE_AGENT);
            __hip_atomic_store(dst + 2 * d + 1, tag | (bits >> 32), __ATOMIC_RELAXED, __HIP_MEMORY_SCOPE_AGENT);
        }
    }

    if (p2_wave) {
        static_assert(P2W * KP2 * 64 <= WPB * (64 * 8 + SRL_WAVE_SCRATCH), "phase-2 rows must fit in the phase-1 per-wave regions");
        double *s_row = reinterpret_cast<double *>(smem + L.off_wave) + w2 * (KP2 * 8);
        const bool accd = status == 2;
        if (sl == 0 && klw < KP2) {
            const double h = dist * weight;
            double4 v;
            v.x = accd ? J[0] : 0.0; v.y = accd ? J[1] : 0.0; v.z = accd ? J[2] : 0.0; v.w = accd ? J[3] : 0.0;
            *reinterpret_cast<double4 *>(s_row + klw * 8) = v;
            v.x = accd ? J[4] : 0.0; v.y = accd ? J[5] : 0.0; v.z = accd ? h : 0.0; v.w = accd ? dist : 0.0;
            *reinterpret_cast<double4 *>(s_row + klw * 8 + 4) = v;
        }
        __builtin_amdgcn_wave_barrier();
        if (lane < SRL_ROW_SUMS) {
            const SrlRowPair p = srl_row_pair(lane);
            double acc = 0.0;
#pragma unroll 16
            for (int k = 0; k < KP2; ++k) acc += s_row[k * 8 + p.ia] * s_row[k * 8 + p.ib];
            s_wpart[w2 * 32 + lane] = acc;
        }
    }
    if constexpr (ARMED) arm_stamp(karg, 24);
    {
        auto per_keypoint = [](unsigned long long m) {
            if (LPK == 2) {
                m &= 0x5555555555555555ull;
                m = (m | (m >> 1)) & 0x3333333333333333ull;
                m = (m | (m >> 2)) & 0x0F0F0F0F0F0F0F0Full;
                m = (m | (m >> 4)) & 0x00FF00FF00FF00FFull;
                m = (m | (m >> 8)) & 0x0000FFFF0000FFFFull;
                m = (m | (m >> 16)) & 0x00000000FFFFFFFFull;
            } else if (LPK == 4) {
                m &= 0x1111111111111111ull;
                m = (m | (m >> 3)) & 0x0303030303030303ull;
                m = (m | (m >> 6)) & 0x000F000F000F000Full;
                m = (m | (m >> 12)) & 0x000000FF000000FFull;
                m = (m | (m >> 24)) & 0xFFFFull;
            }
            return m;
        };
        const unsigned long long acc_mask = __ballot(status == 2 && sl == 0);
        const unsigned long long nan_mask = __ballot(nan_bad);
        const unsigned long long pln_mask = __ballot((status == 1 || status == 2) && sl == 0);
        int pk = (g < n2 && sl == 0) ? s_ncand[kl] : 0;
#pragma unroll
        for (int off = 32; off >= 1; off >>= 1) pk += __shfl_xor(pk, off);
        if (lane == 0) {
            s_winfo[wave * 8 + 3] = n_fallback;
            if (p2_wave) {
                s_winfo[w2 * 8 + 0] = __popcll(acc_mask);
                s_winfo[w2 * 8 + 1] = pk;
                s_winfo[w2 * 8 + 2] = nan_mask ? 1 + w2 * KP2 + (int)__builtin_ctzll(nan_mask) / LPK : 0;
                s_winfo[w2 * 8 + 4] = __popcll(pln_mask);
                const unsigned long long km = per_keypoint(acc_mask);
                s_winfo[w2 * 8 + 5] = (int)(unsigned)km;
                s_winfo[w2 * 8 + 6] = (int)(unsigned)(km >> 32);
            }
        }
    }
    __syncthreads();
    tile_stamp(13);

    if (DBG && (b.ablate & 128) && (tid == 28 || tid == 29 || tid == 30))
        b.partials[(size_t)blockIdx.x * SRL_PART_STRIDE + tid] =
            (tid == 28) ? (double)dbg_t0 : ((tid == 29) ? (double)(long long)wall_clock64() : (double)__builtin_amdgcn_s_getreg(6164) );
    if (tid < SRL_ROW_SUMS && b.granules == nullptr) {
        double v = s_wpart[tid];
// ... 832 lines not shown
```

sr_livo_amd/csrc/srl_map_kernels.hip:

```cpp
#include "srl_ctx.h"
#include "srl_frame_scratch.h"
#include "srl_hash.h"


#include <cstring>
#include <vector>

namespace {


template <bool XF>
__global__ void k_point_slots(const double *xyz, int n, double voxel_size, unsigned long long *keyw, unsigned mask, unsigned epoch16, unsigned *slot_out,
                              unsigned *idx, int *new_flag, const SrlFrameTransform T) {
    const int i = blockIdx.x * blockDim.x + threadIdx.x;
    if (i >= n) return;
    double wx, wy, wz;
    if (XF) {
        srl_transform_point(T.X, T.raw[(size_t)i * 3], T.raw[(size_t)i * 3 + 1], T.raw[(size_t)i * 3 + 2], wx, wy, wz);
        T.world[(size_t)i * 3] = wx; T.world[(size_t)i * 3 + 1] = wy; T.world[(size_t)i * 3 + 2] = wz;
    } else {
        wx = xyz[(size_t)i * 3]; wy = xyz[(size_t)i * 3 + 1]; wz = xyz[(size_t)i * 3 + 2];
    }
    const float fx = (float)wx, fy = (float)wy, fz = (float)wz;
    const short kx = (short)(int)((double)fx / voxel_size);
// ... 252 lines not shown
        const double dy = (double)sl->xyz[0][1] - ly;
        const double dz = (double)sl->xyz[0][2] - lz;
        const bool erase = (dx * dx + dy * dy) + dz * dz > r2;
        keep[v] = erase ? 0 : 1;
        if (erase) mine += sl->count;
    }
#pragma unroll
    for (int off = 32; off >= 1; off >>= 1) mine += __shfl_xor(mine, off);
    if ((threadIdx.x & 63) == 0) wave_sum[threadIdx.x >> 6] = mine;
    __syncthreads();
    if (threadIdx.x == 0) {
        unsigned long long s = 0ull;
        for (int w = 0; w < 16; ++w) s += wave_sum[w];
        if (s != 0ull) atomicAdd(points_removed, s);
    }
}
struct PruneRankSink {
    int *rank;
    int *survivors;
    int n;
    __device__ void operator()(int i, int keep, int excl) const {
        rank[i] = excl;
        if (i == n - 1) *survivors = excl + keep;
    }
};
__global__ void __launch_bounds__(256) k_prune_compact(const unsigned char *slabs, int V, const int *keep, const int *rank, unsigned char *dst) {
    const int v = blockIdx.x * 16 + (threadIdx.x >> 4);
    const int lane = threadIdx.x & 15;
    if (v >= V || !keep[v]) return;
    const uint4 *src = reinterpret_cast<const uint4 *>(slabs + (size_t)v * SRL_SLAB_BYTES);
    uint4 *out = reinterpret_cast<uint4 *>(dst + (size_t)rank[v] * SRL_SLAB_BYTES);
    out[lane] = src[lane];
}

unsigned next_pow2u(unsigned v) { unsigned p = 1; while (p < v) p <<= 1; return p; }

}

extern "C" int srl_map_remove_far(srl_ctx *ctx, const double location[3], double distance, int32_t *num_voxels_removed, int64_t *num_points_removed) {
    if (num_voxels_removed) *num_voxels_removed = 0;
    if (num_points_removed) *num_points_removed = 0;
    if (!ctx || !location) return SRL_ERR_BAD_ARG;
    SRL_DISARM(ctx);
    HIPCHK(ctx, hipSetDevice(ctx->device));
    { const int rcs = srl_map_settle(ctx); if (rcs) return rcs; }
    const int V = ctx->num_voxels;
    if (!ctx->d_table || V <= 0) return SRL_OK;
    hipStream_t st = ctx->stream;
    DevBuf b_keep, b_rank, b_cnt, b_sc;
    HIPCHK(ctx, b_keep.alloc(ctx, (size_t)V * 4));
    HIPCHK(ctx, b_rank.alloc(ctx, (size_t)V * 4));
    HIPCHK(ctx, b_cnt.alloc(ctx, 64));
    HIPCHK(ctx, b_sc.alloc(ctx, srl_scan_scratch_ints(V) * 4));
    unsigned long long *d_removed = b_cnt.as<unsigned long long>();
    int *d_surv = b_cnt.as<int>() + 2;
    HIPCHK(ctx, hipMemsetAsync(b_cnt.p, 0, 16, st));
    hipLaunchKernelGGL(k_prune_mark, dim3(std::min((V + 1023) / 1024, SRL_PRUNE_MARK_BLOCKS)), dim3(1024), 0, st, ctx->d_slabs, V, location[0], location[1],
                       location[2], distance * distance, b_keep.as<int>(), d_removed);
    HIPCHK(ctx, hipGetLastError());
    srl_scan(SrlIntArrayIn{b_keep.as<int>()}, PruneRankSink{b_rank.as<int>(), d_surv, V}, V, b_sc.as<int>(), st);
    HIPCHK(ctx, hipGetLastError());
    { const int rc = ensure_host_scratch(ctx, 64); if (rc) return rc; }
    HIPCHK(ctx, hipMemcpyAsync(ctx->h_scratch, b_cnt.p, 16, hipMemcpyDeviceToHost, st));
    HIPCHK(ctx, hipStreamSynchronize(st));
    long long pts_removed = 0;
    int V_new = 0;
    std::memcpy(&pts_removed, ctx->h_scratch, 8);
    std::memcpy(&V_new, ctx->h_scratch + 8, 4);
    if (V_new == V) return SRL_OK;
    if (V_new > 0) {
        DevBuf b_dst;
        HIPCHK(ctx, b_dst.alloc(ctx, (size_t)V_new * SRL_SLAB_BYTES));
        hipLaunchKernelGGL(k_prune_compact, dim3((V + 15) / 16), dim3(256), 0, st, ctx->d_slabs, V, b_keep.as<int>(), b_rank.as<int>(), b_dst.as<unsigned char>());
        HIPCHK(ctx, hipGetLastError());
        HIPCHK(ctx, hipMemcpyAsync(ctx->d_slabs, b_dst.p, (size_t)V_new * SRL_SLAB_BYTES, hipMemcpyDeviceToDevice, st));
    }
    HIPCHK(ctx, hipMemsetAsync(ctx->d_slabs + (size_t)V_new * SRL_SLAB_BYTES, 0, (size_t)(V - V_new) * SRL_SLAB_BYTES, st));
    hipLaunchKernelGGL(k_fill_empty, dim3((ctx->table_cap + 255) / 256), dim3(256), 0, st, ctx->d_table, ctx->table_cap);
    if (V_new > 0)
        hipLaunchKernelGGL(k_rebuild_table, dim3((V_new + 255) / 256), dim3(256), 0, st, ctx->d_slabs, V_new, ctx->d_table, ctx->table_cap - 1);
    HIPCHK(ctx, hipGetLastError());
    ctx->num_voxels = V_new;
    ctx->num_points -= pts_removed;
    ctx->bound_n = 0;
    ctx->taps_valid = false;
    if (num_voxels_removed) *num_voxels_removed = V - V_new;
    if (num_points_removed) *num_points_removed = pts_removed;
    return SRL_OK;
}

extern "C" int srl_map_probe_checksum(srl_ctx *ctx, const double *world_xyz, int n, int stride, double voxel_size, uint64_t *checksum) {
    if (!ctx || !checksum || !(voxel_size > 0.0) || (world_xyz && n < 0) || stride < 1) return SRL_ERR_BAD_ARG;
    SRL_DISARM(ctx);
    *checksum = 0;
    if (!ctx->d_table) return SRL_ERR_NO_MAP;
    HIPCHK(ctx, hipSetDevice(ctx->device));
    { const int rcs = srl_map_settle(ctx); if (rcs) return rcs; }
    const double *d_pts = nullptr;
    DevBuf b_pts, b_sum;
    if (world_xyz) {
        if (n == 0) return SRL_OK;
        HIPCHK(ctx, b_pts.alloc(ctx, (size_t)n * 3 * sizeof(double)));
        HIPCHK(ctx, hipMemcpyAsync(b_pts.p, world_xyz, (size_t)n * 3 * sizeof(double), hipMemcpyHostToDevice, ctx->stream));
        d_pts = b_pts.as<double>();
    } else {
        if (ctx->frame_world_n <= 0 || !ctx->d_frame_world) return SRL_OK;
        n = ctx->frame_world_n;
        d_pts = ctx->d_frame_world;
    }
    HIPCHK(ctx, b_sum.alloc(ctx, 256));
    HIPCHK(ctx, hipMemsetAsync(b_sum.p, 0, 8, ctx->stream));
    const int probes = (n + stride - 1) / stride;
    hipLaunchKernelGGL(k_probe_checksum, dim3((probes + 255) / 256), dim3(256), 0, ctx->stream, d_pts, n, stride, voxel_size, ctx->d_table, ctx->table_cap - 1,
                       ctx->d_slabs, b_sum.as<unsigned long long>());
    HIPCHK(ctx, hipGetLastError());
    unsigned long long out = 0ull;
    HIPCHK(ctx, hipMemcpyAsync(&out, b_sum.p, 8, hipMemcpyDeviceToHost, ctx->stream));
    HIPCHK(ctx, hipStreamSynchronize(ctx->stream));
    *checksum = (uint64_t)out;
    return SRL_OK;
}

int srl_ctx_grow_map(srl_ctx *ctx, unsigned need_slabs, unsigned need_slots) {
    const unsigned new_slab_cap = ctx->slab_cap >= need_slabs ? ctx->slab_cap : std::max(need_slabs + need_slabs / 2u, 1024u);
    if (new_slab_cap > SRL_MAX_SLABS) { ctx->err = "map too large: slab byte offsets are 32-bit (16.7 M voxels)"; return SRL_ERR_UNSUPPORTED; }
    unsigned new_table_cap = ctx->table_cap;
    while (new_table_cap < need_slots || new_table_cap < SRL_TABLE_FACTOR * new_slab_cap) new_table_cap = next_pow2u(new_table_cap ? new_table_cap * 2u : 2048u);
    if (new_slab_cap != ctx->slab_cap) {
        unsigned char *ns = nullptr;
        HIPCHK(ctx, hipMalloc((void **)&ns, ((size_t)new_slab_cap + 1) * SRL_SLAB_BYTES));
        HIPCHK(ctx, hipMemsetD32Async((hipDeviceptr_t)(ns + (size_t)new_slab_cap * SRL_SLAB_BYTES), 0x7f800000, SRL_SLAB_BYTES / 4, ctx->stream));
        HIPCHK(ctx, hipMemsetAsync(ns, 0, (size_t)new_slab_cap * SRL_SLAB_BYTES, ctx->stream));
        if (ctx->d_slabs && ctx->num_voxels > 0)
            HIPCHK(ctx, hipMemcpyAsync(ns, ctx->d_slabs, (size_t)ctx->num_voxels * SRL_SLAB_BYTES, hipMemcpyDeviceToDevice, ctx->stream));
        HIPCHK(ctx, hipStreamSynchronize(ctx->stream));
        if (ctx->d_slabs) HIPCHK(ctx, hipFree(ctx->d_slabs));
        ctx->d_slabs = ns;
        ctx->slab_cap = new_slab_cap;
    }
    if (new_table_cap != ctx->table_cap) {
        SrlMapSlot *nt = nullptr;
        HIPCHK(ctx, hipMalloc((void **)&nt, (size_t)new_table_cap * sizeof(SrlMapSlot)));
        hipLaunchKernelGGL(k_fill_empty, dim3((new_table_cap + 255) / 256), dim3(256), 0, ctx->stream, nt, new_table_cap);
        if (ctx->num_voxels > 0)
            hipLaunchKernelGGL(k_rebuild_table, dim3((ctx->num_voxels + 255) / 256), dim3(256), 0, ctx->stream,
                               ctx->d_slabs, ctx->num_voxels, nt, new_table_cap - 1);
        HIPCHK(ctx, hipGetLastError());
        HIPCHK(ctx, hipStreamSynchronize(ctx->stream));
        if (ctx->d_table) HIPCHK(ctx, hipFree(ctx->d_table));
        ctx->d_table = nt;
        ctx->table_cap = new_table_cap;
    }
    return SRL_OK;
}

int srl_map_insert_impl(srl_ctx *ctx, const double *world_xyz, bool on_device, int n, double voxel_size,
                        double min_distance_points, int min_num_points, int *num_added, bool defer_counters,
                        const SrlFrameTransform *xf = nullptr, int (*after_first_kernel)(srl_ctx *, void *) = nullptr, void *user = nullptr,
                        const SrlInsertReport *report = nullptr);

extern "C" int srl_debug_radix_sort_pairs(srl_ctx *ctx, const uint32_t *keys, int n, int bits, uint32_t *keys_sorted, uint32_t *positions_sorted) {
    if (!ctx || n < 0 || n > (1 << 25) || bits < 1 || bits > 3 * SRL_RADIX_MAX_BITS || (n > 0 && (!keys || !keys_sorted || !positions_sorted)))
        return SRL_ERR_BAD_ARG;
    if (n == 0) return SRL_OK;
    HIPCHK(ctx, hipSetDevice(ctx->device));
    DevBuf b_in, b_k, b_v, b_tk, b_tv;
    HIPCHK(ctx, b_in.alloc(ctx, (size_t)n * 4)); HIPCHK(ctx, b_k.alloc(ctx, (size_t)n * 4)); HIPCHK(ctx, b_v.alloc(ctx, (size_t)n * 4));
    HIPCHK(ctx, b_tk.alloc(ctx, (size_t)n * 4)); HIPCHK(ctx, b_tv.alloc(ctx, (size_t)n * 4));
    DevBuf b_sc;
    HIPCHK(ctx, b_sc.alloc(ctx, srl_radix_scratch_ints(n) * 4));
    HIPCHK(ctx, hipMemcpyAsync(b_in.p, keys, (size_t)n * 4, hipMemcpyHostToDevice, ctx->stream));
    srl_radix_sort_pairs(b_in.as<unsigned>(), nullptr, b_k.as<unsigned>(), b_v.as<unsigned>(), b_tk.as<unsigned>(), b_tv.as<unsigned>(), n, (unsigned)bits, ctx->stream,
                         b_sc.as<int>());
    HIPCHK(ctx, hipGetLastError());
    HIPCHK(ctx, hipMemcpyAsync(keys_sorted, b_k.p, (size_t)n * 4, hipMemcpyDeviceToHost, ctx->stream));
    HIPCHK(ctx, hipMemcpyAsync(positions_sorted, b_v.p, (size_t)n * 4, hipMemcpyDeviceToHost, ctx->stream));
    HIPCHK(ctx, hipStreamSynchronize(ctx->stream));
    return SRL_OK;
}

int srl_map_insert_device(srl_ctx *ctx, const double *world_xyz, int n, double voxel_size, int cap,
                          double min_distance_points, int min_num_points, int *num_added) {
    (void)cap;
    return srl_map_insert_impl(ctx, world_xyz, false, n, voxel_size, min_distance_points, min_num_points, num_added, false);
}
int srl_map_insert_report_device(srl_ctx *ctx, const double *world_xyz, int n, double voxel_size, int cap, double min_distance_points, int min_num_points,
                                 double ref_z, uint8_t *outcome, srl_cloud_point *cloud, int *num_cloud, int *num_added) {
    (void)cap;
    const SrlInsertReport rep = {ref_z, outcome, cloud, num_cloud};
    return srl_map_insert_impl(ctx, world_xyz, false, n, voxel_size, min_distance_points, min_num_points, num_added, false, nullptr, nullptr, nullptr, &rep);
}

int srl_map_insert_impl(srl_ctx *ctx, const double *world_xyz, bool on_device, int n, double voxel_size,
                        double min_distance_points, int min_num_points, int *num_added, bool defer_counters,
                        const SrlFrameTransform *xf, int (*after_first_kernel)(srl_ctx *, void *), void *user, const SrlInsertReport *report) {
    if (num_added) *num_added = 0;
    if (report && report->num_cloud) *report->num_cloud = 0;
    if (n == 0) return SRL_OK;
    if (!(voxel_size > 0.0)) return SRL_ERR_BAD_ARG;
    ctx->bound_n = 0;
    HIPCHK(ctx, hipSetDevice(ctx->device));
    hipStream_t st = ctx->stream;
    { const int rcs = srl_map_settle(ctx); if (rcs) return rcs; }
    if (!ctx->h_insert_cnt) {
        HIPCHK(ctx, hipHostMalloc((void **)&ctx->h_insert_cnt, 64, hipHostMallocDefault));
        HIPCHK(ctx, hipEventCreateWithFlags(&ctx->ev_insert, hipEventDisableTiming));
    }
    if (!ctx->d_table) {
        ctx->slab_cap = 0; ctx->table_cap = 0; ctx->num_voxels = 0; ctx->num_points = 0;
        int rc = srl_ctx_grow_map(ctx, 4096u, 8192u);
        if (rc) return rc;
    }
    const bool frame_sized = n <= SRL_SCAN_MAX;
    if (frame_sized) {
        const unsigned need_slabs = (unsigned)ctx->num_voxels + (unsigned)n;
        if (need_slabs > ctx->slab_cap || SRL_TABLE_FACTOR * need_slabs > ctx->table_cap) {
            int rc = srl_ctx_grow_map(ctx, need_slabs, SRL_TABLE_FACTOR * need_slabs);
            if (rc) return rc;
        }
    }

    DevBuf b_xyz, b_keys2, b_idx, b_idx2, b_prefix, b_start, b_cnt, b_slot, b_isnew, b_first, b_newflag, b_outcome, b_cloud;
    const double *d_xyz = world_xyz;
    if (!on_device) {
        HIPCHK(ctx, b_xyz.alloc(ctx, (size_t)n * 3 * sizeof(double)));
        HIPCHK(ctx, hipMemcpyAsync(b_xyz.p, world_xyz, (size_t)n * 3 * sizeof(double), hipMemcpyHostToDevice, st));
        d_xyz = b_xyz.as<double>();
    }
    HIPCHK(ctx, b_keys2.alloc(ctx, (size_t)n * 8));
    HIPCHK(ctx, b_idx.alloc(ctx, (size_t)n * 4));
    HIPCHK(ctx, b_idx2.alloc(ctx, (size_t)n * 4));
    HIPCHK(ctx, b_prefix.alloc(ctx, (size_t)n * 4));
    HIPCHK(ctx, b_start.alloc(ctx, (size_t)n * 4));
    HIPCHK(ctx, b_cnt.alloc(ctx, 64));
    HIPCHK(ctx, b_slot.alloc(ctx, (size_t)n * 4));
    HIPCHK(ctx, b_isnew.alloc(ctx, (size_t)n));
    HIPCHK(ctx, b_first.alloc(ctx, (size_t)n * 4));
    HIPCHK(ctx, b_newflag.alloc(ctx, (size_t)n * 4));
    if (report) {
        HIPCHK(ctx, b_outcome.alloc(ctx, (size_t)n));
        HIPCHK(ctx, b_cloud.alloc(ctx, (size_t)n * sizeof(srl_cloud_point)));
    }
    int *cnt = b_cnt.as<int>();
    srl_stage_begin(ctx);
    DevBuf b_sc;
    HIPCHK(ctx, b_sc.alloc(ctx, (srl_radix_scratch_ints(n) + srl_scan_scratch_ints(n)) * 4));
    int *sc_radix = b_sc.as<int>(), *sc_scan = b_sc.as<int>() + srl_radix_scratch_ints(n);
    {
        unsigned cap2 = 1024, bits = 10;
        while (cap2 < 2u * (unsigned)n) { cap2 <<= 1; ++bits; }
        int rct = srl_epoch_table_begin(ctx, ctx->ins_table, cap2, false);
        if (rct) return rct;
        const SrlEpochTable &T = ctx->ins_table;
        DevBuf b_slot_in, b_slot_sorted;
        HIPCHK(ctx, b_slot_in.alloc(ctx, (size_t)n * 4)); HIPCHK(ctx, b_slot_sorted.alloc(ctx, (size_t)n * 4));
        if (xf) {
            hipLaunchKernelGGL(k_point_slots<true>, dim3((n + 255) / 256), dim3(256), 0, st, d_xyz, n, voxel_size, T.keyw, cap2 - 1, T.epoch16,
                               b_slot_in.as<unsigned>(), (unsigned *)nullptr, b_newflag.as<int>(), *xf);
        } else {
            hipLaunchKernelGGL(k_point_slots<false>, dim3((n + 255) / 256), dim3(256), 0, st, d_xyz, n, voxel_size, T.keyw, cap2 - 1, T.epoch16,
                               b_slot_in.as<unsigned>(), (unsigned *)nullptr, b_newflag.as<int>(), SrlFrameTransform());
        }
        HIPCHK(ctx, hipGetLastError());
        if (after_first_kernel) { const int rca = after_first_kernel(ctx, user); if (rca) return rca; }
        srl_radix_sort_pairs(b_slot_in.as<unsigned>(), nullptr, b_slot_sorted.as<unsigned>(), b_idx2.as<unsigned>(), b_prefix.as<unsigned>(), b_idx.as<unsigned>(), n,
                             bits, st, sc_radix);
        HIPCHK(ctx, hipGetLastError());
        srl_stage_end(ctx, 7);
        const SegmentSink seg_sink{b_slot_sorted.as<unsigned>(), b_idx2.as<unsigned>(), T.keyw, b_start.as<int>(), b_keys2.as<unsigned long long>(), ctx->d_table,
                                   ctx->table_cap - 1, b_slot.as<int>(), b_isnew.as<unsigned char>(), min_num_points <= 0 ? b_newflag.as<int>() : (int *)nullptr,
                                   b_first.as<int>(), cnt, n};
        if (report) srl_scan(HeadFlag32{b_slot_sorted.as<unsigned>()}, SegmentSinkReport{seg_sink, b_outcome.as<unsigned char>()}, n, sc_scan, st);
        else srl_scan(HeadFlag32{b_slot_sorted.as<unsigned>()}, seg_sink, n, sc_scan, st);
        HIPCHK(ctx, hipGetLastError());
    }

    srl_stage_end(ctx, 8);
    const bool stage_report = report && frame_sized;
    const size_t stage_outcome = 64, stage_cloud = 64 + (((size_t)n + 63) / 64) * 64;
    int rcs = ensure_host_scratch(ctx, stage_report ? stage_cloud + (size_t)n * sizeof(srl_cloud_point) : 64);
    if (rcs) return rcs;
    int *h_cnt = reinterpret_cast<int *>(ctx->h_scratch);
    if (!frame_sized) {
// ... 61 lines not shown
```

Before: 10720 sweeps/s.

## Cache per-keypoint 27-voxel hash lookups across ESIKF passes when voxel key unchanged

Adds a per-keypoint line of 32 words that records the slab/count results of the 27 neighbour hash probes together with the centre voxel key. On later passes of the same solve, keypoints whose voxel key has not changed read the cached words through buffer loads and skip the hash-table probing. Cached lines are invalidated on map edits, new sweeps and signature changes. The cost is extra HBM traffic for writing and reading the lines, plus some added branching and kernarg fields.

```diff
diff --git a/include/srlivo_hip_debug.h b/include/srlivo_hip_debug.h
--- a/include/srlivo_hip_debug.h
+++ b/include/srlivo_hip_debug.h
@@ -21,6 +21,8 @@
 int srl_debug_set_ablate(srl_ctx *ctx, int bits);
 int srl_debug_set_fused_reduce(srl_ctx *ctx, int enable);
 int srl_debug_set_bound_culling(srl_ctx *ctx, int enable);
+int srl_debug_set_voxel_lines(srl_ctx *ctx, int enable);
+int srl_debug_fetch_voxel_line_taps(srl_ctx *ctx, uint8_t *served);
 int srl_debug_set_pose_box(srl_ctx *ctx, int kind);
 int srl_debug_set_arm_linger(srl_ctx *ctx, double host_linger_us, double kernel_linger_us);
 int srl_debug_pass_stamps(srl_ctx *ctx, int enable, long long *gpu_out, long long *host_out);
diff --git a/sr_livo_amd/capi.py b/sr_livo_amd/capi.py
--- a/sr_livo_amd/capi.py
+++ b/sr_livo_amd/capi.py
@@ -287,6 +287,8 @@
         "srl_debug_set_ablate": ([p, C.c_int], C.c_int),
         "srl_debug_set_fused_reduce": ([p, C.c_int], C.c_int),
         "srl_debug_set_bound_culling": ([p, C.c_int], C.c_int),
+        "srl_debug_set_voxel_lines": ([p, C.c_int], C.c_int),
+        "srl_debug_fetch_voxel_line_taps": ([p, C.c_void_p], C.c_int),
         "srl_debug_set_pose_box": ([p, C.c_int], C.c_int),
         "srl_debug_set_arm_linger": ([p, C.c_double, C.c_double], C.c_int),
         "srl_debug_pass_stamps": ([p, C.c_int, p, p], C.c_int),
@@ -843,6 +845,15 @@
     def set_bound_culling(self, on):
         self._chk(self.lib.srl_debug_set_bound_culling(self.h, 1 if on else 0), "srl_debug_set_bound_culling")
 
+    def set_voxel_lines(self, on):
+        self._chk(self.lib.srl_debug_set_voxel_lines(self.h, 1 if on else 0), "srl_debug_set_voxel_lines")
+
+    def fetch_line_taps(self):
+        _, n, _ = self.sweep_shard()
+        served = np.empty(n, dtype=np.uint8)
+        self._chk(self.lib.srl_debug_fetch_voxel_line_taps(self.h, _ptr(served)), "srl_debug_fetch_voxel_line_taps")
+        return served
+
     def set_search_select_mode(self, mode):
         self._chk(self.lib.srl_debug_set_search_select_mode(self.h, int(mode)), "srl_debug_set_search_select_mode")
 
diff --git a/sr_livo_amd/csrc/srl_capi.cpp b/sr_livo_amd/csrc/srl_capi.cpp
--- a/sr_livo_amd/csrc/srl_capi.cpp
+++ b/sr_livo_amd/csrc/srl_capi.cpp
@@ -44,7 +44,8 @@
     if ((rc = ensure(ctx, ctx->d_rec, (size_t)cap * 8))) return rc;
     if ((rc = ensure(ctx, ctx->d_status, (size_t)cap))) return rc;
     if ((rc = ensure(ctx, ctx->d_bound, (size_t)cap * 4))) return rc;
-    ctx->bound_n = 0;
+    if ((rc = ensure(ctx, ctx->d_line, (size_t)cap * SRL_LINE_WORDS))) return rc;
+    srl_void_pass_memory(ctx);
     if ((rc = ensure(ctx, ctx->d_partials, (size_t)nblocks * SRL_PART_STRIDE))) return rc;
     if ((rc = ensure(ctx, ctx->d_binfo, (size_t)nblocks))) return rc;
     ctx->work_cap = cap;
@@ -71,6 +72,7 @@
     int rc;
     if ((rc = ensure(ctx, ctx->d_tap_ids, (size_t)cap * kk))) return rc;
     if ((rc = ensure(ctx, ctx->d_tap_ncand, (size_t)cap))) return rc;
+    if ((rc = ensure(ctx, ctx->d_tap_line, (size_t)cap))) return rc;
     if ((rc = ensure(ctx, ctx->d_tap_normal, (size_t)cap * 3))) return rc;
     if ((rc = ensure(ctx, ctx->d_tap_a2d, (size_t)cap))) return rc;
     if ((rc = ensure(ctx, ctx->d_tap_offset, (size_t)cap))) return rc;
@@ -178,7 +180,7 @@
     if (ctx->d_sub_kept) hipFree(ctx->d_sub_kept);
     if (ctx->d_sub_seen) hipFree(ctx->d_sub_seen);
     void *bufs[] = {ctx->d_corr_in, ctx->d_corr_rel, ctx->d_corr_imu, ctx->d_corr_raw, ctx->d_corr_seg, ctx->d_frame_raw, ctx->d_frame_world, ctx->d_table, ctx->d_slabs, ctx->d_raw, ctx->d_rec, ctx->d_status, ctx->d_partials, ctx->d_binfo,
-                    ctx->d_out, ctx->d_count, ctx->d_bound, ctx->d_granules, ctx->d_rec_granules, ctx->d_raw_next, ctx->d_stage_next, ctx->d_stage_cur, ctx->d_tap_ids, ctx->d_tap_ncand, ctx->d_tap_normal, ctx->d_tap_a2d,
+                    ctx->d_out, ctx->d_count, ctx->d_bound, ctx->d_line, ctx->d_tap_line, ctx->d_granules, ctx->d_rec_granules, ctx->d_raw_next, ctx->d_stage_next, ctx->d_stage_cur, ctx->d_tap_ids, ctx->d_tap_ncand, ctx->d_tap_normal, ctx->d_tap_a2d,
                     ctx->d_tap_offset, ctx->d_gather, ctx->d_peer, ctx->d_mail};
     for (int r = 0; r < SRL_MAX_PEERS; r++) if (ctx->peer_mapped[r]) hipIpcCloseMemHandle(ctx->peer_mapped[r]);
     if (ctx->d_inbox) hipFree(ctx->d_inbox);
@@ -218,7 +220,7 @@
     if (cap != SRL_VOXEL_CAP) { ctx->err = "max_num_points_in_voxel must be 20"; return SRL_ERR_UNSUPPORTED; }
     HIPCHK(ctx, hipSetDevice(ctx->device));
     { const int rcs = srl_map_settle(ctx); if (rcs) return rcs; }
-    ctx->bound_n = 0;
+    srl_void_pass_memory(ctx);
     const unsigned slab_cap = std::max<unsigned>(1024u, (unsigned)V + (unsigned)V / 2u + 4096u);
     if (slab_cap > SRL_MAX_SLABS) { ctx->err = "map too large: slab byte offsets are 32-bit (16.7 M voxels)"; return SRL_ERR_UNSUPPORTED; }
     const unsigned table_cap = next_pow2(std::max<unsigned>(2048u, SRL_TABLE_FACTOR * slab_cap));
@@ -363,7 +365,7 @@
     ctx->taps_valid = false;
     ctx->passes_in_solve = 0;
     ctx->tail_pending = false;
-    ctx->bound_n = 0;
+    srl_void_pass_memory(ctx);
     if (cnt > ctx->sweep_cap) {
         const int cap = std::max(cnt, 1024);
         int rc = ensure(ctx, ctx->d_raw, (size_t)cap * 3);
@@ -461,7 +463,7 @@
         up = hipSuccess;
     }
     ctx->tail_pending = up != hipSuccess;
-    ctx->bound_n = 0;
+    srl_void_pass_memory(ctx);
     ctx->cur_slot = ctx->next_slot;
     ctx->cur_prefix_n = up == hipSuccess ? ctx->next_n : ctx->next_prefix_n;
     ctx->passes_in_solve = 0;
@@ -900,6 +902,7 @@
     if (ctx->taps) {
         a.tap_ids = ctx->d_tap_ids;
         a.tap_ncand = ctx->d_tap_ncand;
+        a.tap_line = ctx->d_tap_line;
         a.tap_normal = ctx->d_tap_normal;
         a.tap_a2d = ctx->d_tap_a2d;
         a.tap_offset = ctx->d_tap_offset;
@@ -912,6 +915,10 @@
         a.bound_out = ctx->d_bound;
         a.bound_in = ctx->bound_mode != 0 ? ctx->d_bound : nullptr;
         a.bound_use = a.bound_in ? std::min(ctx->bound_n, n_eff) : 0;
+        if (sv_bits != ctx->line_sig) { ctx->line_n = 0; ctx->line_sig = sv_bits; }
+        const bool lines = ctx->line_mode != 0 && p.nb == 1 && (ctx->select_mode == 0 || ctx->select_mode == 4);
+        a.line_in = a.line_out = lines ? ctx->d_line : nullptr;
+        a.line_use = a.line_in ? std::min(ctx->line_n, n_eff) : 0;
     }
     if (p.fused) {
         a.granules = ctx->d_granules;
@@ -970,7 +977,7 @@
     std::memset(sg.t_last, 0, sizeof sg.t_last);
     sg.pose_box = nullptr; sg.pose_relay = nullptr; sg.pose_relayed = 0; sg.pose_epoch = 0; sg.arm_linger_ticks = 0;
     sg.raw_x = sg.raw_y = sg.raw_z = nullptr; sg.alt_x = sg.alt_y = sg.alt_z = nullptr; sg.n = 0; sg.aos = nullptr; sg.alt_aos = nullptr;
-    sg.bound_use = 0;
+    sg.bound_use = 0; sg.line_use = 0;
     return sg;
 }
 
@@ -1054,6 +1061,7 @@
     if ((rc = ensure_pose_box(ctx))) return rc;
     SrlAssocArgs nx = a;
     nx.seq = ctx->seq + 1;
+    nx.line_use = a.line_in ? a.n : 0;
     nx.bound_use = a.bound_in ? a.n : 0;
     const bool has_alt = ctx->d_raw_next != nullptr && ctx->next_cap > 0 && ctx->d_stage_next != nullptr;
     nx.aos = nullptr;
@@ -1234,6 +1242,7 @@
     out->num_fallback = (int32_t)(r.d_fallback + 0.5);
 
     if (a.aos != nullptr && n_eff > ctx->soa_valid_n) ctx->soa_valid_n = n_eff;
+    ctx->line_n = a.line_out ? n_eff : 0;
     ctx->bound_n = n_eff;
     ctx->last_K = p.K;
     ctx->last_nb = p.nb;
@@ -1454,6 +1463,23 @@
     SRL_DISARM(ctx);
     ctx->bound_mode = enable ? 1 : 0;
     ctx->bound_n = 0;
+    return SRL_OK;
+}
+int srl_debug_set_voxel_lines(srl_ctx *ctx, int enable) {
+    if (!ctx) return SRL_ERR_BAD_ARG;
+    SRL_DISARM(ctx);
+    ctx->line_mode = enable ? 1 : 0;
+    ctx->line_n = 0;
+    return SRL_OK;
+}
+int srl_debug_fetch_voxel_line_taps(srl_ctx *ctx, uint8_t *served) {
+    if (!ctx || !served) return SRL_ERR_BAD_ARG;
+    SRL_DISARM(ctx);
+    if (!ctx->taps_valid) { ctx->err = "taps were not enabled for the last srl_build_residuals"; return SRL_ERR_BAD_ARG; }
+    HIPCHK(ctx, hipSetDevice(ctx->device));
+    if (ctx->n == 0) return SRL_OK;
+    HIPCHK(ctx, hipMemcpyAsync(served, ctx->d_tap_line, (size_t)ctx->n, hipMemcpyDeviceToHost, ctx->stream));
+    HIPCHK(ctx, hipStreamSynchronize(ctx->stream));
     return SRL_OK;
 }
 int srl_debug_set_fused_reduce(srl_ctx *ctx, int enable) {
diff --git a/sr_livo_amd/csrc/srl_ctx.h b/sr_livo_amd/csrc/srl_ctx.h
--- a/sr_livo_amd/csrc/srl_ctx.h
+++ b/sr_livo_amd/csrc/srl_ctx.h
@@ -65,6 +65,11 @@
     int bound_n = 0;
     int bound_sig[4] = {0, 0, 0, 0};
     int bound_mode = 1;
+    unsigned *d_line = nullptr;
+    int line_n = 0;
+    int line_sig = 0;
+    int line_mode = 1;
+    unsigned char *d_tap_line = nullptr;
     bool tail_pending = false;
     int cur_slot = 0, cur_prefix_n = 0;
 
@@ -237,6 +242,7 @@
     } while (0)
 
 extern "C" int srl_ctx_disarm(srl_ctx *ctx);
+inline void srl_void_pass_memory(srl_ctx *ctx) { ctx->bound_n = 0; ctx->line_n = 0; }
 #define SRL_DISARM(ctx) do { if ((ctx)->armed) { int rcd__ = srl_ctx_disarm(ctx); if (rcd__) return rcd__; } } while (0)
 
 #include <chrono>
diff --git a/sr_livo_amd/csrc/srl_device.h b/sr_livo_amd/csrc/srl_device.h
--- a/sr_livo_amd/csrc/srl_device.h
+++ b/sr_livo_amd/csrc/srl_device.h
@@ -186,16 +186,27 @@
     float *bound_out;
     int bound_use;
     int pad_bound;
+    const unsigned *line_in;
+    unsigned *line_out;
+    int line_use;
+    int pad_line;
     double *rec;
     unsigned char *status;
     double *partials;
     SrlBlockInfo *binfo;
     int *tap_ids;
     int *tap_ncand;
+    unsigned char *tap_line;
     double *tap_normal;
     double *tap_a2d;
     double *tap_offset;
 };
+
+#define SRL_LINE_WORDS 32
+#define SRL_LINE_KEY 28
+static_assert(SRL_MAX_SLABS < (1u << 24) && SRL_CAP < 256, "a line word is slab | count << 24");
+__host__ __device__ constexpr unsigned srl_line_key_lo(int kx, int ky) { return ((unsigned)kx & 0xFFFFu) | ((unsigned)ky << 16); }
+__host__ __device__ constexpr unsigned srl_line_key_hi(int kz) { return ((unsigned)kz & 0xFFFFu) | 0x10000u; }
 
 #define SRL_POSE_DOUBLES 24
 static_assert(sizeof(SrlAssocArgs) <= 4096, "the struct travels in the kernarg segment");
diff --git a/sr_livo_amd/csrc/srl_frame_kernels.hip b/sr_livo_amd/csrc/srl_frame_kernels.hip
--- a/sr_livo_amd/csrc/srl_frame_kernels.hip
+++ b/sr_livo_amd/csrc/srl_frame_kernels.hip
@@ -824,7 +824,7 @@
         srl_stage_end(ctx, 3);
     }
     if (num_keypoints) *num_keypoints = m;
-    ctx->total_n = m; ctx->shard_begin = 0; ctx->n = m; ctx->sweep_loaded = true; ctx->taps_valid = false; ctx->bound_n = 0; ctx->tail_pending = false;
+    ctx->total_n = m; ctx->shard_begin = 0; ctx->n = m; ctx->sweep_loaded = true; ctx->taps_valid = false; srl_void_pass_memory(ctx); ctx->tail_pending = false;
     ctx->soa_valid_n = m; ctx->passes_in_solve = 0;
     if (n > 0) { const int rcm = srl_mark_frame_read(ctx); if (rcm) return rcm; }
     srl_stage_end(ctx, 4);
diff --git a/sr_livo_amd/csrc/srl_kernels.hip b/sr_livo_amd/csrc/srl_kernels.hip
--- a/sr_livo_amd/csrc/srl_kernels.hip
+++ b/sr_livo_amd/csrc/srl_kernels.hip
@@ -280,43 +280,84 @@
 }
 
 struct ProbeReq {
-    unsigned long long key;
-    unsigned h;
     SrlMapSlot s0, s1;
 };
+__device__ __forceinline__ unsigned long long probe_key(const int *kv, int kl, const LaneRole &role, int lane) {
+    const int *k = kv + (kl + (lane >> 5)) * 4;
+    return srl_pack_key((short)(k[0] + role.pdx), (short)(k[1] + role.pdy), (short)(k[2] + role.pdz));
+}
 __device__ __forceinline__ ProbeReq probe_issue(const int *kv, int kl, const LaneRole &role, const SrlMapSlot *table,
                                                 unsigned mask, int lane) {
     ProbeReq r;
-    r.key = SRL_EMPTY_KEY; r.h = 0;
     r.s0.key = SRL_EMPTY_KEY; r.s0.slab = 0; r.s0.count = 0;
     r.s1 = r.s0;
     if ((lane & 31) < 27) {
-        const int *k = kv + (kl + (lane >> 5)) * 4;
-        r.key = srl_pack_key((short)(k[0] + role.pdx), (short)(k[1] + role.pdy), (short)(k[2] + role.pdz));
-        r.h = srl_hash_key(r.key) & mask;
-        r.s0 = table[r.h];
-        r.s1 = table[(r.h + 1) & mask];
+        const unsigned h = srl_hash_key(probe_key(kv, kl, role, lane)) & mask;
+        r.s0 = table[h];
+        r.s1 = table[(h + 1) & mask];
     }
     return r;
+}
+__device__ __forceinline__ bool pair_on_lines(const int *kv, int kl) {
+    return __builtin_amdgcn_readfirstlane((kv[kl * 4 + 3] != 0 && kv[kl * 4 + 7] != 0) ? 1 : 0) != 0;
+}
+#if defined(__HIP_DEVICE_COMPILE__)
+typedef __amdgpu_buffer_rsrc_t LineRsrc;
+__device__ __forceinline__ LineRsrc lines_rsrc(const unsigned *line0, int bytes) {
+    return __builtin_amdgcn_make_buffer_rsrc((void *)line0, 0, bytes, 0x00020000);
+}
+__device__ __forceinline__ unsigned line_word_load(LineRsrc rs, int kl, int lane) {
+    return __builtin_amdgcn_raw_buffer_load_b32(rs, lane * 4, kl * (SRL_LINE_WORDS * 4), 0);
+}
+__device__ __forceinline__ void line_word_store(LineRsrc rs, int kl, int lane, unsigned w) {
+    __builtin_amdgcn_raw_buffer_store_b32(w, rs, lane * 4, kl * (SRL_LINE_WORDS * 4), 0);
+}
+#else
+struct LineRsrc {};
+__device__ inline LineRsrc lines_rsrc(const unsigned *, int) { return LineRsrc{}; }
+__device__ inline unsigned line_word_load(LineRsrc, int, int) { return 0u; }
+__device__ inline void line_word_store(LineRsrc, int, int, unsigned) {}
+#endif
+__device__ __forceinline__ void line_issue(ProbeReq &r, const int *kv, int kl, LineRsrc lines, int lane) {
+    r.s0.slab = 0u;
+    if ((lane & 31) < 27 && kv[(kl + (lane >> 5)) * 4 + 3] == 1) r.s0.slab = line_word_load(lines, kl, lane);
 }
 __device__ __forceinline__ int probe_finish(const ProbeReq &r, int thr_cap, const SrlMapSlot *table, unsigned mask,
                                             VoxEnt *vox, int lane, int *ncand_pair, bool cull = false, const float *qf_pair = nullptr,
-                                            const int *kv_pair = nullptr, const LaneRole *role = nullptr, float size_voxel = 1.0f) {
+                                            const int *kv_pair = nullptr, const LaneRole *role = nullptr, float size_voxel = 1.0f,
+                                            bool on_lines = false, bool write_lines = false, LineRsrc lines_out = LineRsrc(), int kl_out = 0, int n_exist = 0) {
     const bool prober = (lane & 31) < 27;
-    const bool m0 = prober && r.s0.key == r.key;
-    const bool m1 = prober && !m0 && r.s0.key != SRL_EMPTY_KEY && r.s1.key == r.key;
-    bool found = m0 || m1;
-    unsigned slab = m0 ? r.s0.slab : r.s1.slab, cnt = m0 ? r.s0.count : r.s1.count;
-    const bool more = prober && !found && r.s0.key != SRL_EMPTY_KEY && r.s1.key != SRL_EMPTY_KEY;
-    if (__ballot(more) != 0ull) {
-        if (more) {
-            unsigned h = (r.h + 2) & mask;
-            for (unsigned probe = 2; probe <= mask; ++probe) {
-                const SrlMapSlot sl = table[h];
-                if (sl.key == r.key) { slab = sl.slab; cnt = sl.count; found = true; break; }
-                if (sl.key == SRL_EMPTY_KEY) break;
-                h = (h + 1) & mask;
-            }
+    bool found;
+    unsigned slab, cnt;
+    if (on_lines) {
+        const unsigned w = r.s0.slab;
+        found = w != 0u;
+        slab = w & 0xFFFFFFu;
+        cnt = w >> 24;
+    } else {
+        const unsigned long long key = probe_key(kv_pair, 0, *role, lane);
+        const bool m0 = prober && r.s0.key == key;
+        const bool m1 = prober && !m0 && r.s0.key != SRL_EMPTY_KEY && r.s1.key == key;
+        found = m0 || m1;
+        slab = m0 ? r.s0.slab : r.s1.slab; cnt = m0 ? r.s0.count : r.s1.count;
+        const bool more = prober && !found && r.s0.key != SRL_EMPTY_KEY && r.s1.key != SRL_EMPTY_KEY;
+        if (__ballot(more) != 0ull) {
+            if (more) {
+                unsigned h = ((srl_hash_key(key) & mask) + 2) & mask;
+                for (unsigned probe = 2; probe <= mask; ++probe) {
+                    const SrlMapSlot sl = table[h];
+                    if (sl.key == key) { slab = sl.slab; cnt = sl.count; found = true; break; }
+                    if (sl.key == SRL_EMPTY_KEY) break;
+                    h = (h + 1) & mask;
+                }
+            }
+        }
+        if (write_lines) {
+            const int *kh = kv_pair + 4 * (lane >> 5);
+            const int hl = lane & 31;
+            const unsigned head = hl == SRL_LINE_KEY ? srl_line_key_lo(kh[0], kh[1]) : (hl == SRL_LINE_KEY + 1 ? srl_line_key_hi(kh[2]) : 0u);
+            const unsigned w = prober ? (found ? (slab | (cnt << 24)) : 0u) : head;
+            if ((lane >> 5) < n_exist) line_word_store(lines_out, kl_out, lane, w);
         }
     }
     found = found && (int)cnt >= thr_cap && cnt > 0;
@@ -1094,6 +1135,9 @@
     tile_stamp(10);
     bool use_bounds = A.bound_in != nullptr && A.bound_use > 0;
     if constexpr (ARMED) use_bounds = use_bounds && reinterpret_cast<const int *>(s_pose + SRL_POSE_DOUBLES)[2] == 0 && n_pass() == A.n;
+    constexpr bool LINES = NB == 1 && FAST != 0;
+    bool use_lines = LINES && A.line_in != nullptr && A.line_use > 0;
+    if constexpr (ARMED) use_lines = use_lines && reinterpret_cast<const int *>(s_pose + SRL_POSE_DOUBLES)[2] == 0 && n_pass() == A.n;
     const int bbase_kp = tile * KPB;
     const int wbase_kp = bbase_kp + wave * KPW;
 
@@ -1102,6 +1146,8 @@
         const int kq = wave * KPW + lane;
         const int g = wbase_kp + lane;
         D3 p_imu = d3(0, 0, 0), p_w = d3(0, 0, 0);
+        uint2 line_head; line_head.x = 0u; line_head.y = 0u;
+        if (use_lines && g < A.line_use) line_head = *reinterpret_cast<const uint2 *>(A.line_in + (size_t)g * SRL_LINE_WORDS + SRL_LINE_KEY);
         if constexpr (ARMED) {
             if (g < n_pass()) {
                 p_imu = d3(s_pimu[kq * 3 + 0], s_pimu[kq * 3 + 1], s_pimu[kq * 3 + 2]);
@@ -1164,11 +1210,12 @@
         s_kv[kq * 4 + 0] = kv[0];
         s_kv[kq * 4 + 1] = kv[1];
         s_kv[kq * 4 + 2] = kv[2];
+        s_kv[kq * 4 + 3] = g >= n_pass() ? 2 : ((line_head.x == srl_line_key_lo(kv[0], kv[1]) && line_head.y == srl_line_key_hi(kv[2])) ? 1 : 0);
         s_nfound[kq] = 0;
         s_ncand[kq] = 0;
     } else if (wave == WPB - 1 && lane < KPW + 2) {
         const int kq = KPB + (lane - KPW);
-        s_kv[kq * 4 + 0] = 0; s_kv[kq * 4 + 1] = 0; s_kv[kq * 4 + 2] = 0;
+        s_kv[kq * 4 + 0] = 0; s_kv[kq * 4 + 1] = 0; s_kv[kq * 4 + 2] = 0; s_kv[kq * 4 + 3] = 2;
     }
     __syncthreads();
     tile_stamp(11);
@@ -1202,12 +1249,22 @@
             auto take = [&]() { int p = 0; if (lane == 0) p = atomicAdd(s_next, 1); return __builtin_amdgcn_readfirstlane(p); };
             int cur = take();
             ProbeReq preq;
-            if (!(abl & 32)) preq = probe_issue(s_kv, 2 * (cur < npairs ? cur : npairs), role, A.table, A.table_mask, lane);
+            const int line_bytes = (n_here > 0 ? n_here : 0) * (SRL_LINE_WORDS * 4);
+            const LineRsrc lines = lines_rsrc(A.line_out + (size_t)bbase_kp * SRL_LINE_WORDS, A.line_out != nullptr ? line_bytes : 0);
+            const bool write_lines = A.line_out != nullptr && !(abl & 32);
+            auto issue = [&](int pair) {
+                const int kl = 2 * (pair < npairs ? pair : npairs);
+                const bool on_lines = pair_on_lines(s_kv, kl);
+                if (on_lines) line_issue(preq, s_kv, kl, lines, lane);
+                else preq = probe_issue(s_kv, kl, role, A.table, A.table_mask, lane);
+            };
+            if (!(abl & 32)) issue(cur);
             while (cur < npairs) {
                 const int nxt = take();
                 const int nv_pair = __builtin_amdgcn_readfirstlane((abl & 8) ? 0 : probe_finish(preq, A.thr_cap, A.table, A.table_mask, vox, lane, s_ncand + 2 * cur, use_bounds, s_qf + 16 * cur,
-                                                                                                               s_kv + 8 * cur, &role, (float)A.size_voxel));
-                if (!(abl & 32)) preq = probe_issue(s_kv, 2 * (nxt < npairs ? nxt : npairs), role, A.table, A.table_mask, lane);
+                                                                                                               s_kv + 8 * cur, &role, (float)A.size_voxel, pair_on_lines(s_kv, 2 * cur),
+                                                                                                               write_lines, lines, 2 * cur, n_here - 2 * cur));
+                if (!(abl & 32)) issue(nxt);
                 auto file = [&](int kl, int done, int total) {
                     (void)total;
                     if (done == SEL_DONE) {
@@ -1419,6 +1476,10 @@
         v.x = dist; v.y = weight; r[3] = v;
         b.status[g] = (unsigned char)status;
         if (b.tap_ncand) b.tap_ncand[g] = s_ncand[kl];
+        if (b.tap_line) {
+            const int *s_kvf = reinterpret_cast<const int *>(smem + L.off_kv);
+            b.tap_line[g] = (unsigned char)((s_kvf[kl * 4 + 3] == 1 && s_kvf[(kl ^ 1) * 4 + 3] != 0) ? 1 : 0);
+        }
     }
 
     if (b.rec_granules != nullptr && owner_lane && sl == 0) {
diff --git a/sr_livo_amd/csrc/srl_map_kernels.hip b/sr_livo_amd/csrc/srl_map_kernels.hip
--- a/sr_livo_amd/csrc/srl_map_kernels.hip
+++ b/sr_livo_amd/csrc/srl_map_kernels.hip
@@ -358,7 +358,7 @@
     HIPCHK(ctx, hipGetLastError());
     ctx->num_voxels = V_new;
     ctx->num_points -= pts_removed;
-    ctx->bound_n = 0;
+    srl_void_pass_memory(ctx);
     ctx->taps_valid = false;
     if (num_voxels_removed) *num_voxels_removed = V - V_new;
     if (num_points_removed) *num_points_removed = pts_removed;
@@ -474,7 +474,7 @@
     if (report && report->num_cloud) *report->num_cloud = 0;
     if (n == 0) return SRL_OK;
     if (!(voxel_size > 0.0)) return SRL_ERR_BAD_ARG;
-    ctx->bound_n = 0;
+    srl_void_pass_memory(ctx);
     HIPCHK(ctx, hipSetDevice(ctx->device));
     hipStream_t st = ctx->stream;
     { const int rcs = srl_map_settle(ctx); if (rcs) return rcs; }
```

Measured after the change: 10080 sweeps/s. 6.0% lower.
